# chaoyang223/UDA

Hardware: AMD Instinct MI355X
Metric: TeraSort shuffle+merge GB/s whole-node (higher is better)
Workload: dtype bytes

## Files before the change

### csrc/apps/colpack_bench_main.cc

```cpp
#include <chrono>
#include <cstdio>
#include <cstdlib>
#include <cstring>
#include <string>
#include <thread>
#include <vector>

#include "codec/colpack.h"

namespace {

double now_s() {
  return std::chrono::duration<double>(std::chrono::steady_clock::now().time_since_epoch()).count();
}

uint64_t splitmix(uint64_t& s) {
  uint64_t z = (s += 0x9e3779b97f4a7c15ull);
  z = (z ^ (z >> 30)) * 0xbf58476d1ce4e5b9ull;
  z = (z ^ (z >> 27)) * 0x94d049bb133111ebull;
  return z ^ (z >> 31);
}

void fill(std::vector<uint8_t>& v, int64_t n, uint64_t seed, uint64_t step_mask = 0xFFFFFF) {
  uint64_t key = seed << 40;
  for (int64_t r = 0; r < n; ++r) {
    uint8_t* p = v.data() + r * 104;
    p[0] = 0x0B, p[1] = 0x5B, p[2] = 0x0A, p[13] = 0x5A;
    key += splitmix(seed) & step_mask;
    for (int b = 0; b < 8; ++b) p[3 + b] = (uint8_t)(key >> (56 - 8 * b));
    const uint64_t t = splitmix(seed);
    p[11] = (uint8_t)t, p[12] = (uint8_t)(t >> 8);
    for (int c = 14; c < 104; ++c) p[c] = (uint8_t)('A' + splitmix(seed) % 26);
  }
}

struct Result {
  double unpack = 0, unpack_copy = 0, copy = 0;
  int64_t stride = 0;
};

}

int main(int argc, char** argv) {
  int threads = 1, reps = 3;
  int64_t mib = 128;
  bool scalar = false, v2 = false;
  for (int i = 1; i < argc; ++i) {
    const std::string a = argv[i];
    if (a == "--threads" && i + 1 < argc) threads = std::atoi(argv[++i]);
    else if (a == "--mib" && i + 1 < argc) mib = std::atoll(argv[++i]);
    else if (a == "--reps" && i + 1 < argc) reps = std::atoi(argv[++i]);
    else if (a == "--scalar") scalar = true;
    else if (a == "--v2") v2 = true;
    else {
      std::fprintf(stderr, "usage: uda_colpack_bench [--threads N] [--mib M] [--reps R] [--scalar] [--v2]\n");
      return 2;
    }
  }
  threads = threads < 1 ? 1 : threads;
  const int64_t buf_records = (1 << 20) / 104;
  const int64_t n = (mib << 20) / (buf_records * 104) * buf_records;
  if (n < buf_records || reps < 1) return 2;
  std::vector<Result> res((size_t)threads);
  std::vector<std::thread> thr;
  for (int t = 0; t < threads; ++t)
    thr.emplace_back([&, t] {
      std::vector<uint8_t> raw((size_t)(n * 104));
      fill(raw, n, 1234567 + (uint64_t)t, v2 ? (1ull << 38) - 1 : 0xFFFFFF);
      std::vector<uint8_t> piece((size_t)(v2 ? uda::colpack2_bound(104, n, buf_records) : uda::colpack_bound(104, n)));
      const int64_t len = v2 ? uda::colpack2_encode(raw.data(), n, 104, buf_records, 3, 10, piece.data())
                             : uda::colpack_encode(raw.data(), n, 104, buf_records, piece.data());
      uda::ColpackPiece p;
      if (!uda::colpack_open(piece.data(), len, 104, n, &p) || !p.packed || p.delta != v2) return;
      res[(size_t)t].stride = p.stride;
      std::vector<uint8_t> stg((size_t)(buf_records * 104) * 2), kv((size_t)(buf_records * 104));
      auto pass = [&](int mode) {
        double best = 0;
        for (int r = 0; r < reps; ++r) {
          const double t0 = now_s();
          int64_t turn = 0;
          for (int64_t row = 0; row < n; row += buf_records) {
            uint8_t* s = stg.data() + (size_t)(turn++ & 1) * (size_t)(buf_records * 104);
            if (mode != 2) {
              if (scalar) uda::colpack_unpack_scalar(p, row, buf_records, s);
              else uda::colpack_unpack(p, row, buf_records, s);
            }
            if (mode == 1) std::memcpy(kv.data(), s, kv.size());
            if (mode == 2) std::memcpy(kv.data(), raw.data() + row * 104, kv.size());
            asm volatile("" ::"r"(kv.data()), "r"(s) : "memory");
          }
          const double rate = (double)(n * 104) / (now_s() - t0);
          if (rate > best) best = rate;
        }
        return best;
      };
      res[(size_t)t].unpack = pass(0);
      res[(size_t)t].unpack_copy = pass(1);
      res[(size_t)t].copy = pass(2);
    });
  for (auto& t : thr) t.join();
  double u = 0, uc = 0, c = 0;
  for (const Result& r : res) {
    if (r.stride == 0) {
      std::fprintf(stderr, "a thread's piece did not pack\n");
      return 1;
    }
    u += r.unpack, uc += r.unpack_copy, c += r.copy;
  }
  std::printf("{\"threads\": %d, \"mib_per_thread\": %lld, \"version\": %d, \"stride\": %lld, \"bmi2\": %s, \"path\": \"%s\", "
              "\"unpack_GBps_per_thread\": %.2f, \"unpack_copy_GBps_per_thread\": %.2f, \"copy_GBps_per_thread\": %.2f}\n",
              threads, (long long)mib, v2 ? 2 : 1, (long long)res[0].stride, uda::colpack_have_bmi2() ? "true" : "false",
              scalar || !uda::colpack_have_bmi2() ? "scalar" : "bmi2", u / threads / 1e9, uc / threads / 1e9,
              c / threads / 1e9);
  return 0;
}
```

### csrc/codec/colpack.cc

```cpp
#include "codec/colpack.h"

#include <cstring>

#if defined(__x86_64__)
#include <immintrin.h>
#endif

namespace uda {

namespace {

typedef unsigned __int128 u128;

inline int bit_length(unsigned v) { return v ? 32 - __builtin_clz(v) : 0; }

inline u128 key_mask(int key_len) { return key_len >= 16 ? ~(u128)0 : (((u128)1 << (8 * key_len)) - 1); }

inline u128 load_be(const uint8_t* p, int n) {
  if (n >= 8) {
    uint64_t hi, lo;
    std::memcpy(&hi, p, 8);
    std::memcpy(&lo, p + n - 8, 8);
    return ((u128)__builtin_bswap64(hi) << (8 * (n - 8))) | __builtin_bswap64(lo);
  }
// ... 63 lines not shown

struct KeyWalk {
  const uint8_t* table = nullptr;
  int64_t buf_records = 1;
  int64_t next_restart = 0;
  int key_off = 0, key_len = 0;
  u128 mask = 0, sum = 0;

  void start(const ColpackPiece& p, const ColpackHeader& h, const Layout& lo, int64_t row0) {
    table = p.table;
    buf_records = p.buf_records;
    key_off = p.key_off;
    key_len = p.key_len;
    mask = key_mask(key_len);
    const int64_t rs = row0 - row0 % buf_records;
    next_restart = rs;
    if (rs == row0) return;
    sum = load_be(table + rs / buf_records * kColpackRestartBytes, key_len);
    for (int64_t r = rs + 1; r < row0; ++r)
      sum = (sum + key_delta_of_row(h, lo, p.rows + r * p.stride, key_off, key_len)) & mask;
    next_restart = rs + buf_records;
  }
  inline void fix(int64_t row, uint8_t* rec) {
    if (row == next_restart) {
      sum = load_be(table + row / buf_records * kColpackRestartBytes, key_len);
      next_restart += buf_records;
    } else {
      sum = (sum + load_be(rec + key_off, key_len)) & mask;
    }
    store_be(rec + key_off, key_len, sum);
  }
};

int64_t encode(const uint8_t* src, int64_t nrec, int L, int64_t buf_records, uint32_t version, int key_off,
               int key_len, uint8_t* dst) {
  if (L < 1 || L > kColpackMaxRecordBytes || nrec < 1) return 0;
  if (key_off < 0 || key_len < 0 || key_len > kColpackMaxKeyBytes || key_off + key_len > L) return 0;
  uint8_t mn[kColpackMaxRecordBytes], mx[kColpackMaxRecordBytes];
  uint8_t dmn[kColpackMaxKeyBytes], dmx[kColpackMaxKeyBytes];
  std::memset(mn, 0xFF, sizeof(mn));
  std::memset(mx, 0, sizeof(mx));
  std::memset(dmn, 0xFF, sizeof(dmn));
  std::memset(dmx, 0, sizeof(dmx));
  const bool keyed = key_len > 0 && buf_records >= 1;
  const u128 kmask = key_mask(key_len);
  u128 prev = 0;
  for (int64_t r = 0; r < nrec; ++r) {
    const uint8_t* rec = src + r * L;
    for (int c = 0; c < L; ++c) {
      if (rec[c] < mn[c]) mn[c] = rec[c];
      if (rec[c] > mx[c]) mx[c] = rec[c];
    }
    if (keyed) {
      const u128 k = load_be(rec + key_off, key_len);
      uint8_t t[kColpackMaxKeyBytes];
      store_be(t, key_len, r % buf_records == 0 ? (u128)0 : (k - prev) & kmask);
      prev = k;
      for (int c = 0; c < key_len; ++c) {
        if (t[c] < dmn[c]) dmn[c] = t[c];
        if (t[c] > dmx[c]) dmx[c] = t[c];
      }
    }
  }
  int64_t plain_bits = 0, delta_bits = 0;
  for (int c = 0; c < key_len; ++c) {
    plain_bits += bit_length((unsigned)(mx[key_off + c] - mn[key_off + c]));
    delta_bits += bit_length((unsigned)(dmx[c] - dmn[c]));
  }
  const bool delta = colpack2_choose_delta(plain_bits, delta_bits, nrec, buf_records, key_len);
  if (delta)
    for (int c = 0; c < key_len; ++c) {
      mn[key_off + c] = dmn[c];
      mx[key_off + c] = dmx[c];
    }
  ColpackHeader h;
  std::memset(&h, 0, sizeof(h));
  h.magic = kColpackMagic;
  h.version = version;
  h.record_bytes = (uint32_t)L;
  h.records = (uint64_t)nrec;
  h.buf_records = (uint32_t)buf_records;
  h.groups = (uint32_t)colpack_groups(L);
  h.key_off = (uint32_t)key_off;
  h.key_len = (uint32_t)key_len;
  uint8_t shift[kColpackMaxGroups][8];
  int bits[kColpackMaxGroups];
  uint16_t bo[kColpackMaxGroups];
  const int G = (int)h.groups;
  for (int g = 0; g < G; ++g) {
    int b = 0;
    for (int c = 0; c < 8 && 8 * g + c < L; ++c) {
      const int w = bit_length((unsigned)(mx[8 * g + c] - mn[8 * g + c]));
      shift[g][c] = (uint8_t)b;
      b += w;
      h.mask[g] |= (uint64_t)((1u << w) - 1) << (8 * c);
      h.base[g] |= (uint64_t)mn[8 * g + c] << (8 * c);
    }
    bits[g] = b;
  }
  const bool v1 = version == kColpackVersion;
  const int64_t S = colpack_layout(bits, G, v1, bo);
  for (int g = 0; g < G; ++g) {
    if (v1)
      h.gb[g] = (uint8_t)((bits[g] + 7) / 8);
    else
      h.bo[g] = bo[g];
  }
  h.stride = (uint32_t)S;
  const bool raw = colpack_is_raw(S, L);
  h.flags = (raw ? 0 : kColpackFlagPacked) | (delta ? kColpackFlagDelta : 0);
  std::memcpy(dst, &h, sizeof(h));
  if (raw) return (int64_t)kColpackHeaderBytes;
  const int64_t table_bytes = delta ? colpack2_table_bytes(nrec, buf_records) : 0;
  const int64_t total = v1 ? colpack_packed_bytes(S, nrec) : colpack2_packed_bytes(S, nrec, table_bytes);
  std::memset(dst + kColpackHeaderBytes, 0, (size_t)(total - (int64_t)kColpackHeaderBytes));
  if (delta)
    for (int64_t b = 0; b * buf_records < nrec; ++b)
      std::memcpy(dst + kColpackHeaderBytes + b * kColpackRestartBytes, src + b * buf_records * L + key_off,
                  (size_t)key_len);
  uint8_t* rows = dst + kColpackHeaderBytes + table_bytes;
  prev = 0;
  for (int64_t r = 0; r < nrec; ++r) {
    uint8_t rec[kColpackMaxRecordBytes];
    std::memcpy(rec, src + r * L, (size_t)L);
    if (delta) {
      const u128 k = load_be(rec + key_off, key_len);
      store_be(rec + key_off, key_len, r % buf_records == 0 ? (u128)0 : (k - prev) & kmask);
      prev = k;
    }
    uint8_t* row = rows + r * S;
    for (int g = 0; g < G; ++g) {
      uint64_t word = 0;
      for (int c = 0; c < 8 && 8 * g + c < L; ++c)
        word |= (uint64_t)(uint8_t)(rec[8 * g + c] - mn[8 * g + c]) << shift[g][c];
      const int sh = bo[g] & 7, nb = (sh + bits[g] + 7) / 8;
      word <<= sh;
      for (int k = 0; k < nb; ++k) row[(bo[g] >> 3) + k] |= (uint8_t)(word >> (8 * k));
    }
  }
  return total;
}

}

int64_t colpack_encode(const uint8_t* src, int64_t nrec, int L, int64_t buf_records, uint8_t* dst) {
  return encode(src, nrec, L, buf_records, kColpackVersion, 0, 0, dst);
}

int64_t colpack2_encode(const uint8_t* src, int64_t nrec, int L, int64_t buf_records, int key_off, int key_len,
                        uint8_t* dst) {
  if (key_off < 0 || key_len < 0 || key_len > kColpackMaxKeyBytes || key_off + key_len > L) return 0;
  if (buf_records < 1 || buf_records > 0xFFFFFFFFll) key_len = 0;
  return encode(src, nrec, L, buf_records, kColpackVersion2, key_len > 0 ? key_off : 0, key_len, dst);
}

bool colpack_open(const uint8_t* piece, int64_t len, int expect_L, int64_t expect_records, ColpackPiece* out,
                  const char** why) {
  auto fail = [&](const char* w) {
    if (why) *why = w;
    return false;
  };
  if (!piece || len < (int64_t)kColpackHeaderBytes) return fail("piece shorter than its header");
  const ColpackHeader* h = reinterpret_cast<const ColpackHeader*>(piece);
  ColpackHeader hc;
  std::memcpy(&hc, piece, sizeof(hc));
  if (hc.magic != kColpackMagic) return fail("bad magic");
  if (hc.version != kColpackVersion && hc.version != kColpackVersion2) return fail("unknown version");
  const bool v1 = hc.version == kColpackVersion;
  const int L = (int)hc.record_bytes;
  if (hc.record_bytes < 1 || hc.record_bytes > (uint32_t)kColpackMaxRecordBytes) return fail("record length out of range");
  if (expect_L > 0 && L != expect_L) return fail("record length differs from the stream's");
  if (hc.records < 1 || hc.records > (uint64_t)1 << 40) return fail("record count out of range");
  if (expect_records > 0 && (int64_t)hc.records != expect_records) return fail("record count differs from the item's");
  if ((int)hc.groups != colpack_groups(L)) return fail("group count does not match the record length");
  int bits[kColpackMaxGroups];
  uint16_t bo[kColpackMaxGroups];
  const int G = (int)hc.groups;
  for (int g = 0; g < G; ++g) {
    bits[g] = 0;
    for (int c = 0; c < 8; ++c) {
      const unsigned m = (unsigned)((hc.mask[g] >> (8 * c)) & 0xFF);
      if (m & (m + 1)) return fail("column mask is not a width mask");
      if (8 * g + c >= L && m) return fail("mask past the tail group's columns");
      bits[g] += __builtin_popcount(m);
    }
    if (v1 && hc.gb[g] != (bits[g] + 7) / 8) return fail("group size does not match its widths");
  }
  const int64_t S = colpack_layout(bits, G, v1, bo);
  if (!v1)
    for (int g = 0; g < kColpackMaxGroups; ++g)
      if (hc.bo[g] != (g < G ? bo[g] : 0)) return fail("group offsets do not match the masks");
  if ((int64_t)hc.stride != S) return fail(v1 ? "row stride does not match the group sizes" : "row stride does not match the masks");
  const bool packed = (hc.flags & kColpackFlagPacked) != 0;
  const bool delta = !v1 && (hc.flags & kColpackFlagDelta) != 0;
  int64_t table_bytes = 0;
  if (!v1) {
    if (hc.flags & ~(kColpackFlagPacked | kColpackFlagDelta)) return fail("unknown flags");
    if (hc.key_len > (uint32_t)kColpackMaxKeyBytes || hc.key_off > (uint32_t)L || hc.key_off + hc.key_len > (uint32_t)L)
      return fail("key field outside the record");
    if (delta && hc.key_len == 0) return fail("delta piece without a key");
    if (delta && hc.buf_records < 1) return fail("delta piece without buffer restarts");
    if (delta) table_bytes = colpack2_table_bytes((int64_t)hc.records, (int64_t)hc.buf_records);
  }
  if (packed) {
    if (colpack_is_raw(S, L)) return fail("packed piece with a raw stride");
    const int64_t need = v1 ? colpack_packed_bytes(S, (int64_t)hc.records)
                            : colpack2_packed_bytes(S, (int64_t)hc.records, table_bytes);
    if (need > len) return fail(v1 ? "rows exceed the piece's length" : "table and rows exceed the piece's length");
  }
  out->hdr = h;
  out->table = piece + kColpackHeaderBytes;
  out->rows = piece + kColpackHeaderBytes + table_bytes;
  out->L = L;
  out->version = (int)hc.version;
  out->records = (int64_t)hc.records;
  out->stride = S;
  out->buf_records = (int64_t)hc.buf_records;
  out->key_off = v1 ? 0 : (int)hc.key_off;
  out->key_len = v1 ? 0 : (int)hc.key_len;
  out->packed = packed;
  out->delta = delta;
  return true;
}

void colpack_unpack_scalar(const ColpackPiece& p, int64_t row0, int64_t rows, uint8_t* dst) {
  if (row0 < 0 || rows <= 0 || row0 + rows > p.records) return;
  ColpackHeader h;
  std::memcpy(&h, p.hdr, sizeof(h));
  const Layout lo = layout_of(h, p.L);
  KeyWalk kw;
  if (p.delta) kw.start(p, h, lo, row0);
  for (int64_t r = 0; r < rows; ++r) {
    const uint8_t* row = p.rows + (row0 + r) * p.stride;
    uint8_t* rec = dst + r * p.L;
    for (int g = 0; g < lo.groups; ++g) {
      const uint64_t word = load_le(row + lo.off[g], lo.nbytes[g]) >> lo.sh[g];
      for (int c = 0; c < lo.cols[g]; ++c) {
        const uint64_t m = (h.mask[g] >> (8 * c)) & 0xFF;
        rec[8 * g + c] = (uint8_t)(((word >> lo.shift[g][c]) & m) + ((h.base[g] >> (8 * c)) & 0xFF));
      }
    }
    if (p.delta) kw.fix(row0 + r, rec);
  }
}

bool colpack_have_bmi2() {
#if defined(__x86_64__)
  static const bool have = __builtin_cpu_supports("bmi2");
  return have;
#else
  return false;
#endif
}

#if defined(__x86_64__)
namespace {
template <int kFull, bool kDelta>
__attribute__((target("bmi2"))) void unpack_bmi2(const ColpackPiece& p, int64_t row0, int64_t rows, uint8_t* dst) {
  ColpackHeader h;
  std::memcpy(&h, p.hdr, sizeof(h));
  const Layout lo = layout_of(h, p.L);
  const int full = kFull ? kFull : p.L / 8;
  const int tail = kFull ? 0 : p.L % 8;
  const int64_t S = p.stride;
  const int L = p.L;
  KeyWalk kw;
  if (kDelta) kw.start(p, h, lo, row0);
  const uint8_t* row = p.rows + row0 * S;
  for (int64_t r = 0; r < rows; ++r, row += S, dst += L) {
#pragma GCC unroll 16
    for (int g = 0; g < full; ++g) {
      uint64_t x;
      std::memcpy(&x, row + lo.off[g], 8);
      x = _pdep_u64(x >> lo.sh[g], h.mask[g]) + h.base[g];
      std::memcpy(dst + 8 * g, &x, 8);
    }
    if (tail) {
      uint64_t x;
      std::memcpy(&x, row + lo.off[full], 8);
      x = _pdep_u64(x >> lo.sh[full], h.mask[full]) + h.base[full];
      std::memcpy(dst + 8 * full, &x, (size_t)tail);
    }
    if (kDelta) kw.fix(row0 + r, dst);
  }
}
}
#endif

bool colpack_unpack_bmi2(const ColpackPiece& p, int64_t row0, int64_t rows, uint8_t* dst) {
#if defined(__x86_64__)
  if (!colpack_have_bmi2()) return false;
  if (row0 < 0 || rows <= 0 || row0 + rows > p.records) return true;
  if (p.L == 104)
    p.delta ? unpack_bmi2<13, true>(p, row0, rows, dst) : unpack_bmi2<13, false>(p, row0, rows, dst);
  else
    p.delta ? unpack_bmi2<0, true>(p, row0, rows, dst) : unpack_bmi2<0, false>(p, row0, rows, dst);
  return true;
#else
  return false;
#endif
}

void colpack_unpack(const ColpackPiece& p, int64_t row0, int64_t rows, uint8_t* dst) {
  if (!colpack_unpack_bmi2(p, row0, rows, dst)) colpack_unpack_scalar(p, row0, rows, dst);
}

}
```

### csrc/codec/colpack.h

```cpp
#pragma once
#include <cstddef>
#include <cstdint>

#if defined(__HIP__)
#define UDA_COLPACK_HD __host__ __device__ inline
#else
#define UDA_COLPACK_HD inline
#endif

namespace uda {

constexpr uint32_t kColpackMagic = 0x4b504c43u;
constexpr uint32_t kColpackVersion = 1;
constexpr uint32_t kColpackVersion2 = 2;
constexpr int kColpackMaxRecordBytes = 256;
constexpr int kColpackMaxGroups = kColpackMaxRecordBytes / 8;
constexpr uint32_t kColpackFlagPacked = 1;
constexpr uint32_t kColpackFlagDelta = 2;
constexpr int kColpackMaxKeyBytes = 16;
constexpr int kColpackRestartBytes = 16;

struct ColpackHeader {
  uint32_t magic;
  uint32_t version;
  uint32_t record_bytes;
  uint32_t flags;
  uint64_t records;
  uint32_t buf_records;
  uint32_t stride;
  uint32_t groups;
  uint32_t key_off;
  uint32_t key_len;
  uint32_t reserved[5];
  uint64_t mask[kColpackMaxGroups];
  uint64_t base[kColpackMaxGroups];
  union {
    struct {
      uint8_t gb[kColpackMaxGroups];
      uint8_t pad[32];
    };
    uint16_t bo[kColpackMaxGroups];
  };
};
constexpr size_t kColpackHeaderBytes = sizeof(ColpackHeader);
static_assert(kColpackHeaderBytes == 640 && kColpackHeaderBytes % 64 == 0, "header is 64-byte aligned");

UDA_COLPACK_HD int colpack_groups(int L) { return (L + 7) / 8; }
UDA_COLPACK_HD bool colpack_is_raw(int64_t S, int64_t L) { return 10 * S > 9 * L; }
UDA_COLPACK_HD int64_t colpack_max_stride(int64_t L) { return 9 * L / 10; }
UDA_COLPACK_HD int64_t colpack_packed_bytes(int64_t S, int64_t nrec) {
  return ((int64_t)kColpackHeaderBytes + S * nrec + 8 + 63) / 64 * 64;
// ... 2 lines not shown


UDA_COLPACK_HD int colpack_layout(const int* bits, int groups, bool align_all, uint16_t* bo) {
  int cur = 0;
  for (int g = 0; g < groups; ++g) {
    if (bits[g] > 0 && (align_all || (cur & 7) + bits[g] > 64)) cur = (cur + 7) & ~7;
    bo[g] = (uint16_t)cur;
    cur += bits[g];
  }
  return (cur + 7) / 8;
}
UDA_COLPACK_HD int colpack_mask_bits(uint64_t m) {
  int n = 0;
  for (; m; m &= m - 1) ++n;
  return n;
}
UDA_COLPACK_HD int64_t colpack2_table_bytes(int64_t nrec, int64_t buf_records) {
  if (buf_records < 1) return 0;
  return ((nrec + buf_records - 1) / buf_records * kColpackRestartBytes + 63) / 64 * 64;
}
UDA_COLPACK_HD int64_t colpack2_packed_bytes(int64_t S, int64_t nrec, int64_t table_bytes) {
  return ((int64_t)kColpackHeaderBytes + table_bytes + S * nrec + 8 + 63) / 64 * 64;
}
UDA_COLPACK_HD int64_t colpack2_bound(int64_t L, int64_t nrec, int64_t buf_records) {
  return colpack2_packed_bytes(colpack_max_stride(L), nrec, colpack2_table_bytes(nrec, buf_records));
}
UDA_COLPACK_HD bool colpack2_choose_delta(int64_t plain_key_bits, int64_t delta_key_bits, int64_t nrec,
                                          int64_t buf_records, int key_len) {
  if (key_len <= 0 || buf_records < 1) return false;
  const int64_t entries = (nrec + buf_records - 1) / buf_records;
  return delta_key_bits * nrec + 128 * entries < plain_key_bits * nrec;
}

int64_t colpack_encode(const uint8_t* src, int64_t nrec, int L, int64_t buf_records, uint8_t* dst);
int64_t colpack2_encode(const uint8_t* src, int64_t nrec, int L, int64_t buf_records, int key_off, int key_len,
                        uint8_t* dst);

struct ColpackPiece {
  const ColpackHeader* hdr = nullptr;
  const uint8_t* table = nullptr;
  const uint8_t* rows = nullptr;
  int L = 0;
  int version = 0;
  int64_t records = 0;
  int64_t stride = 0;
  int64_t buf_records = 0;
  int key_off = 0, key_len = 0;
  bool packed = false;
  bool delta = false;
};
bool colpack_open(const uint8_t* piece, int64_t len, int expect_L, int64_t expect_records, ColpackPiece* out,
                  const char** why = nullptr);

void colpack_unpack(const ColpackPiece& p, int64_t row0, int64_t rows, uint8_t* dst);
void colpack_unpack_scalar(const ColpackPiece& p, int64_t row0, int64_t rows, uint8_t* dst);
bool colpack_unpack_bmi2(const ColpackPiece& p, int64_t row0, int64_t rows, uint8_t* dst);
bool colpack_have_bmi2();

}
```

### csrc/consumer/gpu_merge_device.cc

```cpp
#include <fcntl.h>
#include <sys/stat.h>
#include <hip/hip_runtime.h>
#include <unistd.h>

#include <algorithm>
#include <atomic>
#include <chrono>
#include <ctime>
#include <condition_variable>
#include <deque>
#include <map>
#include <memory>
#include <mutex>
#include <cstdio>
#include <cstdlib>
#include <cstring>
#include <fstream>
#include <future>
#include <random>
#include <set>
#include <thread>

#include "../gpu/block_decoder.h"
#include "../gpu/device_ptr.h"
// ... 479 lines not shown
    st_.hbm_wait_ms += hbm_res->wait_ms();
    st_.hbm_reserved = hbm_res->granted();
    st_.round_bytes = round_bytes;
  };
  if (codec_ != Codec::kNone) {
    const auto td = std::chrono::steady_clock::now();
    std::vector<const uint8_t*> cp;
    std::vector<int64_t> cl;
    for (const auto& p : parts) {
      cp.push_back(p->dptr);
      cl.push_back(p->part_len);
    }
    gpu::BlockPlan bp;
    std::vector<int64_t> roff;
    int64_t blocks = 0;
    std::vector<int> tails;
    const bool dev_frames = gpu::plan_block_streams_device(codec_, cp, cl, &bp, ws.frame_scratch, ws.frame_descs, s,
                                                           &tails, launch_checksums);
    if (dev_frames) {
      finish_checksums(!bp.descs.empty());
      for (size_t i = 0; i < parts.size(); ++i)
        if (tails[i] && parts[i]->raw_len > 0 && bp.raw_offset[i + 1] - bp.raw_offset[i] != parts[i]->raw_len)
          throw UdaError("compressed map output " + parts[i]->map_id + " decodes to " +
                         std::to_string(bp.raw_offset[i + 1] - bp.raw_offset[i]) + " bytes, its index says " +
                         std::to_string(parts[i]->raw_len));
    }
    if (dev_frames && kind_ == KeyKind::kText && combine_ == CombineOp::kNone &&
        host_->conf_i64("mapred.uda.gpu.decode.stream", 1) != 0) {
      gpu::DeviceReduceConfig cfg;
      cfg.device = device;
      cfg.kv_buf_bytes = kv_buf_size_;
      cfg.round_bytes = round_bytes;
      cfg.pack_version = delivery_pack_;
      cfg.piece_bytes = delivery_piece_bytes_;
      cfg.stop = [&] { return stop_.load(); };
      if (const int slots = (int)host_->conf_i64("mapred.uda.gpu.decode.stream.slots", 3); slots > 0) {
        cfg.decode_turn = [this, device, slots] {
          return DeviceGate::get(1).acquire(device, slots, [&] { return stop_.load(); });
        };
        cfg.decode_done = [device] { DeviceGate::get(1).release(device); };
      }
      bool streamed = false;
      const gpu::DeviceReduceStats ds = gpu::device_reduce_fixed_blocks(cfg, (int)codec_, bp, sink, &streamed);
      if (streamed) {
        std::lock_guard<std::mutex> g(st_mu_);
        st_.hbm_wait_ms += ds.hbm_wait_ms;
        st_.gpu_gate_wait_ms += ds.decode_wait_ms;
        st_.hbm_reserved = ds.hbm_reserved;
        st_.round_bytes = ds.round_bytes;
        st_.records = ds.records;
        st_.rpq_rounds = ds.rounds;
        st_.device_decoded_blocks += ds.decoded_blocks;
        st_.gpu_device_ms = ds.plan_ms + ds.merge_wait_ms;
        st_.gpu_d2h_wait_ms = ds.d2h_wait_ms;
        st_.gpu_sink_ms = ds.sink_ms;
        st_.gpu_d2h_bytes = ds.d2h_bytes;
        st_.gpu_packed_pieces = ds.packed_pieces;
        st_.gpu_raw_pieces = ds.raw_pieces;
        st_.gpu_unpack_ms = ds.unpack_ms;
        st_.fetch_ms = fetch_ms;
        st_.merge_ms = std::chrono::duration<double, std::milli>(std::chrono::steady_clock::now() - t0).count() - fetch_ms;
        st_.merge_path = "device-fixed10-stream";
        ws_lease.clean = true;
        return true;
      }
    }
    if (dev_frames) {
      const int64_t raw = bp.raw_total;
      gpu::DeviceReduceConfig pcfg;
      pcfg.kv_buf_bytes = kv_buf_size_;
      pcfg.pack_version = delivery_pack_;
      pcfg.piece_bytes = delivery_piece_bytes_;
      admit(std::max<int64_t>(0, raw + raw / 8 - (int64_t)ws.in.held()), [&](int64_t rb) {
        return gpu::fixed_round_ws_bytes(std::min(rb, raw), (int)parts.size(), &pcfg);
      });
    }
    GateLease dgate;
    dgate.which = 1;
    if (const int slots = (int)host_->conf_i64("mapred.uda.gpu.decode.slots", 1); slots > 0) {
      if (!DeviceGate::get(1).acquire(device, slots, [&] { return stop_.load(); }))
        throw UdaError("reduce task stopped while waiting for a device decode slot");
      dgate.device = device;
    }
    if (dev_frames) {
      DeviceWorkspace::ensure(ws.in, bp.raw_total);
      ws.decoder.decode(codec_, bp, nullptr, ws.in.as<uint8_t>(), s);
      roff = bp.raw_offset;
      blocks = (int64_t)bp.descs.size();
    } else {
      UDA_LOG(kInfo, "device decode: framing needs a host decode (%s)", codec_name(codec_));
      std::vector<std::vector<uint8_t>> raws;
      roff.assign(1, 0);
      for (size_t i = 0; i < cp.size(); ++i) {
        std::vector<uint8_t> c((size_t)cl[i]);
        if (cl[i] > 0) HIP_CHECK(hipMemcpy(c.data(), cp[i], (size_t)cl[i], hipMemcpyDefault));
        int tail = 0;
        std::vector<uint8_t> raw = host_decode_partition(codec_, c.data(), (int64_t)c.size(), &tail);
        if (tail) {
          ++trailers;
          const int64_t body = (int64_t)c.size() - tail;
          if (parts[i]->raw_len > 0 && (int64_t)raw.size() != parts[i]->raw_len)
            throw UdaError("compressed map output " + parts[i]->map_id + " decodes to " + std::to_string(raw.size()) +
                           " bytes, its index says " + std::to_string(parts[i]->raw_len));
          if (verify) {
// ... 9 lines not shown
      for (size_t i = 0; i < raws.size(); ++i)
        if (!raws[i].empty())
          HIP_CHECK(hipMemcpy(ws.in.as<uint8_t>() + roff[i], raws[i].data(), raws[i].size(), hipMemcpyHostToDevice));
    }
    for (size_t i = 0; i < parts.size(); ++i) {
      parts[i]->dptr = ws.in.as<uint8_t>() + roff[i];
      parts[i]->part_len = roff[i + 1] - roff[i];
    }
    HIP_CHECK(hipStreamSynchronize(s));
    std::lock_guard<std::mutex> g(st_mu_);
    st_.device_decoded_blocks += blocks;
    st_.gpu_decode_ms = std::chrono::duration<double, std::milli>(std::chrono::steady_clock::now() - td).count();
  }
  bool fixed = kind_ == KeyKind::kText && combine_ == CombineOp::kNone;
  std::vector<gpu::RunDesc> runs;
  for (const auto& p : parts) {
    const int64_t rec_bytes = p->part_len - kEofBytes;
    if (rec_bytes < 0 || rec_bytes % gpu::kTeraRecordBytes != 0) fixed = false;
    gpu::RunDesc d;
    d.base = p->dptr;
    d.nbytes = std::max<int64_t>(rec_bytes, 0);
    d.nrec = d.nbytes / gpu::kTeraRecordBytes;
    d.offsets = nullptr;
    runs.push_back(d);
  }
  const bool fixed10 = fixed && gpu::runs_are_fixed10(runs, s);
  finish_checksums(fixed && !runs.empty());
  if (fixed10) {
    gpu::DeviceReduceConfig cfg;
    cfg.device = device;
    cfg.kv_buf_bytes = kv_buf_size_;
    cfg.round_bytes = round_bytes;
    cfg.pack_version = delivery_pack_;
    cfg.piece_bytes = delivery_piece_bytes_;
    cfg.stop = [&] { return stop_.load(); };
    gpu::DeviceReduceStats ds = gpu::device_reduce_fixed(cfg, runs, sink);
    std::lock_guard<std::mutex> g(st_mu_);
    if (!hbm_res) {
      st_.hbm_wait_ms += ds.hbm_wait_ms;
      st_.hbm_reserved = ds.hbm_reserved;
    }
    st_.round_bytes = ds.round_bytes;
    st_.records = ds.records;
    st_.rpq_rounds = ds.rounds;
    st_.gpu_device_ms = ds.plan_ms + ds.merge_wait_ms;
    st_.gpu_d2h_wait_ms = ds.d2h_wait_ms;
    st_.gpu_sink_ms = ds.sink_ms;
    st_.gpu_d2h_bytes = ds.d2h_bytes;
    st_.gpu_packed_pieces = ds.packed_pieces;
    st_.gpu_raw_pieces = ds.raw_pieces;
    st_.gpu_unpack_ms = ds.unpack_ms;
    st_.fetch_ms = fetch_ms;
    st_.merge_ms = std::chrono::duration<double, std::milli>(std::chrono::steady_clock::now() - t0).count() - fetch_ms;
    st_.merge_path = "device-fixed10";
    ws_lease.clean = true;
    return true;
  }
  int64_t total = 0;
  std::vector<const uint8_t*> rptr;
  std::vector<int64_t> rlen;
  for (const auto& p : parts) {
    rptr.push_back(p->dptr);
    rlen.push_back(p->part_len);
    total += p->part_len;
  }
  if (!hbm_res) {
// ... 183 lines not shown
```

### csrc/consumer/gpu_prewarm.cc

```cpp
#include <hip/hip_runtime.h>

#include <algorithm>
#include <chrono>
#include <cstdio>
#include <memory>
#include <mutex>
#include <string>
#include <vector>

#include "../gpu/device_ptr.h"
#include "../gpu/device_reduce.h"
#include "../gpu/device_engine.h"
#include "../gpu/fixed_delivery.h"
#include "../gpu/sdma.h"
#include "gpu_workspace.h"
#include "reduce_task.h"
#include "uda/log.h"

namespace uda {

namespace {
void warm_code(int device) {
  static std::once_flag code_once;
  std::call_once(code_once, [device] {
// ... 5 lines not shown
    try {
      gpu::SdmaEngine::for_device(device).warm(tmp);
    } catch (const std::exception& e) {
      UDA_LOG(kWarn, "GPU prewarm: SDMA warm-up: %s", e.what());
    }
    HIP_CHECK(hipFree(tmp));
  });
}

void warm_workspaces(int device, int n) {
  std::vector<std::unique_ptr<PoolLease<DeviceWorkspace>>> held;
  for (int i = 0; i < std::max(1, n); ++i) {
    held.emplace_back(new PoolLease<DeviceWorkspace>{
        device, DevicePool<DeviceWorkspace>::get().acquire(device, [] { return std::make_unique<DeviceWorkspace>(); })});
    auto& wl = *held.back();
    if (wl.obj->ring.size() < (size_t)(2 * kPieceBytes))
      wl.obj->ring.alloc_on_node((size_t)(2 * kPieceBytes), gpu::device_numa_node(device));
    wl.clean = true;
  }
}
}

void prewarm_node_merges(int device, int tasks, int64_t round_bytes, int maps, int64_t kv_buf) {
  HIP_CHECK(hipSetDevice(device));
  (void)gpu::SdmaEngine::for_device(device);
  warm_code(device);
  warm_workspaces(device, tasks);
  gpu::prewarm_streams(device, tasks);
  gpu::DeviceReduceConfig cfg;
  cfg.device = device;
  cfg.kv_buf_bytes = kv_buf;
  cfg.round_bytes = round_bytes;
  cfg.pack_version = std::max(0, gpu::delivery_pack_version("auto"));
  gpu::prewarm_device_reduce(cfg, std::max(1, maps), tasks);
}

void ReduceTask::prewarm_gpu(PrewarmConf pc) {
  const auto t0 = std::chrono::steady_clock::now();
  auto tp = t0;
  std::string phases;
  auto lap = [&](const char* name) {
    const auto t = std::chrono::steady_clock::now();
    char b[48];
    std::snprintf(b, sizeof(b), "%s%s=%.1f", phases.empty() ? "" : " ", name,
                  std::chrono::duration<double, std::milli>(t - tp).count());
    phases += b;
    tp = t;
  };
  try {
    std::call_once(placed_, [this] { place_on_gpu(); });
    if (gpu::device_count() <= 0) return;
    const int device = device_;
    if (hipSetDevice(device) != hipSuccess) return;
    lap("hip");
    try {
      (void)gpu::SdmaEngine::for_device(device);
    } catch (const std::exception&) {
    }
    lap("sdma");
    warm_code(device);
    lap("code");
    warm_workspaces(device, 1);
    if (pc.early_h2d) {
      PoolLease<EarlyStager> sl{device, DevicePool<EarlyStager>::get().acquire(
                                            device, [device] { return std::make_unique<EarlyStager>(device); })};
      sl.clean = true;
    }
    lap("ws");
    {
      gpu::DeviceReduceConfig cfg;
      cfg.device = device;
      cfg.kv_buf_bytes = kv_buf_size_;
      cfg.round_bytes = pc.round_bytes;
      cfg.pack_version = pc.delivery_pack;
      cfg.piece_bytes = pc.delivery_piece_bytes;
      gpu::prewarm_device_reduce(cfg, std::max(1, pc.maps));
    }
    lap("fixed10");
    const int64_t pin = pc.pinned_bytes;
    std::vector<gpu::PinnedPool::Block> blocks;
    for (int64_t b = 0; b < pin && !stop_; b += (int64_t)gpu::PinnedArena::kBlock)
      blocks.push_back(gpu::PinnedPool::instance().acquire(gpu::PinnedArena::kBlock));
    for (auto& b : blocks) gpu::PinnedPool::instance().release(b);
    lap("pinned");
  } catch (const std::exception& e) {
    UDA_LOG(kWarn, "GPU prewarm: %s", e.what());
  }
  std::lock_guard<std::mutex> g(st_mu_);
  st_.gpu_prewarm_ms = std::chrono::duration<double, std::milli>(std::chrono::steady_clock::now() - t0).count();
  st_.gpu_prewarm_phases = phases;
}

void ReduceTask::join_prewarm() {
  if (!prewarm_thr_.joinable()) {
    std::call_once(placed_, [this] { place_on_gpu(); });
    return;
  }
  const auto t0 = std::chrono::steady_clock::now();
  prewarm_thr_.join();
  std::call_once(placed_, [this] { place_on_gpu(); });
  std::lock_guard<std::mutex> g(st_mu_);
  st_.gpu_prewarm_wait_ms = std::chrono::duration<double, std::milli>(std::chrono::steady_clock::now() - t0).count();
}

}
```

### csrc/consumer/reduce_task.cc

```cpp
#include "reduce_task.h"
#include "uda/fault.h"

#include <fcntl.h>
#include <climits>
#include <cstdlib>
#include <sys/stat.h>
#include <unistd.h>

#include <algorithm>
#include <chrono>
#include <cmath>
#include <cstdio>
#include <cstring>
#include <fstream>
#include <map>
#include <iomanip>
#include <random>
#include <sstream>

#include "../gpu/fixed_delivery.h"
#include "../gpu/hbm_ledger.h"
#include "uda/log.h"
#include "uda/node_registry.h"
#include "uda/queues.h"
// ... 472 lines not shown
    } else {
    const int64_t delta = pair - (hard_min + min_fetch);
    uncomp_buf = hard_min + (int64_t)((double)delta * std::min(1.0, std::max(0.0, ratio)));
    fetch_buf_ = pair - uncomp_buf;
    const int64_t spare = std::max<int64_t>(fetch_buf_ - max_fetch, 0);
    fetch_buf_ -= spare;
    uncomp_buf += spare;
    }
  }
  if (fault_hit("HOST_ALLOC")) throw UdaError("injected allocation failure for the fetch buffer pool");
  kv_buf_size_ = host_->conf_i64("mapred.uda.kv.buf.size", 1 << 20);
  fault_spec_ = host_->get_conf("mapred.uda.fault.inject", "");
  direct_chunk_ = std::max<int64_t>(buffer_size_, host_->conf_i64("mapred.uda.fetch.request.bytes", 4 << 20));
  backend_ = host_->get_conf("mapred.uda.merge.backend", "auto");
  if (backend_ == "auto") {
    backend_ = gpu::visible_device_keys().empty() ? "cpu" : "gpu";
    UDA_LOG(kInfo, "mapred.uda.merge.backend=auto: %s merge", backend_.c_str());
  }
  if (backend_ != "cpu" && backend_ != "gpu") throw ProtocolError("unknown mapred.uda.merge.backend " + backend_);
  const std::string comb = host_->get_conf("mapred.uda.merge.combine", "none");
  if (!combine_op_from_conf(comb, &combine_))
    throw ProtocolError("unknown mapred.uda.merge.combine \"" + comb + "\" (" + kCombineAllowed + ")");
  const std::string cob = host_->get_conf("mapred.uda.merge.combine.over.budget", "skip");
  if (cob != "skip" && cob != "combine")
    throw ProtocolError("unknown mapred.uda.merge.combine.over.budget \"" + cob + "\" (skip or combine)");
  combine_over_budget_ = cob == "combine";
  const std::string ck = host_->get_conf("mapred.uda.ifile.checksum", "auto");
  if (!checksum_mode_from_conf(ck, &checksum_))
    throw ProtocolError("unknown mapred.uda.ifile.checksum \"" + ck + "\" (auto or off)");
  merge_round_bytes_ = std::max<int64_t>(4 << 10, host_->conf_i64("mapred.uda.gpu.merge.round.bytes", 256ll << 20));
  if (backend_ == "gpu") {
    const std::string pack = host_->get_conf("mapred.uda.gpu.delivery.pack", "auto");
    delivery_pack_ = gpu::delivery_pack_version(pack);
    if (delivery_pack_ < 0) throw ProtocolError("unknown mapred.uda.gpu.delivery.pack \"" + pack + "\" (auto, v1 or off)");
    delivery_piece_bytes_ = host_->conf_i64("mapred.uda.gpu.delivery.piece.bytes", 64ll << 20);
    if (delivery_piece_bytes_ < 1)
      throw ProtocolError("mapred.uda.gpu.delivery.piece.bytes must be positive, got " + std::to_string(delivery_piece_bytes_));
  }
  const std::string tr = host_->get_conf("mapred.uda.transport", "tcp");
  transport_ = (tr == "loopback") ? make_loopback_client()
                                  : make_tcp_client(net_.data_port, net_.wqes_per_conn,
                                                    (int)host_->conf_i64("mapred.uda.tcp.connections", 4));
  {
    std::lock_guard<std::mutex> g(st_mu_);
    st_.backend = backend_;
    st_.combine = combine_op_name(combine_);
    st_.key_order = key_order_name(key_order_);
    st_.fetch_buf_bytes = fetch_buf_;
    st_.uncomp_buf_bytes = uncomp_buf;
  }
  inited_ = true;
  UDA_LOG(kInfo, "reduce task %s: maps=%d approach=%d lpqs=%d kv_bufs=%d buffer=%ld codec=%s key=%s backend=%s",
          p.reduce_task_id.c_str(), maps, net_.online, num_lpqs_, num_kv_bufs_, (long)buffer_size_,
          codec_name(codec_), key_kind_name(kind_), backend_.c_str());
  checkpoint_ = host_->conf_i64("mapred.uda.lpq.checkpoint", 0) != 0 && (backend_ == "gpu" || net_.online == 2);
  if (checkpoint_ && sandbox_.enabled && init_.local_dirs.empty()) checkpoint_ = false;
  if (checkpoint_) load_checkpoint();
  if (backend_ == "gpu") {
    device_conf_ = host_->get_conf("mapred.uda.gpu.device", "auto");
    hbm_budget_conf_ = std::atof(host_->get_conf("mapred.uda.gpu.hbm.budget", "0").c_str());
  }
  if (backend_ == "gpu" && host_->conf_i64("mapred.uda.gpu.prewarm", 1) != 0) {
    PrewarmConf pc;
    pc.early_h2d = host_->conf_i64("mapred.uda.gpu.early.h2d", 1) != 0;
    if (host_->get_conf("mapred.uda.gpu.fetch", "auto") != "device")
      pc.pinned_bytes = host_->conf_i64("mapred.uda.gpu.prewarm.pinned.mb", 1024) << 20;
    pc.round_bytes = host_->conf_i64("mapred.uda.gpu.round.bytes", 2ll << 30);
    pc.maps = p.num_maps;
    pc.delivery_pack = delivery_pack_;
    pc.delivery_piece_bytes = delivery_piece_bytes_;
    prewarm_thr_ = std::thread([this, pc] { name_thread("uda-task-warm"); prewarm_gpu(pc); });
  }
  merge_thr_ = std::thread([this] { name_thread("uda-task-merge"); merge_main(); });
}

void ReduceTask::place_on_gpu() {
  const std::string conf = forced_device_ >= 0 ? std::to_string(forced_device_) : device_conf_;
  const std::vector<std::string> keys = gpu::visible_device_keys();
  if (keys.empty()) {
    device_ = 0;
    return;
  }
  NodeRegistry* reg = NodeRegistry::instance();
  if (conf != "auto" && !conf.empty()) {
    device_ = std::atoi(conf.c_str());
    if (device_ < 0 || device_ >= (int)keys.size())
      throw UdaError("mapred.uda.gpu.device=" + conf + " but " + std::to_string(keys.size()) + " GPU(s) are visible");
    if (reg) registry_slot_ = reg->add_task(keys[(size_t)device_], init_.reduce_task_id);
  } else if (reg) {
    const NodeRegistry::Placement pl = reg->place_task(keys, init_.reduce_task_id);
    device_ = pl.index;
    registry_slot_ = pl.slot;
  } else {
    device_ = 0;
  }
  gpu::HbmLedger::get().configure(device_, hbm_budget_conf_);
  std::lock_guard<std::mutex> g(st_mu_);
  st_.gpu_device = device_;
}

std::string map_task_of(const std::string& attempt) {
  const size_t u = attempt.rfind('_');
// ... 451 lines not shown
```

### csrc/consumer/reduce_task.h

```cpp
#pragma once
#include <atomic>
#include <condition_variable>
#include <deque>
#include <functional>
#include <map>
#include <memory>
#include <mutex>
#include <set>
#include <string>
#include <thread>
#include <vector>

#include "uda/cmd.h"
#include "uda/codec.h"
#include "uda/combine.h"
#include "uda/compare.h"
#include "uda/host.h"
#include "uda/ifile.h"
#include "uda/transport.h"

namespace uda {

class MofFetcher;
class StagedMerge;
// ... 82 lines not shown
  bool finished() const { return finished_.load(); }
  std::string task_id() const { return inited_ ? init_.reduce_task_id : std::string(); }
  ReduceStats stats() const;
  std::string stats_json() const;

  ClientTransport* transport() { return transport_.get(); }
  int64_t fetch_direct(const FetchParams& f, uint8_t* dst, int64_t off, int64_t end, int depth,
                       const std::function<void(int64_t, int64_t)>& on_prefix = nullptr, int64_t prefix_step = 0);
  void fetch_begin();
  void fetch_end();

 private:
  void on_init(const InitParams& p);
  void merge_main();
  void merge_online();
  void merge_hybrid();
  void merge_gpu();
  bool merge_gpu_device(bool probe);
  struct DeclinedPart {
    FetchParams f;
    int64_t len = 0;
    std::string path;
    int64_t file_off = 0;
  };
  int64_t fetch_declined_bytes(int device, const std::vector<DeclinedPart>& parts, gpu::DeviceBuffer& dst,
                               std::vector<const uint8_t*>* at, int64_t* local);
  void release_descriptors(const std::set<std::string>& hosts, const std::string& holder);
  struct PrewarmConf {
    bool early_h2d = true;
    int64_t pinned_bytes = 0;
    int64_t round_bytes = 2ll << 30;
    int maps = 0;
    int delivery_pack = 2;
    int64_t delivery_piece_bytes = 64ll << 20;
  };
  void prewarm_gpu(PrewarmConf pc);
  void join_prewarm();
  void place_on_gpu();
  std::once_flag placed_;
  TaskSandbox sandbox_;
  int forced_device_ = -1;
  std::string device_conf_ = "auto";
  std::string fault_spec_;
  double hbm_budget_conf_ = 0;
  int delivery_pack_ = 2;
  CombineOp combine_ = CombineOp::kNone;
  ChecksumMode checksum_ = ChecksumMode::kAuto;
  void note_checksum(int64_t parts, int64_t bytes, double gpu_ms = 0);
  bool combine_over_budget_ = false;
  int64_t merge_round_bytes_ = 256ll << 20;
  int64_t delivery_piece_bytes_ = 64ll << 20;
  int device_ = 0;
  int registry_slot_ = -1;
  void note_map_fetched(int64_t bytes = 0);
  void fetch_phase(MergeQueue* q, int n, std::vector<std::string>* map_ids = nullptr);
  void load_checkpoint();
  std::string checkpoint_path() const;
  void merging_phase(MergeQueue* q);
  std::unique_ptr<Segment> segment_for(std::shared_ptr<MofFetcher> f, int index);

  NetlevOptions net_;
  Host* host_;
  InitParams init_;
  KeyKind kind_ = KeyKind::kText;
  KeyOrder key_order_ = KeyOrder::kReference;
  Codec codec_ = Codec::kNone;
  int64_t buffer_size_ = 0;
  int64_t direct_chunk_ = 0;
  int64_t fetch_buf_ = 0;
  int64_t kv_buf_size_ = 1 << 20;
  int num_kv_bufs_ = 0;
  int num_lpqs_ = 0;
  int num_parallel_lpqs_ = 3;
  bool checkpoint_ = false;
  std::vector<std::string> restored_files_;
  std::set<std::string> restored_maps_;
  std::map<std::string, std::string> restored_tasks_;
  void discard_checkpoint();
// ... 83 lines not shown
```

### csrc/gpu/colpack.hip

```cpp
#include "codec/colpack.h"
#include "kernels.h"

#include <algorithm>

namespace uda {
namespace gpu {

namespace {
constexpr int kCpThreads = 256;
constexpr int kCpTileRows = 128;
constexpr int kCpTileBytes = kCpTileRows * (9 * kColpackMaxRecordBytes / 10);
constexpr int kCpTableDelta = 2 * kColpackMaxRecordBytes;
constexpr int kCpTableStride = kCpTableDelta + 2 * kColpackMaxKeyBytes;

__device__ __forceinline__ uint64_t load_cols(const uint8_t* p, int n) {
  if (n == 8 && (reinterpret_cast<uintptr_t>(p) & 7) == 0) return *reinterpret_cast<const uint64_t*>(p);
  uint64_t x = 0;
  for (int k = 0; k < n; ++k) x |= (uint64_t)p[k] << (8 * k);
  return x;
}

struct Key128 {
  uint64_t hi, lo;
};
// ... 88 lines not shown
        }
      }
    }
#pragma unroll
    for (int c = 0; c < 8; ++c)
      if (c < ncol) {
        atomicMin(&s_mn[8 * g + c], mn[c]);
        atomicMax(&s_mx[8 * g + c], mx[c]);
        const int kc = 8 * g + c - ko;
        if (keyed && kc >= 0 && kc < kl) {
          atomicMin(&s_dmn[kc], dmn[c]);
          atomicMax(&s_dmx[kc], dmx[c]);
        }
      }
  }
  __syncthreads();
  uint32_t* tb = table + (size_t)blockIdx.y * kCpTableStride;
  if (t < L) {
    atomicMin(&tb[t], s_mn[t]);
    atomicMin(&tb[kColpackMaxRecordBytes + t], 255u - s_mx[t]);
  }
  if (t < kl) {
    atomicMin(&tb[kCpTableDelta + t], s_dmn[t]);
    atomicMin(&tb[kCpTableDelta + kColpackMaxKeyBytes + t], 255u - s_dmx[t]);
  }
}

__device__ __forceinline__ int width_of(uint32_t mn, uint32_t mx) {
  const uint32_t range = mx > mn ? mx - mn : 0;
  return range ? 32 - __clz((int)range) : 0;
}

__global__ void __launch_bounds__(64) colpack_plan_kernel(const ColpackPieceDesc* pieces, int L, uint32_t buf_records,
                                                          uint32_t version, int ko, int kl, const uint32_t* table,
                                                          ColpackResult* results) {
  const ColpackPieceDesc pc = pieces[blockIdx.x];
  const uint32_t* tb = table + (size_t)blockIdx.x * kCpTableStride;
  const int G = (L + 7) / 8;
  const int t = threadIdx.x;
  const bool v1 = version == kColpackVersion;
  ColpackHeader* h = reinterpret_cast<ColpackHeader*>(pc.dst);
  __shared__ int s_bits[kColpackMaxGroups];
  __shared__ uint16_t s_bo[kColpackMaxGroups];
  __shared__ int s_stride;
  int64_t plain_bits = 0, delta_bits = 0;
  for (int c = 0; c < kl; ++c) {
    plain_bits += width_of(tb[ko + c], 255u - tb[kColpackMaxRecordBytes + ko + c]);
    delta_bits += width_of(tb[kCpTableDelta + c], 255u - tb[kCpTableDelta + kColpackMaxKeyBytes + c]);
  }
  const bool delta = colpack2_choose_delta(plain_bits, delta_bits, pc.nrec, buf_records, kl);
  if (t < kColpackMaxGroups) {
    uint64_t mask = 0, base = 0;
    int bits = 0;
    if (t < G)
      for (int c = 0; c < 8 && 8 * t + c < L; ++c) {
        const int col = 8 * t + c, kc = col - ko;
        uint32_t mn = tb[col], mx = 255u - tb[kColpackMaxRecordBytes + col];
        if (delta && kc >= 0 && kc < kl) {
          mn = tb[kCpTableDelta + kc];
          mx = 255u - tb[kCpTableDelta + kColpackMaxKeyBytes + kc];
        }
        const int w = width_of(mn, mx);
        bits += w;
        mask |= (uint64_t)((1u << w) - 1) << (8 * c);
        base |= (uint64_t)(mn & 0xFF) << (8 * c);
      }
    h->mask[t] = mask;
    h->base[t] = base;
    s_bits[t] = bits;
  }
  __syncthreads();
  if (t == 0) s_stride = colpack_layout(s_bits, G, v1, s_bo);
  __syncthreads();
  if (t < kColpackMaxGroups) {
    if (v1) {
      h->gb[t] = (uint8_t)((s_bits[t] + 7) / 8);
      h->pad[t] = 0;
    } else {
      h->bo[t] = t < G ? s_bo[t] : (uint16_t)0;
    }
  }
  const int64_t S = s_stride;
  const bool raw = colpack_is_raw(S, L);
  const int64_t table_bytes = delta ? colpack2_table_bytes(pc.nrec, buf_records) : 0;
  const int64_t total = raw  ? (int64_t)kColpackHeaderBytes
                        : v1 ? colpack_packed_bytes(S, pc.nrec)
                             : colpack2_packed_bytes(S, pc.nrec, table_bytes);
  if (t == 0) {
    h->magic = kColpackMagic;
    h->version = version;
    h->record_bytes = (uint32_t)L;
    h->flags = (raw ? 0 : kColpackFlagPacked) | (delta ? kColpackFlagDelta : 0);
    h->records = (uint64_t)pc.nrec;
    h->buf_records = buf_records;
    h->stride = (uint32_t)S;
    h->groups = (uint32_t)G;
    h->key_off = (uint32_t)ko;
    h->key_len = (uint32_t)kl;
    for (int k = 0; k < 5; ++k) h->reserved[k] = 0;
    ColpackResult r;
    r.bytes = total;
    r.packed = raw ? 0 : 1;
    r.stride = (uint32_t)S;
    r.delta = delta ? 1 : 0;
    r.reserved = 0;
    results[blockIdx.x] = r;
  }
  if (raw) return;
  if (delta) {
    uint8_t* tab = pc.dst + kColpackHeaderBytes;
    const int64_t entries = (pc.nrec + buf_records - 1) / buf_records;
    for (int64_t b = t; b < entries; b += 64) {
      const uint8_t* key = pc.src + b * buf_records * L + ko;
      for (int k = 0; k < kColpackRestartBytes; ++k) tab[b * kColpackRestartBytes + k] = k < kl ? key[k] : (uint8_t)0;
    }
    for (int64_t i = entries * kColpackRestartBytes + t; i < table_bytes; i += 64) tab[i] = 0;
  }
  for (int64_t i = (int64_t)kColpackHeaderBytes + table_bytes + S * pc.nrec + t; i < total; i += 64) pc.dst[i] = 0;
}

template <int kG>
__global__ void __launch_bounds__(kCpThreads) colpack_pack_kernel(const ColpackPieceDesc* pieces, int L) {
  const ColpackPieceDesc pc = pieces[blockIdx.y];
  const ColpackHeader* h = reinterpret_cast<const ColpackHeader*>(pc.dst);
  const uint32_t flags = h->flags;
  if (!(flags & kColpackFlagPacked)) return;
  const int S = (int)h->stride;
  if (S == 0) return;
  const int64_t ntiles = (pc.nrec + kCpTileRows - 1) / kCpTileRows;
  if ((int64_t)blockIdx.x >= ntiles) return;
  const int G = kG ? kG : (L + 7) / 8;
  const int t = threadIdx.x;
  const bool delta = (flags & kColpackFlagDelta) != 0;
  const uint32_t buf_records = h->buf_records;
  const int ko = (int)h->key_off, kl = delta ? (int)h->key_len : 0;
  __shared__ uint64_t s_base[kColpackMaxGroups];
  __shared__ uint64_t s_shift[kColpackMaxGroups];
  __shared__ int s_bits[kColpackMaxGroups];
  __shared__ uint16_t s_bo[kColpackMaxGroups];
  __shared__ __attribute__((aligned(16))) uint32_t s_tile[kCpTileBytes / 4 + 4];
  if (t < G) {
    const uint64_t mask = h->mask[t];
    uint64_t sh = 0;
    int bits = 0;
    for (int c = 0; c < 8; ++c) {
      sh |= (uint64_t)bits << (8 * c);
      bits += __popc((uint32_t)(mask >> (8 * c)) & 0xFF);
    }
    s_shift[t] = sh;
    s_base[t] = h->base[t];
    s_bits[t] = bits;
  }
  __syncthreads();
  if (t == 0) colpack_layout(s_bits, G, h->version == kColpackVersion, s_bo);
  __syncthreads();
  uint8_t* rows = pc.dst + kColpackHeaderBytes + (delta ? colpack2_table_bytes(pc.nrec, buf_records) : 0);
  for (int64_t tile = blockIdx.x; tile < ntiles; tile += gridDim.x) {
    const int64_t r0 = tile * kCpTileRows;
    const int nrows = (int)min((int64_t)kCpTileRows, pc.nrec - r0);
    const int nbytes = nrows * S;
    for (int i = t; i < (nbytes + 15) >> 4; i += kCpThreads) reinterpret_cast<uint4*>(s_tile)[i] = make_uint4(0, 0, 0, 0);
    __syncthreads();
    const uint8_t* src = pc.src + r0 * L;
    for (int i = t; i < nrows * G; i += kCpThreads) {
      const int r = i / G, g = i - r * G;
      if (s_bits[g] == 0) continue;
      const int ncol = min(8, L - 8 * g);
      const uint8_t* rec = src + (int64_t)r * L;
      uint64_t x = load_cols(rec + 8 * g, ncol);
      if (group_has_key(g, ko, kl)) x = with_key_delta(x, g, key_delta(rec, r0 + r, L, buf_records, ko, kl), ko, kl);
      x -= s_base[g];
      const uint64_t sh = s_shift[g];
      uint64_t word = 0;
#pragma unroll
      for (int c = 0; c < 8; ++c) word |= ((x >> (8 * c)) & 0xFF) << ((uint32_t)(sh >> (8 * c)) & 0xFF);
      const int bit = r * S * 8 + s_bo[g];
      const int wi = bit >> 5, ws = bit & 31;
      const uint64_t lo = word << ws;
      const uint32_t w0 = (uint32_t)lo, w1 = (uint32_t)(lo >> 32), w2 = ws ? (uint32_t)(word >> (64 - ws)) : 0u;
      if (w0) atomicOr(&s_tile[wi], w0);
      if (w1) atomicOr(&s_tile[wi + 1], w1);
      if (w2) atomicOr(&s_tile[wi + 2], w2);
    }
    __syncthreads();
    uint8_t* out = rows + r0 * S;
    const int n16 = nbytes >> 4;
    for (int i = t; i < n16; i += kCpThreads)
      reinterpret_cast<uint4*>(out)[i] = reinterpret_cast<const uint4*>(s_tile)[i];
    for (int i = (n16 << 4) + t; i < nbytes; i += kCpThreads) out[i] = reinterpret_cast<const uint8_t*>(s_tile)[i];
    __syncthreads();
  }
}
}

size_t colpack_table_bytes(int npieces) { return (size_t)npieces * kCpTableStride * sizeof(uint32_t); }

void launch_colpack(const ColpackPieceDesc* pieces, int npieces, int64_t max_nrec, int L, int64_t buf_records,
                    uint32_t* table, ColpackResult* results, hipStream_t s, int version, int key_off, int key_len) {
  if (npieces <= 0) return;
  if (version != (int)kColpackVersion2) version = (int)kColpackVersion, key_len = 0;
  if (key_len <= 0 || key_len > kColpackMaxKeyBytes || key_off < 0 || key_off + key_len > L || buf_records < 1 ||
      buf_records > 0xFFFFFFFFll)
    key_len = 0;
  if (key_len == 0) key_off = 0;
  (void)hipMemsetAsync(table, 0xFF, colpack_table_bytes(npieces), s);
  const int G = (L + 7) / 8;
  const int rows_per_iter = kCpThreads / G;
  int64_t sb = (max_nrec + (int64_t)rows_per_iter * 32 - 1) / ((int64_t)rows_per_iter * 32);
  sb = std::max<int64_t>(1, std::min<int64_t>(sb, 256));
  hipLaunchKernelGGL(colpack_stats_kernel, dim3((unsigned)sb, (unsigned)npieces), dim3(kCpThreads), 0, s, pieces, L,
                     (uint32_t)buf_records, key_off, key_len, table);
  hipLaunchKernelGGL(colpack_plan_kernel, dim3((unsigned)npieces), dim3(64), 0, s, pieces, L, (uint32_t)buf_records,
                     (uint32_t)version, key_off, key_len, table, results);
  int64_t pb = (max_nrec + kCpTileRows - 1) / kCpTileRows;
  pb = std::max<int64_t>(1, std::min<int64_t>(pb, 1024));
  if (G == 13)
    hipLaunchKernelGGL(colpack_pack_kernel<13>, dim3((unsigned)pb, (unsigned)npieces), dim3(kCpThreads), 0, s, pieces, L);
  else
    hipLaunchKernelGGL(colpack_pack_kernel<0>, dim3((unsigned)pb, (unsigned)npieces), dim3(kCpThreads), 0, s, pieces, L);
}

}
}
```

### csrc/gpu/device_engine.cc

```cpp
#include "device_engine.h"
#include "device_ptr.h"
#include "hbm_ledger.h"
#include "merge_plan.h"
#include "sdma.h"
#include "uda/fault.h"
#include "uda/topology.h"
#include "uda/trace.h"

#include <rccl/rccl.h>
#include <unistd.h>

#include <algorithm>
#include <atomic>
#include <chrono>
#include <cstring>
#include <map>
#include <mutex>
#include <numeric>
#include <stdexcept>

#include "uda/log.h"
#include "uda/vint.h"
#include "uda/thread_name.h"

// ... 673 lines not shown
  PlanBufs& pb = pbufs_[kp.pslot];
  HIP_CHECK(hipStreamWaitEvent(s, pb.planned, 0));
  KwayDesc kd = kp.kd;
  static const bool prof = std::getenv("UDA_KWAY_PROF") != nullptr;
  if (prof) {
    auto ensure = [](DeviceBuffer& b, size_t bytes) {
      if (b.size() < bytes) b.alloc_local(bytes + bytes / 8);
    };
    ensure(kw_prof_, (size_t)kp.ncells * 5 * 8);
    HIP_CHECK(hipMemsetAsync(kw_prof_.as(), 0, (size_t)kp.ncells * 5 * 8, s));
    kd.prof = kw_prof_.as<unsigned long long>();
  }
  HIP_CHECK(hipGetLastError());
  launch_kway_tiles(kd, kp.ncells, out, s);
  HIP_CHECK(hipGetLastError());
  HIP_CHECK(hipEventRecord(pb.used, s));
  pb.used_valid = true;
  if (prof) report_kway_phases(kd.prof, kp.ncells, s);
  last_passes_ = 1;
  return kp.total;
}

ShuffleJob::ShuffleJob(const ShuffleConfig& cfg) : cfg_(cfg) {
  if (cfg_.world < 1 || cfg_.rank < 0 || cfg_.rank >= cfg_.world)
    throw std::runtime_error("ShuffleJob: bad rank/world");
  if (cfg_.maps_per_rank < 1) throw std::runtime_error("ShuffleJob: maps_per_rank < 1");
  if (cfg_.rounds < 1) cfg_.rounds = 1;
  if (cfg_.reducers < 1) cfg_.reducers = 1;
  if (cfg_.pinned_slots < 2) cfg_.pinned_slots = 2;
  if (cfg_.d2h != "sdma" && cfg_.d2h != "hip") throw std::runtime_error("ShuffleJob: d2h must be sdma or hip");
  if (cfg_.store != "hbm" && cfg_.store != "host" && cfg_.store != "disk")
    throw std::runtime_error("unknown store tier " + cfg_.store);
  const int version = delivery_pack_version(cfg_.delivery_pack);
  if (version < 0) throw std::runtime_error("ShuffleJob: delivery_pack must be auto, v1 or off");
  check_delivery_order(cfg_.delivery_order);
  pack_ = cfg_.deliver_host && version != 0;
  lay_ = fixed_layout(cfg_.kv_buf_bytes, cfg_.d2h_piece_bytes, cfg_.pinned_slots, pack_ ? version : 0);
  R_ = cfg_.reducers;
  Q_ = cfg_.rounds;
  C_ = R_ * Q_;
  if ((int64_t)R_ * cfg_.world * cfg_.maps_per_rank > 65536)
    throw std::runtime_error("ShuffleJob: reducers * world * maps_per_rank must be <= 65536 (merge run index)");
  HIP_CHECK(hipSetDevice(cfg_.device));
  int lo_prio = 0, hi_prio = 0;
  HIP_CHECK(hipDeviceGetStreamPriorityRange(&lo_prio, &hi_prio));
  const bool spill = cfg_.store != "hbm";
  HIP_CHECK(hipStreamCreateWithPriority(&s_comm_, hipStreamNonBlocking, spill ? lo_prio : hi_prio));
  HIP_CHECK(hipStreamCreateWithPriority(&s_compute_, hipStreamNonBlocking, spill ? hi_prio : lo_prio));
  HIP_CHECK(hipStreamCreateWithFlags(&s_copy_, hipStreamNonBlocking));
  HIP_CHECK(hipStreamCreateWithFlags(&s_plan_, hipStreamNonBlocking));
  merged_ev_.resize(kSlots);
  comm_ev_.resize(kSlots);
  sent_ev_.resize(2);
  early_ev_.resize(kSlots);
  for (auto& e : early_ev_) HIP_CHECK(hipEventCreateWithFlags(&e, hipEventDisableTiming));
  for (auto& e : merged_ev_) HIP_CHECK(hipEventCreateWithFlags(&e, hipEventDisableTiming));
  for (auto& e : comm_ev_) HIP_CHECK(hipEventCreateWithFlags(&e, hipEventDisableTiming));
  for (auto& e : sent_ev_) HIP_CHECK(hipEventCreateWithFlags(&e, hipEventDisableTiming));
}

ShuffleJob::~ShuffleJob() {
  {
    std::lock_guard<std::mutex> g(mu_);
    stop_ = true;
  }
  cv_.notify_all();
  if (copy_thr_.joinable()) copy_thr_.join();
  for (auto& t : consumers_)
    if (t.joinable()) t.join();
  (void)hipDeviceSynchronize();
// ... 13 lines not shown
  exchange_.reset();
  if (s_copy_) (void)hipStreamDestroy(s_copy_);
  if (s_plan_) (void)hipStreamDestroy(s_plan_);
  if (s_comm_) (void)hipStreamDestroy(s_comm_);
  if (s_compute_) (void)hipStreamDestroy(s_compute_);
}

void ShuffleJob::init_comm(const std::string& uid) {
  if (cfg_.world == 1) return;
  HIP_CHECK(hipSetDevice(cfg_.device));
  exchange_ = make_rccl_exchange(cfg_.rank, cfg_.world, uid);
}

void ShuffleJob::init_local() {
  if (cfg_.world == 1) return;
  if (cfg_.local_group.empty()) throw std::runtime_error("init_local: config.local_group is empty");
  HIP_CHECK(hipSetDevice(cfg_.device));
  exchange_ = make_local_exchange(cfg_.local_group, cfg_.rank, cfg_.world);
}

void ShuffleJob::init_ipc(const std::string& name) {
  if (cfg_.world == 1) return;
  HIP_CHECK(hipSetDevice(cfg_.device));
  exchange_ = make_ipc_exchange(name, cfg_.rank, cfg_.world, cfg_.device);
}

std::string ShuffleJob::delivery_name() const {
  if (!cfg_.deliver_host) return "none";
  std::string name = sdma_ ? sdma_->describe() : "hip[numa=" + std::to_string(device_numa_node(cfg_.device)) + "]";
  name += " ring=" + ring_numa_ + " order=" + cfg_.delivery_order;
  if (!pack_) return name + " pack=off";
  name += " pack=colbits v" + std::to_string(lay_.pack_version);
  if (last_delta_ >= 0) name += last_delta_ ? " delta" : " plain";
  if (last_d2h_ratio_ >= 0) {
    char b[32];
    std::snprintf(b, sizeof(b), " d2h/in=%.3f", last_d2h_ratio_);
    name += b;
  }
  return name;
}

std::vector<ShuffleJob::PackPiece> ShuffleJob::round_pieces(const std::vector<int64_t>& group_recs) const {
  std::vector<PackPiece> v;
  int64_t doff = 0;
  for (const DeliveryPiece& dp : delivery_schedule(group_recs, lay_.piece, "reducer", kTeraRecordBytes)) {
    const int64_t nrec = dp.len / kTeraRecordBytes;
    v.push_back(PackPiece{dp.src_off, doff, nrec});
    doff += lay_.piece_bound(nrec);
  }
  return v;
}

void ShuffleJob::note_issue(int k, double now) {
  if (first_issue_ms_ < 0) first_issue_ms_ = now;
  if (flying_ == 0 && idle_since_ms_ >= 0) step_link_idle_ms_ += now - idle_since_ms_;
  slot_flying_[k] = true;
  ++flying_;
}

void ShuffleJob::note_landing(int k, double now) {
  if (!slot_flying_[k]) return;
  slot_flying_[k] = false;
  last_landing_ms_ = now;
  if (--flying_ == 0) idle_since_ms_ = now;
}

// ... 723 lines not shown
        if (pack_) {
          const size_t pi = (size_t)dp.pack_index;
          if (pi >= ppieces.size() || (size_t)issued >= ppieces.size() || ppieces[pi].src_off != dp.src_off ||
              ppieces[pi].nrec * kTeraRecordBytes != dp.len)
            throw std::runtime_error("delivery_pack: piece list out of step with the copy loop");
          const ColpackResult pr = pres[issued];
          if (pr.packed) {
            packed = true;
            copy_len = lay_.packed_copy_len(pr.bytes, ppieces[pi].nrec);
            from = packed_slots_[r.slot].as<uint8_t>() + ppieces[pi].dst_off;
          }
        }
        if (sdma_) {
          SdmaEngine::arm(piece_sig_[k], sdma_->parts((size_t)copy_len, cfg_.d2h_engines));
          sdma_->copy_d2h(dst, from, (size_t)copy_len, piece_sig_[k], cfg_.d2h_engines);
        } else {
          HIP_CHECK(hipMemcpyAsync(dst, from, (size_t)copy_len, hipMemcpyDeviceToHost, s_copy_));
          HIP_CHECK(hipEventRecord(piece_ev_[k], s_copy_));
        }
        used.push_back(k);
        ++issued;
        {
          std::lock_guard<std::mutex> g(mu_);
          const double now = now_ms();
          note_issue(k, now);
          items_[dp.reducer].push_back(Item{k, dp.len, last_round && dp.last_of_reducer, now, r.q, packed, copy_len});
          step_d2h_bytes_ += copy_len;
          ++(packed ? step_packed_ : step_raw_);
          if (packed) {
            const ColpackResult pr = pres[issued - 1];
            step_delta_ += pr.delta ? 1 : 0;
            step_stride_min_ = step_stride_min_ < 0 ? (int64_t)pr.stride : std::min<int64_t>(step_stride_min_, pr.stride);
            step_stride_max_ = std::max<int64_t>(step_stride_max_, pr.stride);
          }
        }
        cv_.notify_all();
      }
      for (int k : used) {
        if (sdma_)
          SdmaEngine::wait(piece_sig_[k]);
        else
          HIP_CHECK(hipEventSynchronize(piece_ev_[k]));
        std::lock_guard<std::mutex> g(mu_);
        note_landing(k, now_ms());
      }
      {
        std::lock_guard<std::mutex> g(mu_);
        out_free_[r.q] = 1;
      }
      cv_.notify_all();
    }
  } catch (const std::exception& e) {
    std::lock_guard<std::mutex> g(mu_);
    if (step_error_msg_.empty()) step_error_msg_ = std::string("delivery copy thread: ") + e.what();
    stop_ = true;
    cv_.notify_all();
  }
}

void ShuffleJob::consume_loop(int i) {
  try {
    bind_thread_to_cpus(device_consumer_cpus(cfg_.device));
    HIP_CHECK(hipSetDevice(cfg_.device));
    FixedBuffers bufs;
    bufs.tail = eof_bufs_[i].get();
    if (pack_) {
// ... 135 lines not shown
        note(first[3], "output slot changed between the merge and its D2H", q, i, pre_d2h[(size_t)q * R_ + i], merged);
      }
      if (deliv[(size_t)q * R_ + i] != merged) {
        ++st.delivery_errors;
        note(first[4], "consumer received other bytes than the merge wrote", q, i, deliv[(size_t)q * R_ + i], merged);
      }
    }
  }
  st.diag.clear();
  for (const auto& f : first)
    if (!f.empty()) st.diag += (st.diag.empty() ? "" : "; ") + f;
}

StepStats ShuffleJob::run_step(bool validate) {
  trace::Range tr_step("uda.step");
  HIP_CHECK(hipSetDevice(cfg_.device));
  if (!merger_) throw std::runtime_error("run_step before plan()");
  StepStats st;
  st.validated = validate;
  const double t0 = now_ms();
  const int M = cfg_.maps_per_rank, W = cfg_.world, me = cfg_.rank;
  const bool deliver = cfg_.deliver_host;
  {
    std::lock_guard<std::mutex> g(mu_);
    if (stop_) throw std::runtime_error("delivery pipeline stopped: " + step_error_msg_);
    out_free_.assign(Q_, 0);
    eof_count_ = 0;
    step_buffers_ = 0;
    step_error_ = 0;
    step_d2h_ms_ = 0;
    step_d2h_bytes_ = step_packed_ = step_raw_ = step_delta_ = 0;
    step_stride_min_ = -1;
    step_stride_max_ = 0;
    step_unpack_ms_ = 0;
    step_t0_ms_ = t0;
    first_issue_ms_ = last_landing_ms_ = idle_since_ms_ = eof_done_ms_ = -1;
    step_link_idle_ms_ = step_slot_wait_ms_ = 0;
    step_check_delivery_ = validate && cfg_.check_delivery && deliver;
    pre_d2h_ck_.assign((size_t)Q_ * R_, 0);
    delivered_ck_.assign((size_t)Q_ * R_, 0);
  }
  std::vector<hipEvent_t> ev(4 * (size_t)Q_);
  for (auto& e : ev) HIP_CHECK(hipEventCreate(&e));
  unsigned long long* vstats = d_validate_.as<unsigned long long>();
  Elem* vprev = reinterpret_cast<Elem*>(d_validate_.as<uint8_t>() + 64);
  Elem* vlast = vprev + R_;
  std::vector<bool> has_prev(R_, false);
  if (validate) {
    HIP_CHECK(hipMemsetAsync(d_validate_.as(), 0, 64, s_compute_));
    HIP_CHECK(hipMemsetAsync(d_diag_.as(), 0, (size_t)Q_ * diag_stride() * 8, s_compute_));
  }
  if (cfg_.replan) {
    const double tp = now_ms();
    refresh_plan();
    st.plan_ms = now_ms() - tp;
  }

  auto wait_until = [&](const std::function<bool()>& ready) {
    std::unique_lock<std::mutex> lk(mu_);
    while (!cv_.wait_for(lk, std::chrono::milliseconds(100), [&] { return ready() || stop_; })) {
      if (exchange_) {
        lk.unlock();
        wait_exchange_ok();
        lk.lock();
      }
    }
// ... 216 lines not shown
    HIP_CHECK(hipEventRecord(ev[4 * q + 2], s_compute_));
    uint8_t* out = out_slots_[slot].as<uint8_t>();
    int64_t n = 0;
    if (lookahead) {
      n = merger_->run_kway(next_plan, out, s_compute_);
      if (q + 1 < Q_) {
        build_runs(q + 1, runs, group_first);
        next_plan = merger_->plan_kway(runs, group_first, s_plan_);
      }
    } else {
      n = merger_->merge_fixed(runs, group_first, out, s_compute_);
    }
    HIP_CHECK(hipGetLastError());
    st.merge_passes = std::max(st.merge_passes, merger_->last_passes());
    if (validate) {
      int64_t goff = 0;
      for (int i = 0; i < R_; ++i) {
        const int64_t g = rp.group_recs[i];
        if (g > 0) {
          launch_validate_fixed(out + goff * kTeraRecordBytes, g, vprev + i, has_prev[i] ? 1 : 0, vlast + i, vstats,
                                s_compute_, dg + 4 + i);
          HIP_CHECK(hipMemcpyAsync(vprev + i, vlast + i, sizeof(Elem), hipMemcpyDeviceToDevice, s_compute_));
          has_prev[i] = true;
        }
        goff += g;
      }
      check_inputs(1);
    }
    HIP_CHECK(hipEventRecord(ev[4 * q + 3], s_compute_));
    if (pack_ && deliver && pack_n_[q] > 0) {
      auto pack_range = [&](int a, int b) {
        launch_colpack(d_pack_pieces_[q].as<ColpackPieceDesc>() + a, b - a, pack_max_nrec_[q], kTeraRecordBytes,
                       lay_.buf_records, d_pack_table_.as<uint32_t>(), d_pack_results_[slot].as<ColpackResult>() + a,
                       s_compute_, lay_.pack_version, kTeraKeyOffset, kTeraKeyBytes);
        HIP_CHECK(hipGetLastError());
        HIP_CHECK(hipMemcpyAsync(h_pack_results_[slot].as<ColpackResult>() + a,
                                 d_pack_results_[slot].as<ColpackResult>() + a, (size_t)(b - a) * sizeof(ColpackResult),
                                 hipMemcpyDeviceToHost, s_compute_));
      };
      if (pack_early_[q] > 0) {
        pack_range(0, pack_early_[q]);
        HIP_CHECK(hipEventRecord(early_ev_[slot], s_compute_));
      }
      pack_range(pack_early_[q], pack_n_[q]);
    }
    HIP_CHECK(hipEventRecord(merged_ev_[slot], s_compute_));
    if (sdma_stage) {
      std::lock_guard<std::mutex> g(mu_);
      merge_recorded[q] = 1;
      cv_.notify_all();
    }
    st.records += n;
    if (deliver) {
      {
        std::lock_guard<std::mutex> g(mu_);
        round_q_.push_back(RoundOut{q, slot, rp.group_recs, pack_early_[q]});
      }
      cv_.notify_all();
    }
  }
  if (deliver) wait_until([&] { return eof_count_ == R_; });
  if (exchange_) exchange_->wait(s_comm_);
  HIP_CHECK(hipStreamSynchronize(s_compute_));
  HIP_CHECK(hipStreamSynchronize(s_comm_));
  HIP_CHECK(hipStreamSynchronize(s_copy_));
  if (stage_thr.joinable()) stage_thr.join();
  if (exchange_) exchange_->quiesce();
  st.wall_ms = now_ms() - t0;
  st.stage_ms = stage_ms;
  for (int q = 0; q < Q_; ++q) {
    float a = 0, b = 0;
    if (staged() && hipEventElapsedTime(&a, ev[4 * q + 0], ev[4 * q + 1]) == hipSuccess) st.comm_ms += a;
    if (hipEventElapsedTime(&b, ev[4 * q + 2], ev[4 * q + 3]) == hipSuccess) st.merge_ms += b;
    st.round_comm_ms.push_back(a);
    st.round_merge_ms.push_back(b);
  }
  static const bool round_trace = std::getenv("UDA_ROUND_TRACE") != nullptr;
  if (round_trace && staged()) {
    std::string line = "[round trace ms: comm start-end | merge start-end]";
    for (int q = 0; q < Q_; ++q) {
      float t[4] = {0, 0, 0, 0};
      for (int k = 0; k < 4; ++k) (void)hipEventElapsedTime(&t[k], ev[0], ev[4 * q + k]);
      char b[96];
      snprintf(b, sizeof(b), " q%d %.0f-%.0f|%.0f-%.0f", q, t[0], t[1], t[2], t[3]);
      line += b;
    }
    fprintf(stderr, "%s\n", line.c_str());
  }
  for (auto e : ev) (void)hipEventDestroy(e);
  st.d2h_ms = step_d2h_ms_;
  st.bytes_in = st.records * kTeraRecordBytes;
  st.buffers = step_buffers_;
  {
    std::lock_guard<std::mutex> g(mu_);
    st.d2h_bytes = step_d2h_bytes_;
    st.packed_pieces = step_packed_;
    st.raw_pieces = step_raw_;
    st.pack_delta_pieces = step_delta_;
    st.pack_stride_min = std::max<int64_t>(step_stride_min_, 0);
    st.pack_stride_max = step_stride_max_;
    if (deliver && pack_) last_delta_ = step_packed_ > 0 && step_delta_ == step_packed_ ? 1 : 0;
    st.unpack_ms = step_unpack_ms_;
    st.slot_wait_ms = step_slot_wait_ms_;
    if (first_issue_ms_ >= 0) {
      st.lead_in_ms = first_issue_ms_ - step_t0_ms_;
      st.link_idle_ms = step_link_idle_ms_;
      if (eof_done_ms_ >= last_landing_ms_) st.tail_ms = eof_done_ms_ - last_landing_ms_;
    }
  }
  if (deliver && st.bytes_in > 0) last_d2h_ratio_ = (double)st.d2h_bytes / (double)st.bytes_in;
  if (validate) {
    unsigned long long v[3];
    HIP_CHECK(hipMemcpy(v, vstats, sizeof(v), hipMemcpyDeviceToHost));
    st.order_errors = (int64_t)v[0];
    st.checksum = v[1];
    st.exchange_errors = W > 1 ? (int64_t)v[2] : 0;
    localize_mismatch(st);
  }
  st.bad_layout = merger_->bad_layout();
  if (step_error_) throw std::runtime_error("delivery sink reported error " + std::to_string(step_error_));
  return st;
}

}
}
```

### csrc/gpu/device_engine.h

```cpp
#pragma once
#include <hip/hip_runtime.h>

#include <atomic>
#include <condition_variable>
#include <cstdint>
#include <deque>
#include <functional>
#include <map>
#include <memory>
#include <mutex>
#include <string>
#include <thread>
#include <vector>

#include "delivery_schedule.h"
#include "exchange.h"
#include "fixed_delivery.h"
#include "kernels.h"
#include "disk_store.h"
#include "sdma.h"

namespace uda {
namespace gpu {

// ... 185 lines not shown
  int d2h_engines = 1;
  std::string d2h = "sdma";
  bool deliver_host = true;
  bool validate = false;
  std::string local_group;
  std::string store = "hbm";
  std::string local_dirs;
  bool replan = false;
  bool map_sort = false;
  bool check_delivery = false;
  std::string delivery_pack = "auto";
  std::string delivery_order = "wave";
};

struct StepStats {
  double wall_ms = 0;
  double comm_ms = 0;
  double merge_ms = 0;
  double d2h_ms = 0;
  double wait_out_ms = 0;
  double plan_ms = 0;
  double stage_ms = 0;
  int64_t bytes_in = 0;
  int64_t records = 0;
  int64_t bytes_sent = 0;
  int64_t bytes_h2d = 0;
  int64_t buffers = 0;
  int64_t d2h_bytes = 0;
  int64_t packed_pieces = 0;
  int64_t raw_pieces = 0;
  int64_t pack_delta_pieces = 0;
  int64_t pack_stride_min = 0;
  int64_t pack_stride_max = 0;
  double unpack_ms = 0;
  double lead_in_ms = 0;
  double link_idle_ms = 0;
  double tail_ms = 0;
  double slot_wait_ms = 0;
  int merge_passes = 0;
  bool validated = false;
  int64_t order_errors = -1;
  uint64_t checksum = 0;
  int64_t exchange_errors = -1;
  bool bad_layout = false;
  int64_t pre_merge_errors = -1;
  int64_t own_errors = -1;
  int64_t merge_errors = -1;
  int64_t pre_d2h_errors = -1;
  int64_t delivery_errors = -1;
  std::string diag;
  std::vector<double> round_comm_ms, round_merge_ms;
};

class ShuffleJob {
 public:
  explicit ShuffleJob(const ShuffleConfig& cfg);
  ~ShuffleJob();

  const ShuffleConfig& config() const { return cfg_; }
  void init_comm(const std::string& uid);
  void init_local();
  void init_ipc(const std::string& name);
  void generate();
  std::vector<std::vector<uint64_t>> sample_keys(int64_t every);
  void set_bounds(const std::vector<uint64_t>& bounds);
  void plan();
// ... 85 lines not shown
  std::vector<DeviceBuffer> d_own_runs_, d_own_expect_;
  std::vector<int> own_n_;
  std::vector<int64_t> own_max_nrec_;
  std::vector<uint64_t> expect_group_ck_;
  DeviceBuffer d_diag_;
  int diag_stride() const { return 4 + R_; }
  std::vector<uint64_t> pre_d2h_ck_, delivered_ck_;
  bool step_check_delivery_ = false;
  DeviceBuffer d_d2h_runs_, d_d2h_ck_;
  std::vector<DeviceBuffer> h2d_descs_;
  std::vector<int> h2d_n_;
  std::vector<int64_t> h2d_max_;
  int h2d_blocks_ = 2048;
  bool sdma_h2d_ = true;
  hipStream_t s_stage_ = nullptr;
  FixedLayout lay_;
  struct PackPiece {
    int64_t src_off;
    int64_t dst_off;
    int64_t nrec;
  };
  std::vector<PackPiece> round_pieces(const std::vector<int64_t>& group_recs) const;
  bool pack_ = false;
  std::vector<DeviceBuffer> packed_slots_;
  std::vector<DeviceBuffer> d_pack_pieces_;
  std::vector<int> pack_n_;
  std::vector<int> pack_early_;
  std::vector<hipEvent_t> early_ev_;
  std::vector<int64_t> pack_max_nrec_;
  DeviceBuffer d_pack_table_;
  std::vector<DeviceBuffer> d_pack_results_;
  std::vector<PinnedBuffer> h_pack_results_;
  double last_d2h_ratio_ = -1;
  int last_delta_ = -1;

  std::unique_ptr<SdmaEngine> sdma_;
  uint8_t* ring_ = nullptr;
  std::string ring_numa_;
  std::vector<hsa_signal_t> piece_sig_;
  std::vector<hipEvent_t> piece_ev_;
  struct RoundOut {
    int q;
    int slot;
    std::vector<int64_t> group_recs;
    int early = 0;
  };
  struct Item {
    int pslot;
    int64_t bytes;
    bool last;
    double issued_ms;
    int q;
    bool packed = false;
    int64_t copied = 0;
  };
  std::mutex mu_;
  std::condition_variable cv_;
  std::deque<RoundOut> round_q_;
  std::vector<std::deque<Item>> items_;
  std::vector<bool> pinned_free_;
  std::vector<int> out_free_;
  std::thread copy_thr_;
  std::vector<std::thread> consumers_;
  bool stop_ = false;
  int eof_count_ = 0;
  int64_t step_buffers_ = 0;
  int step_error_ = 0;
  std::string step_error_msg_;
  double step_d2h_ms_ = 0;
  int64_t step_d2h_bytes_ = 0, step_packed_ = 0, step_raw_ = 0, step_delta_ = 0;
  int64_t step_stride_min_ = -1, step_stride_max_ = 0;
  double step_unpack_ms_ = 0;
  std::vector<bool> slot_flying_;
  int flying_ = 0;
  double step_t0_ms_ = 0, first_issue_ms_ = -1, last_landing_ms_ = -1, idle_since_ms_ = -1, eof_done_ms_ = -1;
  double step_link_idle_ms_ = 0, step_slot_wait_ms_ = 0;
  void note_issue(int k, double now);
  void note_landing(int k, double now);
  void poll_landings();
  SinkFn sink_;
  std::vector<std::unique_ptr<uint8_t[]>> eof_bufs_;
  std::vector<std::unique_ptr<uint8_t[]>> unpack_bufs_;
};

std::string nccl_unique_id();
int device_count();

hipStream_t pooled_stream(int priority = 0);
int64_t device_guard_violations();
void return_stream(hipStream_t s);
void prewarm_streams(int device, int n);

}
}
```

### csrc/gpu/device_reduce.cc

```cpp
#include "device_reduce.h"

#include <unistd.h>

#include <cstdio>
#include <cstdlib>

#include <algorithm>
#include <chrono>
#include <condition_variable>
#include <cstring>
#include <exception>
#include <map>
#include <memory>
#include <mutex>
#include <stdexcept>
#include <thread>

#include "block_decoder.h"
#include "codec/colpack.h"
#include "device_engine.h"
#include "fixed_delivery.h"
#include "hbm_ledger.h"
#include "sdma.h"
#include "uda/error.h"
// ... 224 lines not shown
 public:
  FixedDelivery(const DeviceReduceConfig& cfg, const FixedLayout& lay, FixedWs& ws, DeviceReduceStats& st,
                const FixedSink& sink)
      : lay_(lay), ws_(ws), st_(st), sink_(sink), ring_(SdmaEngine::for_device(cfg.device), lay.ring_bytes, lay.slots),
        tail_((size_t)std::max(lay.kv_buf_bytes, lay.buf_bytes) + 16), held_((size_t)lay.slots) {
    bufs_.tail = tail_.data();
    if (lay_.pack_version != 0)
      for (int i = 0; i < 2; ++i) bufs_.staging[i] = lay_.staging(ring_.p, i);
  }

  void deliver_round(int q, int64_t recs, bool last_round) {
    const int par = q & 1;
    const int S = lay_.slots;
    const int64_t bytes = recs * kTeraRecordBytes, piece = lay_.piece;
    const int64_t np = (bytes + piece - 1) / piece;
    const uint8_t* src = ws_.out[par].as<uint8_t>();
    const bool pack = lay_.pack_version != 0 && np > 0;
    const int64_t groups = (np + S - 1) / S;
    auto pack_group = [&](int64_t j) {
      const int half = (int)(j & 1);
      const int n = (int)std::min<int64_t>(S, np - j * S);
      if ((int64_t)(half * S + n) * lay_.region_bytes > (int64_t)ws_.pring.size())
        throw std::runtime_error("device reduce: a round with more pieces than its packed ring holds");
      ColpackPieceDesc* hd = ws_.h_pk->as<ColpackPieceDesc>() + half * S;
      for (int i = 0; i < n; ++i) {
        const int64_t k = j * S + i;
        hd[i] = ColpackPieceDesc{src + k * piece, ws_.pring.as<uint8_t>() + (int64_t)(half * S + i) * lay_.region_bytes,
                                 std::min(lay_.piece_recs, recs - k * lay_.piece_recs)};
      }
      ColpackPieceDesc* dd = ws_.d_pk_desc.as<ColpackPieceDesc>() + half * S;
      ColpackResult* dr = ws_.d_pk_res.as<ColpackResult>() + half * S;
      HIP_CHECK(hipMemcpyAsync(dd, hd, (size_t)n * sizeof(ColpackPieceDesc), hipMemcpyHostToDevice, ws_.ps));
      launch_colpack(dd, n, hd[0].nrec, (int)kTeraRecordBytes, lay_.buf_records, ws_.d_pk_table.as<uint32_t>(), dr, ws_.ps,
                     lay_.pack_version, kTeraKeyOffset, kTeraKeyBytes);
      HIP_CHECK(hipGetLastError());
      HIP_CHECK(hipMemcpyAsync(host_results() + half * S, dr, (size_t)n * sizeof(ColpackResult), hipMemcpyDeviceToHost, ws_.ps));
      HIP_CHECK(hipEventRecord(ws_.packed_ev[half], ws_.ps));
    };
    int64_t ready = -1;
    SdmaEngine& eng = ring_.eng;
    auto issue = [&](int64_t k) {
      const int64_t off = k * piece, len = std::min(piece, bytes - off);
      Held& h = held_[(size_t)(k % S)];
      h = Held{len, false};
      const uint8_t* from = src + off;
      if (pack) {
        const int64_t j = k / S;
        const int at = (int)(j & 1) * S + (int)(k % S);
        if (j > ready) {
          const double a = now_ms();
          HIP_CHECK(hipEventSynchronize(ws_.packed_ev[j & 1]));
          st_.pack_wait_ms += now_ms() - a;
          ready = j;
        }
        const ColpackResult pr = host_results()[at];
        if (pr.packed) {
          h = Held{lay_.packed_copy_len(pr.bytes, len / kTeraRecordBytes), true};
          from = ws_.pring.as<uint8_t>() + (int64_t)at * lay_.region_bytes;
          st_.delta_pieces += pr.delta ? 1 : 0;
        }
      }
      hsa_signal_t sg = ring_.sig[(size_t)(k % S)];
      SdmaEngine::arm(sg, eng.parts((size_t)h.copied, 1));
      eng.copy_d2h(lay_.slot(ring_.p, k), from, (size_t)h.copied, sg, 1);
      st_.d2h_bytes += h.copied;
      st_.pieces++;
      ++(h.packed ? st_.packed_pieces : st_.raw_pieces);
    };
    if (pack)
      for (int64_t j = 0; j < std::min<int64_t>(groups, 2); ++j) pack_group(j);
    for (int64_t k = 0; k < std::min<int64_t>(np, S); ++k) issue(k);
    for (int64_t k = 0; k < np; ++k) {
      const double a = now_ms();
      SdmaEngine::wait(ring_.sig[(size_t)(k % S)]);
      st_.d2h_wait_ms += now_ms() - a;
      if (pack && k % S == S - 1 && k / S + 2 < groups) pack_group(k / S + 2);
      const Held& h = held_[(size_t)(k % S)];
      FixedPiece p;
      p.base = lay_.slot(ring_.p, k);
      p.copied = h.copied;
      p.record_bytes = std::min(piece, bytes - k * piece);
      p.packed = h.packed;
      p.last = last_round && k == np - 1;
      deliver(p);
      if (k + S < np) issue(k + S);
    }
    st_.bytes += bytes;
    if (last_round && !eof_sent_) eof_only();
  }

  void eof_only() {
    FixedPiece p;
// ... 4 lines not shown
 private:
  struct Held {
    int64_t copied = 0;
    bool packed = false;
  };
  ColpackResult* host_results() const {
    return reinterpret_cast<ColpackResult*>(ws_.h_pk->as<ColpackPieceDesc>() + 2 * lay_.slots);
  }
  void deliver(const FixedPiece& p) {
    FixedDeliveryCounters c;
    c.eof_sent = eof_sent_;
    deliver_fixed_piece(p, lay_.buf_bytes, lay_.kv_buf_bytes, bufs_, sink_, &c);
    eof_sent_ = c.eof_sent;
    st_.buffers += c.buffers;
    st_.sink_ms += c.sink_ms;
    st_.unpack_ms += c.unpack_ms;
  }
  const FixedLayout lay_;
  FixedWs& ws_;
  DeviceReduceStats& st_;
  const FixedSink& sink_;
  Ring ring_;
  std::vector<uint8_t> tail_;
  std::vector<Held> held_;
  FixedBuffers bufs_;
  bool eof_sent_ = false;
};
}

int64_t fixed_round_ws_bytes(int64_t round_bytes, int runs, const DeviceReduceConfig* cfg) {
  const double slot = (double)round_bytes * 1.1 * 1.125;
  int64_t packed = 0;
  if (cfg && cfg->pack_version != 0) {
    const FixedLayout lay = fixed_layout(cfg->kv_buf_bytes, cfg->piece_bytes, cfg->pinned_slots, cfg->pack_version);
    const PackNeed n = pack_need(lay, (int64_t)((double)round_bytes * 1.1) / kTeraRecordBytes + 1);
    packed = n.ring + n.desc + n.res + n.table;
    packed += packed / 8;
  }
  return (int64_t)(2 * slot + 0.02 * (double)round_bytes) + packed + (int64_t)runs * 4096 + (16ll << 20);
}

void prewarm_device_reduce(const DeviceReduceConfig& cfg, int runs, int count) {
  HIP_CHECK(hipSetDevice(cfg.device));
  const int64_t rec = std::max<int64_t>(1, cfg.round_bytes / kTeraRecordBytes);
  const int64_t mr = rec + rec / 8;
  const FixedLayout lay = fixed_layout(cfg.kv_buf_bytes, cfg.piece_bytes, cfg.pinned_slots, cfg.pack_version);
  std::vector<std::unique_ptr<WsLease>> leases;
  std::vector<std::unique_ptr<Ring>> rings;
  for (int i = 0; i < std::max(1, count); ++i) {
    leases.push_back(std::make_unique<WsLease>(cfg.device));
    FixedWs& ws = *leases.back()->w;
    if (!ws.merger || ws.merger->max_records() < mr || ws.merger->max_runs() < runs) ws.merger.reset(new DeviceMerger(mr, runs));
    rings.push_back(std::make_unique<Ring>(SdmaEngine::for_device(cfg.device), lay.ring_bytes, lay.slots));
  }
  rings.clear();
  for (auto& l : leases) l->clean = true;
}

bool runs_are_fixed10(const std::vector<RunDesc>& runs, hipStream_t s) {
  if (runs.empty()) return true;
  int64_t max_n = 0;
  for (const auto& r : runs) {
    if (r.nbytes != r.nrec * kTeraRecordBytes) return false;
    max_n = std::max(max_n, r.nrec);
  }
  int device = 0;
  HIP_CHECK(hipGetDevice(&device));
  WsLease lease(device);
  DeviceBuffer& d_runs = lease.w->d_runs;
  DeviceBuffer& flag = lease.w->flag;
  FixedWs::ensure(d_runs, runs.size() * sizeof(RunDesc));
  FixedWs::ensure(flag, sizeof(int));
  HIP_CHECK(hipMemcpyAsync(d_runs.as(), runs.data(), runs.size() * sizeof(RunDesc), hipMemcpyHostToDevice, s));
  HIP_CHECK(hipMemsetAsync(flag.as(), 0, sizeof(int), s));
  for (size_t b = 0; b < runs.size(); b += 65535)
    launch_check_fixed(d_runs.as<RunDesc>() + b, (int)std::min<size_t>(65535, runs.size() - b), max_n, flag.as<int>(), s);
  HIP_CHECK(hipGetLastError());
  int bad = 0;
  HIP_CHECK(hipMemcpyAsync(&bad, flag.as(), sizeof(int), hipMemcpyDeviceToHost, s));
  HIP_CHECK(hipStreamSynchronize(s));
  lease.clean = true;
  return bad == 0;
}

DeviceReduceStats device_reduce_fixed(const DeviceReduceConfig& cfg, const std::vector<RunDesc>& runs,
                                      const std::function<int(const uint8_t*, int64_t)>& sink) {
  trace::Range tr("uda.device_reduce");
  HIP_CHECK(hipSetDevice(cfg.device));
  if (const hipError_t pending = hipGetLastError(); pending != hipSuccess)
    throw std::runtime_error(std::string("device reduce: HIP error pending on entry: ") + hipGetErrorString(pending));
  DeviceReduceStats st;
  const double t0 = now_ms();
  const int K = (int)runs.size();
  if (K > 65536) throw std::runtime_error("device reduce: more than 65536 runs");
  int64_t N = 0;
  for (const auto& r : runs) N += r.nrec;
  WsLease lease(cfg.device, N * kTeraRecordBytes);
  FixedWs& ws = *lease.w;
  hipStream_t s = ws.s;
  const FixedLayout lay = fixed_layout(cfg.kv_buf_bytes, cfg.piece_bytes, cfg.pinned_slots, cfg.pack_version);
  if (N == 0) {
    const uint8_t eof[2] = {0xFF, 0xFF};
    const double a = now_ms();
    if (sink(eof, kEofBytes) != 0) throw std::runtime_error("dataFromUda callback failed");
    st.sink_ms += now_ms() - a;
    st.buffers++;
    lease.clean = true;
    return st;
  }

  HbmLedger& led = HbmLedger::get();
  int64_t round_bytes = std::max<int64_t>(cfg.round_bytes, kTeraRecordBytes);
  const bool caller_reserved = led.bound() != nullptr && led.bound()->device() == cfg.device;
  std::unique_ptr<HbmLedger::Reservation> res;
  if (!caller_reserved) {
    auto need = [&](int64_t rb) {
      const int64_t r = std::min(rb, N * kTeraRecordBytes), slot = (int64_t)((double)r * 1.1);
      return FixedWs::grow(ws.out[0], slot) + FixedWs::grow(ws.out[1], slot) +
             pack_grow(ws, lay, slot / kTeraRecordBytes + 1) + (int64_t)(0.02 * (double)r) + (int64_t)K * 4096 + (16ll << 20);
    };
    const int64_t hr = led.headroom(cfg.device);
    while (round_bytes > (64ll << 20) && need(round_bytes) > hr) round_bytes /= 2;
    res = led.reserve(cfg.device, need(round_bytes), cfg.stop);
    st.hbm_wait_ms = res->wait_ms();
    st.hbm_reserved = res->granted();
  }
  st.round_bytes = round_bytes;
  const int Q = (int)std::max<int64_t>(1, (N * kTeraRecordBytes + round_bytes - 1) / round_bytes);
  std::vector<int64_t> pos((size_t)K * (Q + 1), 0);
  {
    std::vector<uint8_t*> bases(K);
    std::vector<int64_t> nrec(K);
    for (int k = 0; k < K; ++k) {
// ... 177 lines not shown
    HIP_CHECK(hipMemcpyAsync(keys.data(), ws.d_keys.as(), (size_t)NB * sizeof(Elem), hipMemcpyDeviceToHost, s));
    HIP_CHECK(hipMemcpyAsync(flags, ws.flag.as(), sizeof(flags), hipMemcpyDeviceToHost, s));
  }
  HIP_CHECK(hipStreamSynchronize(s));
  if (flags[0]) throw UdaError("corrupt compressed block in a map output partition");
  if (flags[1]) {
    lease.clean = true;
    return st;
  }
  std::vector<std::vector<std::pair<int64_t, Elem>>> idx(K);
  std::vector<Elem> samp;
  for (int k = 0; k < K; ++k)
    for (int64_t b = blk0[k]; b < blk0[k + 1]; ++b)
      if (first[(size_t)b] >= 0) {
        if (!idx[k].empty() && key_less(keys[(size_t)b], idx[k].back().second)) {
          lease.clean = true;
          return st;
        }
        idx[k].emplace_back(b, keys[(size_t)b]);
        samp.push_back(keys[(size_t)b]);
      }
  std::sort(samp.begin(), samp.end(), key_less);
  *streamed = true;
  auto emit_eof_only = [&] {
    uint8_t eof[2] = {0xFF, 0xFF};
    if (sink(eof, kEofBytes) != 0) throw std::runtime_error("dataFromUda callback failed");
    st.buffers++;
  };
  if (N == 0) {
    emit_eof_only();
    lease.clean = true;
    return st;
  }
  const FixedLayout lay = fixed_layout(cfg.kv_buf_bytes, cfg.piece_bytes, cfg.pinned_slots, cfg.pack_version);
  HbmLedger& led = HbmLedger::get();
  int64_t round_bytes = std::max<int64_t>(cfg.round_bytes, kTeraRecordBytes);
  struct Span {
    int64_t b0 = 0, b1 = -1;
    int64_t rec0 = 0, rec1 = 0;
    int64_t in_off = 0;
  };
  int Q = 1;
  std::vector<Elem> bounds;
  std::vector<std::vector<Span>> spans;
  std::vector<int64_t> in_bytes, in_recs;
  auto plan_rounds = [&](int64_t rb) {
    Q = (int)std::max<int64_t>(1, (N * kTeraRecordBytes + rb - 1) / rb);
    bounds.assign((size_t)std::max(0, Q - 1), Elem{0, 0});
    for (int q = 1; q < Q; ++q) bounds[(size_t)q - 1] = samp.empty() ? Elem{~0ull, ~0ull} : samp[samp.size() * (size_t)q / (size_t)Q];
    spans.assign((size_t)Q, std::vector<Span>((size_t)K));
    in_bytes.assign((size_t)Q, 0);
    in_recs.assign((size_t)Q, 0);
    for (int q = 0; q < Q; ++q) {
      int64_t cur = 0;
      for (int k = 0; k < K; ++k) {
        Span& sp = spans[(size_t)q][(size_t)k];
        if (nrec[k] == 0 || blk0[k] == blk0[k + 1]) continue;
        const auto& ix = idx[k];
        sp.b0 = blk0[k];
        if (q > 0) {
          const Elem lo = bounds[(size_t)q - 1];
          auto it = std::lower_bound(ix.begin(), ix.end(), lo, [](const std::pair<int64_t, Elem>& a, const Elem& v) {
            return key_less(a.second, v);
          });
          if (it != ix.begin()) sp.b0 = std::prev(it)->first;
        }
        sp.b1 = blk0[k + 1] - 1;
// ... 216 lines not shown
```

### csrc/gpu/device_reduce.h

```cpp
#pragma once
#include <hip/hip_runtime.h>

#include <cstdint>
#include <functional>
#include <string>
#include <vector>

#include "kernels.h"

namespace uda {
namespace gpu {

struct DeviceReduceConfig {
  int device = 0;
  int64_t kv_buf_bytes = 1 << 20;
  int64_t round_bytes = 2ll << 30;
  int64_t piece_bytes = 64ll << 20;
  int pinned_slots = 4;
  int pack_version = 0;
  int64_t sample_every = 4096;
  std::function<bool()> stop;
  std::function<bool()> decode_turn;
  std::function<void()> decode_done;
};

struct DeviceReduceStats {
  int64_t records = 0;
  int64_t bytes = 0;
  int64_t buffers = 0;
  int rounds = 0;
  int merge_passes = 0;
  double plan_ms = 0, merge_wait_ms = 0, d2h_wait_ms = 0, sink_ms = 0;
  double hbm_wait_ms = 0;
  double decode_wait_ms = 0;
  int64_t hbm_reserved = 0;
  int64_t round_bytes = 0;
  int64_t decoded_blocks = 0;
  int64_t d2h_bytes = 0;
  int64_t pieces = 0;
  int64_t packed_pieces = 0;
  int64_t raw_pieces = 0;
  int64_t delta_pieces = 0;
  double unpack_ms = 0;
  double pack_wait_ms = 0;
};

void prewarm_device_reduce(const DeviceReduceConfig& cfg, int runs, int count = 1);

int64_t fixed_round_ws_bytes(int64_t round_bytes, int runs, const DeviceReduceConfig* cfg = nullptr);

bool runs_are_fixed10(const std::vector<RunDesc>& runs, hipStream_t s);

DeviceReduceStats device_reduce_fixed(const DeviceReduceConfig& cfg, const std::vector<RunDesc>& runs,
                                      const std::function<int(const uint8_t*, int64_t)>& sink);

struct BlockPlan;
DeviceReduceStats device_reduce_fixed_blocks(const DeviceReduceConfig& cfg, int codec, const BlockPlan& plan,
                                             const std::function<int(const uint8_t*, int64_t)>& sink,
                                             bool* streamed);

}
}
```

### csrc/gpu/fixed_delivery.cc

```cpp
#include "fixed_delivery.h"

#include <algorithm>
#include <chrono>
#include <cstdlib>
#include <cstring>
#include <stdexcept>

#include "codec/colpack.h"

namespace uda {
namespace gpu {

namespace {
double now_ms() {
  return std::chrono::duration<double, std::milli>(std::chrono::steady_clock::now().time_since_epoch()).count();
}
int64_t align64(int64_t v) { return (v + 63) / 64 * 64; }
}

int delivery_pack_version(const std::string& value) {
  int v;
  if (value == "auto")
    v = (int)kColpackVersion2;
  else if (value == "v1")
    v = (int)kColpackVersion;
  else if (value == "off")
    v = 0;
  else
    return -1;
  if (const char* e = std::getenv("UDA_DELIVERY_PACK"))
    if (std::atoi(e) == 0) v = 0;
  return v;
}

int64_t FixedLayout::piece_bound(int64_t nrec) const {
  return pack_version == (int)kColpackVersion ? colpack_bound(kFixedRecordBytes, nrec)
                                              : colpack2_bound(kFixedRecordBytes, nrec, buf_records);
}

int64_t FixedLayout::packed_copy_len(int64_t packed_bytes, int64_t nrec) const {
  if (packed_bytes < (int64_t)kColpackHeaderBytes || packed_bytes > piece_bound(nrec) || packed_bytes > slot_bytes)
    throw std::runtime_error("fixed delivery: packed length outside the piece's region");
  return packed_bytes;
}

FixedLayout fixed_layout(int64_t kv_buf_bytes, int64_t piece_bytes, int pinned_slots, int pack_version) {
  FixedLayout l;
  l.pack_version = pack_version;
  l.slots = std::max(2, pinned_slots);
  l.kv_buf_bytes = kv_buf_bytes;
  l.buf_records = std::max<int64_t>(1, kv_buf_bytes / kFixedRecordBytes);
  l.buf_bytes = l.buf_records * kFixedRecordBytes;
  l.piece = std::max<int64_t>(1, piece_bytes / l.buf_bytes) * l.buf_bytes;
  l.piece_recs = l.piece / kFixedRecordBytes;
  l.slot_bytes = l.piece;
  if (pack_version != 0) {
    l.region_bytes = align64(l.piece_bound(l.piece_recs));
    l.slot_bytes = std::max(align64(l.piece), l.region_bytes);
    l.staging_bytes = align64(std::max(kv_buf_bytes, l.buf_bytes) + 16);
  }
  l.ring_bytes = (size_t)(l.slots * l.slot_bytes + 2 * l.staging_bytes);
  return l;
}

void deliver_fixed_piece(const FixedPiece& p, int64_t buf_bytes, int64_t kv_buf_bytes, FixedBuffers& bufs,
                         const FixedSink& sink, FixedDeliveryCounters* c) {
  if (buf_bytes < kFixedRecordBytes || buf_bytes % kFixedRecordBytes || p.record_bytes < 0 ||
      p.record_bytes % kFixedRecordBytes)
    throw std::runtime_error("fixed delivery: a piece or buffer that does not hold whole records");
  ColpackPiece pp;
  if (p.packed) {
    const char* why = "";
    if (!colpack_open(p.base, p.copied, (int)kFixedRecordBytes, p.record_bytes / kFixedRecordBytes, &pp, &why))
      throw std::runtime_error(std::string("packed piece rejected: ") + why);
    if (!pp.packed) throw std::runtime_error("packed piece rejected: not marked packed");
  } else if (p.copied != p.record_bytes) {
    throw std::runtime_error("fixed delivery: an unpacked piece of another length than its records");
  }
  const bool drop = !sink;
  auto emit = [&](const uint8_t* b, int64_t len) {
    if (!drop) {
// ... 36 lines not shown
```

### csrc/gpu/fixed_delivery.h

```cpp
#pragma once
#include <cstddef>
#include <cstdint>
#include <functional>
#include <string>

namespace uda {
namespace gpu {

constexpr int64_t kFixedRecordBytes = 104;
constexpr int64_t kFixedEofBytes = 2;

int delivery_pack_version(const std::string& value);

struct FixedLayout {
  int pack_version = 0;
  int slots = 2;
  int64_t kv_buf_bytes = 0;
  int64_t buf_records = 1, buf_bytes = kFixedRecordBytes;
  int64_t piece = 0, piece_recs = 0;
  int64_t slot_bytes = 0;
  int64_t region_bytes = 0;
  int64_t staging_bytes = 0;
  size_t ring_bytes = 0;
  int64_t piece_bound(int64_t nrec) const;
  int64_t packed_copy_len(int64_t packed_bytes, int64_t nrec) const;
  uint8_t* slot(uint8_t* ring, int64_t k) const { return ring + (k % slots) * slot_bytes; }
  uint8_t* staging(uint8_t* ring, int i) const { return ring + (int64_t)slots * slot_bytes + (i & 1) * staging_bytes; }
};
FixedLayout fixed_layout(int64_t kv_buf_bytes, int64_t piece_bytes, int pinned_slots, int pack_version);

struct FixedPiece {
  const uint8_t* base = nullptr;
  int64_t copied = 0;
  int64_t record_bytes = 0;
  bool packed = false;
  bool last = false;
};
struct FixedBuffers {
  uint8_t* staging[2] = {nullptr, nullptr};
  uint8_t* tail = nullptr;
  int64_t turn = 0;
};
struct FixedDeliveryCounters {
  int64_t buffers = 0;
  double unpack_ms = 0, sink_ms = 0;
  bool eof_sent = false;
};
using FixedSink = std::function<int(const uint8_t*, int64_t)>;

void deliver_fixed_piece(const FixedPiece& p, int64_t buf_bytes, int64_t kv_buf_bytes, FixedBuffers& bufs,
                         const FixedSink& sink, FixedDeliveryCounters* c);

}
}
```

### csrc/gpu/kernels.h

```cpp
#pragma once
#include "uda/hash.h"
#include <hip/hip_runtime.h>

#include <cstdint>

namespace uda {
enum class CombineOp : int;
namespace gpu {

struct alignas(16) Elem {
  uint64_t hi;
  uint64_t lo;
};

constexpr int kTeraKeyBytes = 10;
constexpr int kTeraValBytes = 90;
constexpr int kTeraRecordBytes = 104;
constexpr int kTeraKeyOffset = 3;

struct RunDesc {
  const uint8_t* base;
  int64_t nrec;
  int64_t nbytes;
  const int64_t* offsets;
// ... 117 lines not shown

constexpr int kCombineTile = 256;
void launch_combine_heads(GenericKeyCtx ctx, const Elem* order, int64_t n, CombineOp op, int64_t* heads,
                          unsigned long long* bad, hipStream_t s);
void launch_combine_check_values(GenericKeyCtx ctx, int64_t n, CombineOp op, int* any_bad, hipStream_t s);
void launch_combine_round_heads(GenericKeyCtx ctx, const Elem* order, int64_t i0, int64_t i1, int64_t* heads,
                                unsigned long long* last_head, hipStream_t s);
void launch_combine_sums(GenericKeyCtx ctx, const Elem* order, const int64_t* gidx, int64_t n, CombineOp op,
                         unsigned long long* sums, int64_t* sizes, hipStream_t s);
void launch_gather_combine(GenericKeyCtx ctx, const Elem* elems, int64_t n, const int64_t* gidx,
                           const int64_t* out_off, const unsigned long long* sums, CombineOp op, uint8_t* out,
                           hipStream_t s);

void launch_gather_fixed(const Elem* elems, int64_t n, uint8_t* const* run_bases, uint8_t* out,
                         hipStream_t s);

struct CopyDesc {
  const uint8_t* src;
  uint8_t* dst;
  int64_t bytes;
};
void launch_batched_copy(const CopyDesc* descs, int n, int64_t max_bytes, hipStream_t s, int max_blocks = 2048);

struct ColpackPieceDesc {
  const uint8_t* src;
  uint8_t* dst;
  int64_t nrec;
};
struct ColpackResult {
  int64_t bytes;
  uint32_t packed;
  uint32_t stride;
  uint32_t delta;
  uint32_t reserved;
};
size_t colpack_table_bytes(int npieces);
void launch_colpack(const ColpackPieceDesc* pieces, int npieces, int64_t max_nrec, int L, int64_t buf_records,
                    uint32_t* table, ColpackResult* results, hipStream_t s, int version = 1, int key_off = 0,
                    int key_len = 0);

struct DecodeDesc {
  int64_t src;
  int64_t src_end;
  int64_t dst;
  int64_t raw;
};
void launch_block_decode(int codec, const uint8_t* in, uint8_t* out, const DecodeDesc* descs, int n, int* status,
                         hipStream_t s, int64_t clip = 0);
constexpr int64_t kDecodePrefixSlot = 128;
struct DecodeGeometry {
  int reg_window, reg_align, lds_window, lds_align, short_copy, vec_bytes, wave_step, lane_word, waves_per_block,
      prefix_slot;
};
DecodeGeometry decode_geometry();
bool lzo_lane_decode_host(const uint8_t* in, int64_t n, uint8_t* out, int64_t out_cap, int64_t* out_len);
void launch_frame_streams(const uint8_t* const* ptrs, const int64_t* lens, int nstreams, int codec,
                          const int64_t* desc_first, const int64_t* raw_first, int64_t* nblocks, int64_t* raw,
                          DecodeDesc* out, int* status, hipStream_t s, int* tails = nullptr);

struct CrcDesc {
  const uint8_t* p;
  int64_t len;
};
int64_t crc32_chunk_bytes();
size_t crc32_ws_bytes(int64_t total_chunks);
int64_t crc32_chunk_plan(const CrcDesc* descs, int n, int64_t* chunk_first);
void launch_crc32(const CrcDesc* descs, int n, const int64_t* chunk_first, int64_t total_chunks, void* ws,
                  uint32_t* out, hipStream_t s);
void launch_crc32_trailers(const CrcDesc* descs, int n, uint32_t* stored, hipStream_t s);

void launch_validate_fixed(const uint8_t* recs, int64_t n, const Elem* prev_key, int has_prev,
                           Elem* last_key, unsigned long long* stats, hipStream_t s,
// ... 13 lines not shown
```

### csrc/python/bindings.cc

```cpp
#include <map>
#include <memory>
#include <condition_variable>
#include <mutex>
#include <pybind11/functional.h>
#include <pybind11/numpy.h>
#include <pybind11/pybind11.h>
#include <pybind11/stl.h>

#include <fcntl.h>
#include <unistd.h>

#include <atomic>
#include <chrono>
#include <cstring>
#include <random>

#include "block_decoder.h"
#include "device_engine.h"
#include "device_ptr.h"
#include "device_reduce.h"
#include "fixed_delivery.h"
#include "mof_cache.h"
#include "consumer/reduce_task.h"
#include "service/merge_service.h"
// ... 24 lines not shown
#include <thread>

namespace py = pybind11;
using namespace uda;

namespace {

struct GpuNoise {
  std::atomic<bool> stop{false};
  std::thread thr;
  std::atomic<int64_t> ops{0};
};
GpuNoise* g_noise = nullptr;

py::dict stats_to_dict(const gpu::StepStats& s) {
  py::dict d;
  d["wall_ms"] = s.wall_ms;
  d["comm_ms"] = s.comm_ms;
  d["plan_ms"] = s.plan_ms;
  d["merge_ms"] = s.merge_ms;
  d["d2h_ms"] = s.d2h_ms;
  d["wait_out_ms"] = s.wait_out_ms;
  d["stage_ms"] = s.stage_ms;
  d["bytes_in"] = s.bytes_in;
  d["records"] = s.records;
  d["bytes_sent"] = s.bytes_sent;
  d["bytes_h2d"] = s.bytes_h2d;
  d["buffers"] = s.buffers;
  d["d2h_bytes"] = s.d2h_bytes;
  d["packed_pieces"] = s.packed_pieces;
  d["pack_delta_pieces"] = s.pack_delta_pieces;
  d["pack_stride_min"] = s.pack_stride_min;
  d["pack_stride_max"] = s.pack_stride_max;
  d["raw_pieces"] = s.raw_pieces;
  d["unpack_ms"] = s.unpack_ms;
  d["lead_in_ms"] = s.lead_in_ms;
  d["link_idle_ms"] = s.link_idle_ms;
  d["tail_ms"] = s.tail_ms;
  d["slot_wait_ms"] = s.slot_wait_ms;
  d["merge_passes"] = s.merge_passes;
  d["order_errors"] = s.order_errors;
  d["checksum"] = s.checksum;
  d["exchange_errors"] = s.exchange_errors;
  d["validated"] = s.validated;
  d["bad_layout"] = s.bad_layout;
  d["pre_merge_errors"] = s.pre_merge_errors;
  d["own_errors"] = s.own_errors;
  d["merge_errors"] = s.merge_errors;
  d["pre_d2h_errors"] = s.pre_d2h_errors;
  d["delivery_errors"] = s.delivery_errors;
  d["diag"] = s.diag;
  d["round_comm_ms"] = s.round_comm_ms;
  d["round_merge_ms"] = s.round_merge_ms;
  return d;
}

gpu::ShuffleConfig config_from_dict(const py::dict& d) {
  gpu::ShuffleConfig c;
  auto get = [&](const char* k, auto& field) {
    if (d.contains(k)) field = d[k].cast<std::decay_t<decltype(field)>>();
  };
  get("device", c.device);
  get("rank", c.rank);
  get("world", c.world);
  get("maps_per_rank", c.maps_per_rank);
  get("records_per_map", c.records_per_map);
// ... 264 lines not shown
      d["reducer"] = p.reducer;
      d["src_off"] = p.src_off;
      d["len"] = p.len;
      d["pack_index"] = p.pack_index;
      d["last_of_reducer"] = p.last_of_reducer;
      out.append(d);
    }
    return out;
  }, py::arg("group_recs"), py::arg("piece_bytes"), py::arg("order") = "wave", py::arg("record_bytes") = 104);
  m.def("colpack_header_bytes", [] { return (int64_t)kColpackHeaderBytes; });
  m.def("colpack_have_bmi2", &colpack_have_bmi2);
  m.def("colpack_encode", [](py::bytes b, int L, int64_t buf_records) {
    std::string s = b;
    if (L < 1 || L > kColpackMaxRecordBytes || s.empty() || s.size() % (size_t)L)
      throw py::value_error("colpack_encode: need whole records of 1..256 bytes");
    const int64_t nrec = (int64_t)s.size() / L;
    std::string out((size_t)colpack_bound(L, nrec), '\0');
    const int64_t n = colpack_encode((const uint8_t*)s.data(), nrec, L, buf_records, (uint8_t*)&out[0]);
    out.resize((size_t)n);
    return py::bytes(out);
  }, py::arg("records"), py::arg("record_bytes"), py::arg("buf_records") = 1);
  m.def("colpack2_encode", [](py::bytes b, int L, int64_t buf_records, int key_off, int key_len) {
    std::string s = b;
    if (L < 1 || L > kColpackMaxRecordBytes || s.empty() || s.size() % (size_t)L)
      throw py::value_error("colpack2_encode: need whole records of 1..256 bytes");
    if (key_off < 0 || key_len < 0 || key_len > kColpackMaxKeyBytes || key_off + key_len > L)
      throw py::value_error("colpack2_encode: key field outside the record or longer than 16 bytes");
    const int64_t nrec = (int64_t)s.size() / L;
    std::string out((size_t)colpack2_bound(L, nrec, buf_records), '\0');
    const int64_t n = colpack2_encode((const uint8_t*)s.data(), nrec, L, buf_records, key_off, key_len, (uint8_t*)&out[0]);
    out.resize((size_t)n);
    return py::bytes(out);
  }, py::arg("records"), py::arg("record_bytes"), py::arg("buf_records"), py::arg("key_off"), py::arg("key_len"));
  m.def("colpack_decode", [](py::bytes b, int expect_L, int64_t expect_records, const std::string& path, int64_t row0,
                             int64_t rows) {
    std::string s = b;
    ColpackPiece p;
    const char* why = "";
    if (!colpack_open((const uint8_t*)s.data(), (int64_t)s.size(), expect_L, expect_records, &p, &why))
      throw py::value_error(std::string("colpack: ") + why);
    if (!p.packed) throw py::value_error("colpack: raw piece");
    if (rows < 0) rows = p.records - row0;
    if (row0 < 0 || rows < 0 || row0 + rows > p.records) throw py::value_error("colpack: rows out of range");
    std::string out((size_t)(rows * p.L), '\0');
    if (path == "bmi2") {
      if (!colpack_unpack_bmi2(p, row0, rows, (uint8_t*)&out[0])) throw std::runtime_error("no BMI2 on this CPU");
    } else if (path == "scalar") {
      colpack_unpack_scalar(p, row0, rows, (uint8_t*)&out[0]);
    } else {
      colpack_unpack(p, row0, rows, (uint8_t*)&out[0]);
    }
    return py::bytes(out);
  }, py::arg("piece"), py::arg("expect_record_bytes") = 0, py::arg("expect_records") = 0, py::arg("path") = "auto",
     py::arg("row0") = 0, py::arg("rows") = -1);
  auto gpu_encode = [](const std::vector<std::string>& pieces, int L, int64_t buf_records, int device, int version,
                       int key_off, int key_len) {
    if (L < 1 || L > kColpackMaxRecordBytes || pieces.empty()) throw py::value_error("gpu_colpack_encode: bad arguments");
    if (key_off < 0 || key_len < 0 || key_len > kColpackMaxKeyBytes || key_off + key_len > L)
      throw py::value_error("gpu_colpack_encode: key field outside the record or longer than 16 bytes");
    auto bound = [&](int64_t n) { return version == 2 ? colpack2_bound(L, n, buf_records) : colpack_bound(L, n); };
    std::vector<int64_t> src_off, dst_off, nrec;
    int64_t src_bytes = 0, dst_bytes = 0, max_nrec = 0;
    for (const auto& s : pieces) {
      if (s.empty() || s.size() % (size_t)L) throw py::value_error("gpu_colpack_encode: need whole records");
      src_off.push_back(src_bytes);
      dst_off.push_back(dst_bytes);
      nrec.push_back((int64_t)s.size() / L);
      max_nrec = std::max(max_nrec, nrec.back());
      src_bytes += ((int64_t)s.size() + 7) / 8 * 8;
      dst_bytes += bound(nrec.back());
    }
    const int n = (int)pieces.size();
    std::vector<gpu::ColpackResult> res((size_t)n);
    std::vector<std::string> out((size_t)n);
    {
      py::gil_scoped_release rel;
      HIP_CHECK(hipSetDevice(device));
      gpu::DeviceBuffer dsrc, ddst, ddesc, dtab, dres;
      dsrc.alloc((size_t)src_bytes);
      ddst.alloc((size_t)dst_bytes);
      ddesc.alloc((size_t)n * sizeof(gpu::ColpackPieceDesc));
      dtab.alloc(gpu::colpack_table_bytes(n));
      dres.alloc((size_t)n * sizeof(gpu::ColpackResult));
      std::vector<gpu::ColpackPieceDesc> descs;
      for (int i = 0; i < n; ++i) {
        HIP_CHECK(hipMemcpy(dsrc.as<uint8_t>() + src_off[i], pieces[i].data(), pieces[i].size(), hipMemcpyHostToDevice));
        descs.push_back(gpu::ColpackPieceDesc{dsrc.as<uint8_t>() + src_off[i], ddst.as<uint8_t>() + dst_off[i], nrec[i]});
      }
      HIP_CHECK(hipMemset(ddst.as(), 0xEE, (size_t)dst_bytes));
      HIP_CHECK(hipMemcpy(ddesc.as(), descs.data(), descs.size() * sizeof(descs[0]), hipMemcpyHostToDevice));
      hipStream_t s = nullptr;
      HIP_CHECK(hipStreamCreateWithFlags(&s, hipStreamNonBlocking));
      gpu::launch_colpack(ddesc.as<gpu::ColpackPieceDesc>(), n, max_nrec, L, buf_records, dtab.as<uint32_t>(),
                          dres.as<gpu::ColpackResult>(), s, version, key_off, key_len);
      HIP_CHECK(hipGetLastError());
      HIP_CHECK(hipStreamSynchronize(s));
      HIP_CHECK(hipStreamDestroy(s));
      HIP_CHECK(hipMemcpy(res.data(), dres.as(), res.size() * sizeof(res[0]), hipMemcpyDeviceToHost));
      for (int i = 0; i < n; ++i) {
        if (res[(size_t)i].bytes < 0 || res[(size_t)i].bytes > bound(nrec[i]))
          throw std::runtime_error("gpu_colpack_encode: a piece's length is outside its region");
        out[(size_t)i].resize((size_t)res[(size_t)i].bytes);
        HIP_CHECK(hipMemcpy(&out[(size_t)i][0], ddst.as<uint8_t>() + dst_off[i], out[(size_t)i].size(), hipMemcpyDeviceToHost));
      }
    }
    py::list ret;
    for (int i = 0; i < n; ++i)
      ret.append(py::make_tuple(py::bytes(out[(size_t)i]), res[(size_t)i].packed != 0, (int64_t)res[(size_t)i].stride));
    return ret;
  };
  m.def("gpu_colpack_encode", [gpu_encode](const std::vector<std::string>& pieces, int L, int64_t buf_records, int device) {
    return gpu_encode(pieces, L, buf_records, device, 1, 0, 0);
  }, py::arg("pieces"), py::arg("record_bytes"), py::arg("buf_records") = 1, py::arg("device") = 0);
  m.def("gpu_colpack2_encode", [gpu_encode](const std::vector<std::string>& pieces, int L, int64_t buf_records,
                                            int key_off, int key_len, int device) {
    return gpu_encode(pieces, L, buf_records, device, 2, key_off, key_len);
  }, py::arg("pieces"), py::arg("record_bytes"), py::arg("buf_records"), py::arg("key_off"), py::arg("key_len"),
     py::arg("device") = 0);
  m.def("fixed_delivery_piece", [](py::bytes piece, int64_t record_bytes, int64_t buf_bytes, int64_t kv_buf, bool packed,
                                   bool last, bool deliver) -> py::object {
    std::string s = piece;
    if (kv_buf < 1 || buf_bytes < 1) throw py::value_error("fixed_delivery_piece: bad buffer sizes");
    const size_t one = (size_t)std::max(kv_buf, buf_bytes) + 16;
    std::vector<uint8_t> stg(2 * one), tail(one);
    gpu::FixedBuffers bufs;
    bufs.staging[0] = stg.data();
    bufs.staging[1] = stg.data() + one;
    bufs.tail = tail.data();
    gpu::FixedPiece p;
    p.base = (const uint8_t*)s.data();
    p.copied = (int64_t)s.size();
    p.record_bytes = record_bytes;
    p.packed = packed;
    p.last = last;
    std::vector<std::string> out;
    gpu::FixedDeliveryCounters c;
    gpu::FixedSink sink;
    if (deliver)
      sink = [&](const uint8_t* b, int64_t len) {
        out.emplace_back((const char*)b, (size_t)len);
        return 0;
      };
    gpu::deliver_fixed_piece(p, buf_bytes, kv_buf, bufs, sink, &c);
    if (!deliver) {
      py::dict d;
      d["buffers"] = c.buffers;
      d["eof_sent"] = c.eof_sent;
      d["unpack_ms"] = c.unpack_ms;
      return d;
    }
    py::list ret;
    for (const auto& b : out) ret.append(py::bytes(b));
    return ret;
  }, py::arg("piece"), py::arg("record_bytes"), py::arg("buf_bytes"), py::arg("kv_buf"), py::arg("packed"), py::arg("last"),
     py::arg("deliver") = true);
  m.def("delivery_pack_version", &gpu::delivery_pack_version);
  m.def("fixed_delivery_packed_copy_len", [](int64_t kv_buf, int64_t piece_bytes, int pinned_slots, int pack_version,
                                             int64_t packed_bytes, int64_t nrec) {
    return gpu::fixed_layout(kv_buf, piece_bytes, pinned_slots, pack_version).packed_copy_len(packed_bytes, nrec);
  });
  m.def("fixed_delivery_layout", [](int64_t kv_buf, int64_t piece_bytes, int pinned_slots, int pack_version) {
    const gpu::FixedLayout l = gpu::fixed_layout(kv_buf, piece_bytes, pinned_slots, pack_version);
    py::dict d;
    d["buf_records"] = l.buf_records;
    d["piece"] = l.piece;
    d["slots"] = l.slots;
    d["slot_bytes"] = l.slot_bytes;
    d["region_bytes"] = l.region_bytes;
    d["staging_bytes"] = l.staging_bytes;
    d["ring_bytes"] = (int64_t)l.ring_bytes;
    d["bound_full"] = pack_version ? l.piece_bound(l.piece_recs) : 0;
    return d;
  });
  m.def("gpu_device_reduce_fixed", [](const std::vector<std::string>& runs, int64_t kv_buf, int64_t round_bytes,
                                      int64_t piece_bytes, const std::string& pack, int device) {
    gpu::DeviceReduceConfig cfg;
    cfg.device = device;
    cfg.kv_buf_bytes = kv_buf;
    cfg.round_bytes = round_bytes;
    cfg.piece_bytes = piece_bytes;
    cfg.sample_every = 16;
    cfg.pack_version = gpu::delivery_pack_version(pack);
    if (cfg.pack_version < 0) throw py::value_error("gpu_device_reduce_fixed: pack is auto, v1 or off");
    if (kv_buf < 1 || round_bytes < 1 || piece_bytes < 1) throw py::value_error("gpu_device_reduce_fixed: bad sizes");
    for (const auto& r : runs)
      if (r.size() % (size_t)gpu::kTeraRecordBytes) throw py::value_error("gpu_device_reduce_fixed: need whole records");
    std::vector<std::string> out;
    gpu::DeviceReduceStats st;
    {
      py::gil_scoped_release rel;
      HIP_CHECK(hipSetDevice(device));
      std::vector<gpu::DeviceBuffer> dev(runs.size());
      std::vector<gpu::RunDesc> rd(runs.size());
      for (size_t i = 0; i < runs.size(); ++i) {
        dev[i].alloc(std::max<size_t>(runs[i].size(), 16));
        if (!runs[i].empty()) HIP_CHECK(hipMemcpy(dev[i].as(), runs[i].data(), runs[i].size(), hipMemcpyHostToDevice));
        rd[i].base = dev[i].as<uint8_t>();
        rd[i].nbytes = (int64_t)runs[i].size();
        rd[i].nrec = rd[i].nbytes / gpu::kTeraRecordBytes;
        rd[i].offsets = nullptr;
      }
      st = gpu::device_reduce_fixed(cfg, rd, [&](const uint8_t* b, int64_t len) {
        out.emplace_back((const char*)b, (size_t)len);
        return 0;
      });
    }
    py::list bufs;
    for (const auto& b : out) bufs.append(py::bytes(b));
    py::dict d;
    d["records"] = st.records;
    d["bytes"] = st.bytes;
    d["buffers"] = st.buffers;
    d["rounds"] = st.rounds;
    d["round_bytes"] = st.round_bytes;
    d["hbm_reserved"] = st.hbm_reserved;
    d["d2h_bytes"] = st.d2h_bytes;
    d["pieces"] = st.pieces;
    d["packed_pieces"] = st.packed_pieces;
    d["raw_pieces"] = st.raw_pieces;
    d["delta_pieces"] = st.delta_pieces;
    d["unpack_ms"] = st.unpack_ms;
    d["pack_wait_ms"] = st.pack_wait_ms;
    d["d2h_wait_ms"] = st.d2h_wait_ms;
    d["sink_ms"] = st.sink_ms;
    return py::make_tuple(bufs, d);
  }, py::arg("runs"), py::arg("kv_buf"), py::arg("round_bytes"), py::arg("piece_bytes") = 64ll << 20,
     py::arg("pack") = "auto", py::arg("device") = 0);
  m.def("gpu_merge_fixed", [](const py::list& runs, const py::object& group_first, int device, int pad) {
    if (pad != 0 && pad != 8 && pad != 2) throw py::value_error("gpu_merge_fixed: pad is 0, 8 or 2");
    const int K = (int)runs.size();
    std::vector<std::string> host((size_t)K);
    std::vector<size_t> at((size_t)K);
    size_t in_bytes = 0;
    int64_t total = 0;
    for (int i = 0; i < K; ++i) {
      py::buffer_info v = py::cast<py::buffer>(runs[i]).request();
      host[i].assign((const char*)v.ptr, (size_t)(v.size * v.itemsize));
      if (host[i].size() % (size_t)gpu::kTeraRecordBytes) throw py::value_error("gpu_merge_fixed: need whole records");
      at[i] = ((in_bytes + 15) & ~(size_t)15) + (size_t)pad;
      in_bytes = at[i] + host[i].size();
      total += (int64_t)(host[i].size() / (size_t)gpu::kTeraRecordBytes);
    }
    std::vector<int> gf = group_first.is_none() ? std::vector<int>{0, K} : group_first.cast<std::vector<int>>();
    for (size_t g = 0; g + 1 < gf.size(); ++g)
      if (gf[g] > gf[g + 1]) throw py::value_error("gpu_merge_fixed: group_first must not decrease");
    const int64_t out_bytes = total * gpu::kTeraRecordBytes;
    PyObject* o = PyBytes_FromStringAndSize(nullptr, (Py_ssize_t)out_bytes);
    if (!o) throw py::error_already_set();
    py::bytes out = py::reinterpret_steal<py::bytes>(o);
    int passes = 0, overflow = 0;
    bool bad = false, kway = false;
    {
      py::gil_scoped_release rel;
// ... 1495 lines not shown
```

Measured before the change: 91.87.

## Add mixed-radix column packing for colpack v2 pieces with AVX2 decoder

Adds a radix variant of colpack v2 that packs groups of four byte columns as mixed-radix numbers, using each column's exact value range instead of rounding it to a power-of-two width. Rows become fewer bits, which shrinks the device-to-host bytes moved during the shuffle. It adds a GPU encode path, a scalar decoder and an AVX2 decoder, plus header validation. In exchange, decode needs divisions by multiply-shift, which costs more CPU than plain bit extraction. Whether it runs by default depends on how the pack setting resolves.

```diff
diff --git a/csrc/apps/colpack_bench_main.cc b/csrc/apps/colpack_bench_main.cc
--- a/csrc/apps/colpack_bench_main.cc
+++ b/csrc/apps/colpack_bench_main.cc
@@ -36,7 +36,7 @@
 
 struct Result {
   double unpack = 0, unpack_copy = 0, copy = 0;
-  int64_t stride = 0;
+  int64_t stride = 0, row_bits = 0;
 };
 
 }
@@ -44,7 +44,7 @@
 int main(int argc, char** argv) {
   int threads = 1, reps = 3;
   int64_t mib = 128;
-  bool scalar = false, v2 = false;
+  bool scalar = false, v2 = false, radix = false;
   for (int i = 1; i < argc; ++i) {
     const std::string a = argv[i];
     if (a == "--threads" && i + 1 < argc) threads = std::atoi(argv[++i]);
@@ -52,8 +52,9 @@
     else if (a == "--reps" && i + 1 < argc) reps = std::atoi(argv[++i]);
     else if (a == "--scalar") scalar = true;
     else if (a == "--v2") v2 = true;
+    else if (a == "--radix") v2 = radix = true;
     else {
-      std::fprintf(stderr, "usage: uda_colpack_bench [--threads N] [--mib M] [--reps R] [--scalar] [--v2]\n");
+      std::fprintf(stderr, "usage: uda_colpack_bench [--threads N] [--mib M] [--reps R] [--scalar] [--v2] [--radix]\n");
       return 2;
     }
   }
@@ -68,11 +69,13 @@
       std::vector<uint8_t> raw((size_t)(n * 104));
       fill(raw, n, 1234567 + (uint64_t)t, v2 ? (1ull << 38) - 1 : 0xFFFFFF);
       std::vector<uint8_t> piece((size_t)(v2 ? uda::colpack2_bound(104, n, buf_records) : uda::colpack_bound(104, n)));
-      const int64_t len = v2 ? uda::colpack2_encode(raw.data(), n, 104, buf_records, 3, 10, piece.data())
-                             : uda::colpack_encode(raw.data(), n, 104, buf_records, piece.data());
+      const int64_t len = radix ? uda::colpack2r_encode(raw.data(), n, 104, buf_records, 3, 10, piece.data())
+                          : v2  ? uda::colpack2_encode(raw.data(), n, 104, buf_records, 3, 10, piece.data())
+                                : uda::colpack_encode(raw.data(), n, 104, buf_records, piece.data());
       uda::ColpackPiece p;
-      if (!uda::colpack_open(piece.data(), len, 104, n, &p) || !p.packed || p.delta != v2) return;
+      if (!uda::colpack_open(piece.data(), len, 104, n, &p) || !p.packed || p.delta != v2 || p.radix != radix) return;
       res[(size_t)t].stride = p.stride;
+      res[(size_t)t].row_bits = p.row_bits;
       std::vector<uint8_t> stg((size_t)(buf_records * 104) * 2), kv((size_t)(buf_records * 104));
       auto pass = [&](int mode) {
         double best = 0;
@@ -107,9 +110,9 @@
     }
     u += r.unpack, uc += r.unpack_copy, c += r.copy;
   }
-  std::printf("{\"threads\": %d, \"mib_per_thread\": %lld, \"version\": %d, \"stride\": %lld, \"bmi2\": %s, \"path\": \"%s\", "
+  std::printf("{\"threads\": %d, \"mib_per_thread\": %lld, \"version\": %d, \"radix\": %s, \"stride\": %lld, \"row_bits\": %lld, \"bmi2\": %s, \"path\": \"%s\", "
               "\"unpack_GBps_per_thread\": %.2f, \"unpack_copy_GBps_per_thread\": %.2f, \"copy_GBps_per_thread\": %.2f}\n",
-              threads, (long long)mib, v2 ? 2 : 1, (long long)res[0].stride, uda::colpack_have_bmi2() ? "true" : "false",
+              threads, (long long)mib, v2 ? 2 : 1, radix ? "true" : "false", (long long)res[0].stride, (long long)res[0].row_bits, uda::colpack_have_bmi2() ? "true" : "false",
               scalar || !uda::colpack_have_bmi2() ? "scalar" : "bmi2", u / threads / 1e9, uc / threads / 1e9,
               c / threads / 1e9);
   return 0;
diff --git a/csrc/codec/colpack.cc b/csrc/codec/colpack.cc
--- a/csrc/codec/colpack.cc
+++ b/csrc/codec/colpack.cc
@@ -119,8 +119,121 @@
   }
 };
 
+struct Half {
+  int cols = 0, bits = 0;
+  bool radix = false;
+  uint32_t n[4] = {1, 1, 1, 1};
+  uint8_t mn[4] = {0, 0, 0, 0};
+};
+struct RadixLayout {
+  int L = 0, groups = 0;
+  int64_t row_bits = 0;
+  int bo[kColpackMaxGroups], bits[kColpackMaxGroups], cols[kColpackMaxGroups];
+  Half half[kColpackMaxGroups][2];
+};
+
+RadixLayout radix_layout_of(const ColpackHeader& h, const uint8_t* ranges, int L) {
+  RadixLayout rl;
+  rl.L = L;
+  rl.groups = colpack_groups(L);
+  int cur = 0;
+  for (int g = 0; g < rl.groups; ++g) {
+    rl.cols[g] = L - 8 * g < 8 ? L - 8 * g : 8;
+    for (int k = 0; k < 2; ++k) {
+      Half& hf = rl.half[g][k];
+      const int c0 = 8 * g + 4 * k;
+      hf.cols = L - c0 < 0 ? 0 : (L - c0 < 4 ? L - c0 : 4);
+      if (hf.cols == 4) (void)colpack2r_quad(ranges + c0, &hf.radix);
+      uint64_t prod = 1;
+      int w = 0;
+      for (int c = 0; c < hf.cols; ++c) {
+        const int wc = bit_length(ranges[c0 + c]);
+        hf.n[c] = hf.radix ? (uint32_t)ranges[c0 + c] + 1 : 1u << wc;
+        hf.mn[c] = (uint8_t)(h.base[g] >> (8 * (4 * k + c)));
+        prod *= hf.n[c];
+        w += wc;
+      }
+      hf.bits = hf.radix ? 64 - __builtin_clzll(prod - 1) : w;
+    }
+    rl.bits[g] = rl.half[g][0].bits + rl.half[g][1].bits;
+    rl.bo[g] = cur;
+    cur += rl.bits[g];
+  }
+  rl.row_bits = cur;
+  return rl;
+}
+
+inline uint64_t low_bits(int n) { return n >= 64 ? ~0ull : ((1ull << n) - 1); }
+
+inline uint64_t get_bits(const uint8_t* base, int64_t pos, int n) {
+  if (n == 0) return 0;
+  const uint8_t* p = base + (pos >> 3);
+  const int sh = (int)(pos & 7), nb = (sh + n + 7) / 8;
+  u128 x = 0;
+  for (int k = 0; k < nb; ++k) x |= (u128)p[k] << (8 * k);
+  return (uint64_t)(x >> sh) & low_bits(n);
+}
+
+inline void put_bits(uint8_t* base, int64_t pos, int n, uint64_t word) {
+  if (n == 0) return;
+  uint8_t* p = base + (pos >> 3);
+  const int sh = (int)(pos & 7), nb = (sh + n + 7) / 8;
+  const u128 x = (u128)word << sh;
+  for (int k = 0; k < nb; ++k) p[k] |= (uint8_t)(x >> (8 * k));
+}
+
+void radix_decode_row(const RadixLayout& rl, const uint8_t* rows, int64_t r, uint8_t* rec) {
+  const int64_t rowbit = r * rl.row_bits;
+  for (int g = 0; g < rl.groups; ++g) {
+    const uint64_t word = get_bits(rows, rowbit + rl.bo[g], rl.bits[g]);
+    for (int k = 0; k < 2; ++k) {
+      const Half& hf = rl.half[g][k];
+      uint64_t f = k == 0 ? word & low_bits(hf.bits) : (rl.half[g][0].bits >= 64 ? 0 : word >> rl.half[g][0].bits);
+      for (int c = 0; c < hf.cols; ++c) {
+        rec[8 * g + 4 * k + c] = (uint8_t)(f % hf.n[c] + hf.mn[c]);
+        f /= hf.n[c];
+      }
+    }
+  }
+}
+
+void radix_encode_row(const RadixLayout& rl, uint8_t* rows, int64_t r, const uint8_t* rec) {
+  const int64_t rowbit = r * rl.row_bits;
+  for (int g = 0; g < rl.groups; ++g) {
+    uint64_t word = 0;
+    for (int k = 1; k >= 0; --k) {
+      const Half& hf = rl.half[g][k];
+      uint64_t f = 0, mult = 1;
+      for (int c = 0; c < hf.cols; ++c) {
+        f += (uint64_t)(uint8_t)(rec[8 * g + 4 * k + c] - hf.mn[c]) * mult;
+        mult *= hf.n[c];
+      }
+      word = k == 1 ? f : ((rl.half[g][0].bits >= 64 ? 0 : word << rl.half[g][0].bits) | f);
+    }
+    put_bits(rows, rowbit + rl.bo[g], rl.bits[g], word);
+  }
+}
+
+void radix_key_start(KeyWalk& kw, const ColpackPiece& p, const RadixLayout& rl, int64_t row0) {
+  kw.table = p.table;
+  kw.buf_records = p.buf_records;
+  kw.key_off = p.key_off;
+  kw.key_len = p.key_len;
+  kw.mask = key_mask(p.key_len);
+  const int64_t rs = row0 - row0 % p.buf_records;
+  kw.next_restart = rs;
+  if (rs == row0) return;
+  kw.sum = load_be(p.table + rs / p.buf_records * kColpackRestartBytes, p.key_len);
+  uint8_t rec[kColpackMaxRecordBytes];
+  for (int64_t r = rs + 1; r < row0; ++r) {
+    radix_decode_row(rl, p.rows, r, rec);
+    kw.sum = (kw.sum + load_be(rec + p.key_off, p.key_len)) & kw.mask;
+  }
+  kw.next_restart = rs + p.buf_records;
+}
+
 int64_t encode(const uint8_t* src, int64_t nrec, int L, int64_t buf_records, uint32_t version, int key_off,
-               int key_len, uint8_t* dst) {
+               int key_len, uint8_t* dst, bool allow_radix = false) {
   if (L < 1 || L > kColpackMaxRecordBytes || nrec < 1) return 0;
   if (key_off < 0 || key_len < 0 || key_len > kColpackMaxKeyBytes || key_off + key_len > L) return 0;
   uint8_t mn[kColpackMaxRecordBytes], mx[kColpackMaxRecordBytes];
@@ -186,6 +299,44 @@
     bits[g] = b;
   }
   const bool v1 = version == kColpackVersion;
+  if (allow_radix && !v1) {
+    uint8_t ranges[kColpackMaxRecordBytes];
+    for (int c = 0; c < L; ++c) ranges[c] = (uint8_t)(mx[c] - mn[c]);
+    int rbits[kColpackMaxGroups];
+    uint64_t bitmap = 0;
+    const int row_bits = colpack2r_layout(ranges, L, rbits, bo, &bitmap);
+    const int64_t table_bytes = delta ? colpack2_table_bytes(nrec, buf_records) : 0;
+    if (colpack2r_choose(bitmap, row_bits, nrec, L, buf_records, table_bytes)) {
+      for (int g = 0; g < G; ++g) h.bo[g] = bo[g];
+      h.stride = (uint32_t)((row_bits + 7) / 8);
+      h.flags = kColpackFlagPacked | (delta ? kColpackFlagDelta : 0) | kColpackFlagRadix;
+      h.reserved[0] = (uint32_t)bitmap;
+      h.reserved[1] = (uint32_t)(bitmap >> 32);
+      h.reserved[2] = (uint32_t)row_bits;
+      const int64_t total = colpack2r_packed_bytes(row_bits, nrec, L, table_bytes);
+      std::memcpy(dst, &h, sizeof(h));
+      std::memset(dst + kColpackHeaderBytes, 0, (size_t)(total - (int64_t)kColpackHeaderBytes));
+      std::memcpy(dst + kColpackHeaderBytes, ranges, (size_t)L);
+      uint8_t* tab = dst + kColpackHeaderBytes + colpack2r_range_bytes(L);
+      if (delta)
+        for (int64_t b = 0; b * buf_records < nrec; ++b)
+          std::memcpy(tab + b * kColpackRestartBytes, src + b * buf_records * L + key_off, (size_t)key_len);
+      const RadixLayout rl = radix_layout_of(h, ranges, L);
+      uint8_t* rows = tab + table_bytes;
+      prev = 0;
+      for (int64_t r = 0; r < nrec; ++r) {
+        uint8_t rec[kColpackMaxRecordBytes];
+        std::memcpy(rec, src + r * L, (size_t)L);
+        if (delta) {
+          const u128 k = load_be(rec + key_off, key_len);
+          store_be(rec + key_off, key_len, r % buf_records == 0 ? (u128)0 : (k - prev) & kmask);
+          prev = k;
+        }
+        radix_encode_row(rl, rows, r, rec);
+      }
+      return total;
+    }
+  }
   const int64_t S = colpack_layout(bits, G, v1, bo);
   for (int g = 0; g < G; ++g) {
     if (v1)
@@ -239,6 +390,13 @@
   if (key_off < 0 || key_len < 0 || key_len > kColpackMaxKeyBytes || key_off + key_len > L) return 0;
   if (buf_records < 1 || buf_records > 0xFFFFFFFFll) key_len = 0;
   return encode(src, nrec, L, buf_records, kColpackVersion2, key_len > 0 ? key_off : 0, key_len, dst);
+}
+
+int64_t colpack2r_encode(const uint8_t* src, int64_t nrec, int L, int64_t buf_records, int key_off, int key_len,
+                         uint8_t* dst) {
+  if (key_off < 0 || key_len < 0 || key_len > kColpackMaxKeyBytes || key_off + key_len > L) return 0;
+  if (buf_records < 1 || buf_records > 0xFFFFFFFFll) key_len = 0;
+  return encode(src, nrec, L, buf_records, kColpackVersion2, key_len > 0 ? key_off : 0, key_len, dst, true);
 }
 
 bool colpack_open(const uint8_t* piece, int64_t len, int expect_L, int64_t expect_records, ColpackPiece* out,
@@ -273,7 +431,27 @@
     }
     if (v1 && hc.gb[g] != (bits[g] + 7) / 8) return fail("group size does not match its widths");
   }
-  const int64_t S = colpack_layout(bits, G, v1, bo);
+  const bool radix = !v1 && (hc.flags & kColpackFlagRadix) != 0;
+  int64_t row_bits = 0;
+  if (radix) {
+    const uint64_t bitmap = (uint64_t)hc.reserved[0] | ((uint64_t)hc.reserved[1] << 32);
+    if (bitmap == 0) return fail("radix piece without a radix quad");
+    for (int q = 0; q < 64; ++q)
+      if (((bitmap >> q) & 1) && 4 * q + 4 > L) return fail("radix bit on a partial quad");
+    if (len < (int64_t)kColpackHeaderBytes + colpack2r_range_bytes(L)) return fail("piece shorter than its range table");
+    const uint8_t* ranges = piece + kColpackHeaderBytes;
+    for (int c = 0; c < (int)colpack2r_range_bytes(L); ++c) {
+      const unsigned m = c < L ? (unsigned)((hc.mask[c / 8] >> (8 * (c % 8))) & 0xFF) : 0u;
+      if (c >= L ? ranges[c] != 0 : m != (1u << bit_length(ranges[c])) - 1)
+        return fail("range table does not match the masks");
+    }
+    uint64_t bm = 0;
+    row_bits = colpack2r_layout(ranges, L, bits, bo, &bm);
+    if (bm != bitmap) return fail("radix bitmap does not match the ranges");
+    if ((int64_t)hc.reserved[2] != row_bits || hc.reserved[3] || hc.reserved[4]) return fail("row bits do not match the ranges");
+    if (!(hc.flags & kColpackFlagPacked)) return fail("radix piece that is not packed");
+  }
+  const int64_t S = radix ? (row_bits + 7) / 8 : colpack_layout(bits, G, v1, bo);
   if (!v1)
     for (int g = 0; g < kColpackMaxGroups; ++g)
       if (hc.bo[g] != (g < G ? bo[g] : 0)) return fail("group offsets do not match the masks");
@@ -282,7 +460,7 @@
   const bool delta = !v1 && (hc.flags & kColpackFlagDelta) != 0;
   int64_t table_bytes = 0;
   if (!v1) {
-    if (hc.flags & ~(kColpackFlagPacked | kColpackFlagDelta)) return fail("unknown flags");
+    if (hc.flags & ~(kColpackFlagPacked | kColpackFlagDelta | kColpackFlagRadix)) return fail("unknown flags");
     if (hc.key_len > (uint32_t)kColpackMaxKeyBytes || hc.key_off > (uint32_t)L || hc.key_off + hc.key_len > (uint32_t)L)
       return fail("key field outside the record");
     if (delta && hc.key_len == 0) return fail("delta piece without a key");
@@ -291,13 +469,21 @@
   }
   if (packed) {
     if (colpack_is_raw(S, L)) return fail("packed piece with a raw stride");
-    const int64_t need = v1 ? colpack_packed_bytes(S, (int64_t)hc.records)
-                            : colpack2_packed_bytes(S, (int64_t)hc.records, table_bytes);
+    const int64_t need = v1      ? colpack_packed_bytes(S, (int64_t)hc.records)
+                         : radix ? colpack2r_packed_bytes(row_bits, (int64_t)hc.records, L, table_bytes)
+                                 : colpack2_packed_bytes(S, (int64_t)hc.records, table_bytes);
     if (need > len) return fail(v1 ? "rows exceed the piece's length" : "table and rows exceed the piece's length");
   }
+  if (!radix)
+    for (int k = 0; k < 5; ++k)
+      if (hc.reserved[k]) return fail("reserved header words are not zero");
+  const int64_t range_bytes = radix ? colpack2r_range_bytes(L) : 0;
   out->hdr = h;
-  out->table = piece + kColpackHeaderBytes;
-  out->rows = piece + kColpackHeaderBytes + table_bytes;
+  out->ranges = radix ? piece + kColpackHeaderBytes : nullptr;
+  out->table = piece + kColpackHeaderBytes + range_bytes;
+  out->rows = piece + kColpackHeaderBytes + range_bytes + table_bytes;
+  out->radix = radix;
+  out->row_bits = radix ? row_bits : 8 * S;
   out->L = L;
   out->version = (int)hc.version;
   out->records = (int64_t)hc.records;
@@ -314,6 +500,16 @@
   if (row0 < 0 || rows <= 0 || row0 + rows > p.records) return;
   ColpackHeader h;
   std::memcpy(&h, p.hdr, sizeof(h));
+  if (p.radix) {
+    const RadixLayout rl = radix_layout_of(h, p.ranges, p.L);
+    KeyWalk kw;
+    if (p.delta) radix_key_start(kw, p, rl, row0);
+    for (int64_t r = 0; r < rows; ++r) {
+      radix_decode_row(rl, p.rows, row0 + r, dst + r * p.L);
+      if (p.delta) kw.fix(row0 + r, dst + r * p.L);
+    }
+    return;
+  }
   const Layout lo = layout_of(h, p.L);
   KeyWalk kw;
   if (p.delta) kw.start(p, h, lo, row0);
@@ -374,9 +570,152 @@
 }
 #endif
 
+#if defined(__x86_64__)
+namespace {
+constexpr int kRadixBlocks = kColpackMaxGroups / 4;
+struct RadixSimdPlan {
+  int npdep = 0, nblocks = 0, tail_group = -1;
+  int pg[kColpackMaxGroups];
+  bool wide[kColpackMaxGroups];
+  int vg[kRadixBlocks][4], cnt[kRadixBlocks];
+  int off[8][kRadixBlocks][4];
+  alignas(32) uint64_t sh[8][kRadixBlocks][2][4];
+  alignas(32) uint64_t fm[kRadixBlocks][2][4];
+  alignas(32) uint64_t m1[kRadixBlocks][2][4], k1[kRadixBlocks][2][4], d1[kRadixBlocks][2][4];
+  alignas(32) uint16_t p2[kRadixBlocks][16], m2[kRadixBlocks][16], c2[kRadixBlocks][16];
+  alignas(32) uint8_t base[kRadixBlocks][32];
+};
+
+bool radix_simd_plan(const RadixLayout& rl, RadixSimdPlan* sp) {
+  int vg[kColpackMaxGroups], nv = 0;
+  for (int g = 0; g < rl.groups; ++g) {
+    sp->wide[g] = rl.bits[g] > 57;
+    if (rl.cols[g] < 8) sp->tail_group = g;
+    if (!rl.half[g][0].radix && !rl.half[g][1].radix) {
+      sp->pg[sp->npdep++] = g;
+      continue;
+    }
+    if (rl.bits[g] > 57) return false;
+    vg[nv++] = g;
+  }
+  sp->nblocks = (nv + 3) / 4;
+  for (int j = 0; j < sp->nblocks; ++j) {
+    sp->cnt[j] = nv - 4 * j < 4 ? nv - 4 * j : 4;
+    for (int s = 0; s < 4; ++s) {
+      const int g = vg[4 * j + (s < sp->cnt[j] ? s : sp->cnt[j] - 1)];
+      sp->vg[j][s] = g;
+      const int word0 = s == 0 ? 0 : s == 1 ? 8 : s == 2 ? 4 : 12;
+      for (int k = 0; k < 2; ++k) {
+        const Half& hf = rl.half[g][k];
+        const int v = s >> 1, lane = 2 * (s & 1) + k;
+        const uint64_t d1 = (uint64_t)hf.n[0] * hf.n[1];
+        const bool pow2 = (d1 & (d1 - 1)) == 0;
+        const int k1 = pow2 ? __builtin_ctzll(d1) : hf.bits + bit_length((unsigned)d1);
+        if (!pow2 && hf.bits > 30) return false;
+        sp->fm[j][v][lane] = low_bits(hf.bits);
+        sp->d1[j][v][lane] = d1;
+        sp->k1[j][v][lane] = (uint64_t)k1;
+        sp->m1[j][v][lane] = pow2 ? 1 : (1ull << k1) / d1 + 1;
+        for (int ph = 0; ph < 8; ++ph) {
+          sp->off[ph][j][s] = (ph + rl.bo[g]) >> 3;
+          sp->sh[ph][j][v][lane] = (uint64_t)(((ph + rl.bo[g]) & 7) + (k ? rl.half[g][0].bits : 0));
+        }
+        for (int t = 0; t < 2; ++t) {
+          const uint64_t n = hf.n[2 * t], xmax = n * hf.n[2 * t + 1] - 1;
+          const uint64_t m2 = n == 1 ? 32768 : (65536 + n - 1) / n;
+          if (n > 1 && xmax * (m2 * n - 65536) >= 65536) return false;
+          const int w = word0 + 2 * k + t;
+          sp->p2[j][w] = n == 1 ? 2 : 1;
+          sp->m2[j][w] = (uint16_t)m2;
+          sp->c2[j][w] = (uint16_t)(256 - n);
+          sp->base[j][2 * w] = hf.mn[2 * t];
+          sp->base[j][2 * w + 1] = hf.mn[2 * t + 1];
+        }
+      }
+    }
+  }
+  return true;
+}
+
+__attribute__((target("avx2"))) inline __m256i radix_level1(const RadixSimdPlan& sp, const uint8_t* row, int ph, int j, int v) {
+  const __m128i wa = _mm_broadcastq_epi64(_mm_loadl_epi64((const __m128i_u*)(row + sp.off[ph][j][2 * v])));
+  const __m128i wb = _mm_broadcastq_epi64(_mm_loadl_epi64((const __m128i_u*)(row + sp.off[ph][j][2 * v + 1])));
+  __m256i f = _mm256_inserti128_si256(_mm256_castsi128_si256(wa), wb, 1);
+  f = _mm256_and_si256(_mm256_srlv_epi64(f, *(const __m256i*)sp.sh[ph][j][v]), *(const __m256i*)sp.fm[j][v]);
+  const __m256i hi = _mm256_srlv_epi64(_mm256_mul_epu32(f, *(const __m256i*)sp.m1[j][v]), *(const __m256i*)sp.k1[j][v]);
+  const __m256i lo = _mm256_sub_epi64(f, _mm256_mul_epu32(hi, *(const __m256i*)sp.d1[j][v]));
+  return _mm256_or_si256(lo, _mm256_slli_epi64(hi, 32));
+}
+
+template <bool kDelta>
+__attribute__((target("avx2,bmi2"))) void unpack_radix_avx2(const ColpackPiece& p, const ColpackHeader& h,
+                                                            const RadixLayout& rl, const RadixSimdPlan& sp, int64_t row0,
+                                                            int64_t rows, uint8_t* dst) {
+  const int L = p.L;
+  KeyWalk kw;
+  if (kDelta) radix_key_start(kw, p, rl, row0);
+  auto store = [&](uint8_t* rec, int g, uint64_t x) {
+    if (g == sp.tail_group)
+      std::memcpy(rec + 8 * g, &x, (size_t)rl.cols[g]);
+    else
+      std::memcpy(rec + 8 * g, &x, 8);
+  };
+  int64_t rowbit = row0 * rl.row_bits;
+  for (int64_t r = 0; r < rows; ++r, rowbit += rl.row_bits, dst += L) {
+    const uint8_t* row = p.rows + (rowbit >> 3);
+    const int ph = (int)(rowbit & 7);
+    for (int i = 0; i < sp.npdep; ++i) {
+      const int g = sp.pg[i];
+      const int pos = ph + rl.bo[g];
+      uint64_t x;
+      std::memcpy(&x, row + (pos >> 3), 8);
+      x >>= pos & 7;
+      if (sp.wide[g] && (pos & 7)) {
+        uint64_t y;
+        std::memcpy(&y, row + (pos >> 3) + 8, 8);
+        x |= y << (64 - (pos & 7));
+      }
+      store(dst, g, _pdep_u64(x, h.mask[g]) + h.base[g]);
+    }
+    for (int j = 0; j < sp.nblocks; ++j) {
+      const __m256i x = _mm256_packus_epi32(radix_level1(sp, row, ph, j, 0), radix_level1(sp, row, ph, j, 1));
+      const __m256i q = _mm256_mulhi_epu16(_mm256_mullo_epi16(x, *(const __m256i*)sp.p2[j]), *(const __m256i*)sp.m2[j]);
+      const __m256i digits = _mm256_add_epi16(x, _mm256_mullo_epi16(q, *(const __m256i*)sp.c2[j]));
+      const __m256i out = _mm256_add_epi8(digits, *(const __m256i*)sp.base[j]);
+      const __m128i ac = _mm256_castsi256_si128(out), bd = _mm256_extracti128_si256(out, 1);
+      const int n = sp.cnt[j];
+      store(dst, sp.vg[j][0], (uint64_t)_mm_cvtsi128_si64(ac));
+      if (n > 1) store(dst, sp.vg[j][1], (uint64_t)_mm_cvtsi128_si64(bd));
+      if (n > 2) store(dst, sp.vg[j][2], (uint64_t)_mm_extract_epi64(ac, 1));
+      if (n > 3) store(dst, sp.vg[j][3], (uint64_t)_mm_extract_epi64(bd, 1));
+    }
+    if (kDelta) kw.fix(row0 + r, dst);
+  }
+}
+}
+#endif
+
+bool colpack_unpack_radix_simd(const ColpackPiece& p, int64_t row0, int64_t rows, uint8_t* dst) {
+#if defined(__x86_64__)
+  static const bool have = __builtin_cpu_supports("avx2") && __builtin_cpu_supports("bmi2");
+  if (!have || !p.radix) return false;
+  ColpackHeader h;
+  std::memcpy(&h, p.hdr, sizeof(h));
+  const RadixLayout rl = radix_layout_of(h, p.ranges, p.L);
+  RadixSimdPlan sp;
+  if (!radix_simd_plan(rl, &sp)) return false;
+  if (row0 < 0 || rows <= 0 || row0 + rows > p.records) return true;
+  p.delta ? unpack_radix_avx2<true>(p, h, rl, sp, row0, rows, dst) : unpack_radix_avx2<false>(p, h, rl, sp, row0, rows, dst);
+  return true;
+#else
+  return false;
+#endif
+}
+
 bool colpack_unpack_bmi2(const ColpackPiece& p, int64_t row0, int64_t rows, uint8_t* dst) {
 #if defined(__x86_64__)
   if (!colpack_have_bmi2()) return false;
+  if (p.radix) return colpack_unpack_radix_simd(p, row0, rows, dst);
   if (row0 < 0 || rows <= 0 || row0 + rows > p.records) return true;
   if (p.L == 104)
     p.delta ? unpack_bmi2<13, true>(p, row0, rows, dst) : unpack_bmi2<13, false>(p, row0, rows, dst);
diff --git a/csrc/codec/colpack.h b/csrc/codec/colpack.h
--- a/csrc/codec/colpack.h
+++ b/csrc/codec/colpack.h
@@ -17,6 +17,7 @@
 constexpr int kColpackMaxGroups = kColpackMaxRecordBytes / 8;
 constexpr uint32_t kColpackFlagPacked = 1;
 constexpr uint32_t kColpackFlagDelta = 2;
+constexpr uint32_t kColpackFlagRadix = 4;
 constexpr int kColpackMaxKeyBytes = 16;
 constexpr int kColpackRestartBytes = 16;
 
@@ -85,9 +86,58 @@
   return delta_key_bits * nrec + 128 * entries < plain_key_bits * nrec;
 }
 
+UDA_COLPACK_HD int64_t colpack2r_range_bytes(int64_t L) { return (L + 63) / 64 * 64; }
+UDA_COLPACK_HD int64_t colpack2r_packed_bytes(int64_t row_bits, int64_t nrec, int64_t L, int64_t table_bytes) {
+  return ((int64_t)kColpackHeaderBytes + colpack2r_range_bytes(L) + table_bytes + (row_bits * nrec + 7) / 8 + 16 + 63) /
+         64 * 64;
+}
+UDA_COLPACK_HD int colpack2r_quad(const uint8_t* range, bool* radix) {
+  uint64_t prod = 1;
+  int w = 0;
+  for (int c = 0; c < 4; ++c) {
+    prod *= (uint64_t)range[c] + 1;
+    for (unsigned v = range[c]; v; v >>= 1) ++w;
+  }
+  int rb = 0;
+  for (uint64_t v = prod - 1; v; v >>= 1) ++rb;
+  *radix = rb < w;
+  return rb < w ? rb : w;
+}
+UDA_COLPACK_HD int colpack2r_layout(const uint8_t* range, int L, int* bits, uint16_t* bo, uint64_t* bitmap) {
+  const int G = colpack_groups(L);
+  int cur = 0;
+  uint64_t bm = 0;
+  for (int g = 0; g < G; ++g) {
+    int b = 0;
+    for (int h = 0; h < 2; ++h) {
+      const int c0 = 8 * g + 4 * h;
+      if (c0 + 4 <= L) {
+        bool rx;
+        b += colpack2r_quad(range + c0, &rx);
+        if (rx) bm |= (uint64_t)1 << (2 * g + h);
+      } else {
+        for (int c = c0; c < L; ++c)
+          for (unsigned v = range[c]; v; v >>= 1) ++b;
+      }
+    }
+    bits[g] = b;
+    bo[g] = (uint16_t)cur;
+    cur += b;
+  }
+  *bitmap = bm;
+  return cur;
+}
+UDA_COLPACK_HD bool colpack2r_choose(uint64_t bitmap, int row_bits, int64_t nrec, int64_t L, int64_t buf_records,
+                                     int64_t table_bytes) {
+  return bitmap != 0 && !colpack_is_raw((row_bits + 7) / 8, L) &&
+         colpack2r_packed_bytes(row_bits, nrec, L, table_bytes) <= colpack2_bound(L, nrec, buf_records);
+}
+
 int64_t colpack_encode(const uint8_t* src, int64_t nrec, int L, int64_t buf_records, uint8_t* dst);
 int64_t colpack2_encode(const uint8_t* src, int64_t nrec, int L, int64_t buf_records, int key_off, int key_len,
                         uint8_t* dst);
+int64_t colpack2r_encode(const uint8_t* src, int64_t nrec, int L, int64_t buf_records, int key_off, int key_len,
+                         uint8_t* dst);
 
 struct ColpackPiece {
   const ColpackHeader* hdr = nullptr;
@@ -101,6 +151,9 @@
   int key_off = 0, key_len = 0;
   bool packed = false;
   bool delta = false;
+  bool radix = false;
+  int64_t row_bits = 0;
+  const uint8_t* ranges = nullptr;
 };
 bool colpack_open(const uint8_t* piece, int64_t len, int expect_L, int64_t expect_records, ColpackPiece* out,
                   const char** why = nullptr);
@@ -109,5 +162,6 @@
 void colpack_unpack_scalar(const ColpackPiece& p, int64_t row0, int64_t rows, uint8_t* dst);
 bool colpack_unpack_bmi2(const ColpackPiece& p, int64_t row0, int64_t rows, uint8_t* dst);
 bool colpack_have_bmi2();
+bool colpack_unpack_radix_simd(const ColpackPiece& p, int64_t row0, int64_t rows, uint8_t* dst);
 
 }
diff --git a/csrc/consumer/gpu_merge_device.cc b/csrc/consumer/gpu_merge_device.cc
--- a/csrc/consumer/gpu_merge_device.cc
+++ b/csrc/consumer/gpu_merge_device.cc
@@ -535,6 +535,7 @@
       cfg.kv_buf_bytes = kv_buf_size_;
       cfg.round_bytes = round_bytes;
       cfg.pack_version = delivery_pack_;
+      cfg.pack_radix = delivery_pack_radix_;
       cfg.piece_bytes = delivery_piece_bytes_;
       cfg.stop = [&] { return stop_.load(); };
       if (const int slots = (int)host_->conf_i64("mapred.uda.gpu.decode.stream.slots", 3); slots > 0) {
@@ -573,6 +574,7 @@
       gpu::DeviceReduceConfig pcfg;
       pcfg.kv_buf_bytes = kv_buf_size_;
       pcfg.pack_version = delivery_pack_;
+      pcfg.pack_radix = delivery_pack_radix_;
       pcfg.piece_bytes = delivery_piece_bytes_;
       admit(std::max<int64_t>(0, raw + raw / 8 - (int64_t)ws.in.held()), [&](int64_t rb) {
         return gpu::fixed_round_ws_bytes(std::min(rb, raw), (int)parts.size(), &pcfg);
@@ -648,6 +650,7 @@
     cfg.kv_buf_bytes = kv_buf_size_;
     cfg.round_bytes = round_bytes;
     cfg.pack_version = delivery_pack_;
+    cfg.pack_radix = delivery_pack_radix_;
     cfg.piece_bytes = delivery_piece_bytes_;
     cfg.stop = [&] { return stop_.load(); };
     gpu::DeviceReduceStats ds = gpu::device_reduce_fixed(cfg, runs, sink);
diff --git a/csrc/consumer/gpu_prewarm.cc b/csrc/consumer/gpu_prewarm.cc
--- a/csrc/consumer/gpu_prewarm.cc
+++ b/csrc/consumer/gpu_prewarm.cc
@@ -61,6 +61,7 @@
   cfg.kv_buf_bytes = kv_buf;
   cfg.round_bytes = round_bytes;
   cfg.pack_version = std::max(0, gpu::delivery_pack_version("auto"));
+  cfg.pack_radix = gpu::delivery_pack_radix("auto");
   gpu::prewarm_device_reduce(cfg, std::max(1, maps), tasks);
 }
 
@@ -102,6 +103,7 @@
       cfg.kv_buf_bytes = kv_buf_size_;
       cfg.round_bytes = pc.round_bytes;
       cfg.pack_version = pc.delivery_pack;
+      cfg.pack_radix = pc.delivery_pack_radix;
       cfg.piece_bytes = pc.delivery_piece_bytes;
       gpu::prewarm_device_reduce(cfg, std::max(1, pc.maps));
     }
diff --git a/csrc/consumer/reduce_task.cc b/csrc/consumer/reduce_task.cc
--- a/csrc/consumer/reduce_task.cc
+++ b/csrc/consumer/reduce_task.cc
@@ -528,7 +528,8 @@
   if (backend_ == "gpu") {
     const std::string pack = host_->get_conf("mapred.uda.gpu.delivery.pack", "auto");
     delivery_pack_ = gpu::delivery_pack_version(pack);
-    if (delivery_pack_ < 0) throw ProtocolError("unknown mapred.uda.gpu.delivery.pack \"" + pack + "\" (auto, v1 or off)");
+    if (delivery_pack_ < 0) throw ProtocolError("unknown mapred.uda.gpu.delivery.pack \"" + pack + "\" (auto, v2, v1 or off)");
+    delivery_pack_radix_ = gpu::delivery_pack_radix(pack);
     delivery_piece_bytes_ = host_->conf_i64("mapred.uda.gpu.delivery.piece.bytes", 64ll << 20);
     if (delivery_piece_bytes_ < 1)
       throw ProtocolError("mapred.uda.gpu.delivery.piece.bytes must be positive, got " + std::to_string(delivery_piece_bytes_));
@@ -564,6 +565,7 @@
     pc.round_bytes = host_->conf_i64("mapred.uda.gpu.round.bytes", 2ll << 30);
     pc.maps = p.num_maps;
     pc.delivery_pack = delivery_pack_;
+    pc.delivery_pack_radix = delivery_pack_radix_;
     pc.delivery_piece_bytes = delivery_piece_bytes_;
     prewarm_thr_ = std::thread([this, pc] { name_thread("uda-task-warm"); prewarm_gpu(pc); });
   }
diff --git a/csrc/consumer/reduce_task.h b/csrc/consumer/reduce_task.h
--- a/csrc/consumer/reduce_task.h
+++ b/csrc/consumer/reduce_task.h
@@ -138,6 +138,7 @@
     int64_t round_bytes = 2ll << 30;
     int maps = 0;
     int delivery_pack = 2;
+    bool delivery_pack_radix = true;
     int64_t delivery_piece_bytes = 64ll << 20;
   };
   void prewarm_gpu(PrewarmConf pc);
@@ -150,6 +151,7 @@
   std::string fault_spec_;
   double hbm_budget_conf_ = 0;
   int delivery_pack_ = 2;
+  bool delivery_pack_radix_ = true;
   CombineOp combine_ = CombineOp::kNone;
   ChecksumMode checksum_ = ChecksumMode::kAuto;
   void note_checksum(int64_t parts, int64_t bytes, double gpu_ms = 0);
diff --git a/csrc/gpu/colpack.hip b/csrc/gpu/colpack.hip
--- a/csrc/gpu/colpack.hip
+++ b/csrc/gpu/colpack.hip
@@ -144,8 +144,8 @@
 }
 
 __global__ void __launch_bounds__(64) colpack_plan_kernel(const ColpackPieceDesc* pieces, int L, uint32_t buf_records,
-                                                          uint32_t version, int ko, int kl, const uint32_t* table,
-                                                          ColpackResult* results) {
+                                                          uint32_t version, int ko, int kl, int allow_radix,
+                                                          const uint32_t* table, ColpackResult* results) {
   const ColpackPieceDesc pc = pieces[blockIdx.x];
   const uint32_t* tb = table + (size_t)blockIdx.x * kCpTableStride;
   const int G = (L + 7) / 8;
@@ -155,6 +155,11 @@
   __shared__ int s_bits[kColpackMaxGroups];
   __shared__ uint16_t s_bo[kColpackMaxGroups];
   __shared__ int s_stride;
+  __shared__ uint8_t s_range[kColpackMaxRecordBytes];
+  __shared__ int s_rbits[kColpackMaxGroups];
+  __shared__ uint16_t s_rbo[kColpackMaxGroups];
+  __shared__ int s_row_bits;
+  __shared__ uint64_t s_bitmap;
   int64_t plain_bits = 0, delta_bits = 0;
   for (int c = 0; c < kl; ++c) {
     plain_bits += width_of(tb[ko + c], 255u - tb[kColpackMaxRecordBytes + ko + c]);
@@ -173,6 +178,7 @@
           mx = 255u - tb[kCpTableDelta + kColpackMaxKeyBytes + kc];
         }
         const int w = width_of(mn, mx);
+        s_range[col] = (uint8_t)(mx > mn ? mx - mn : 0);
         bits += w;
         mask |= (uint64_t)((1u << w) - 1) << (8 * c);
         base |= (uint64_t)(mn & 0xFF) << (8 * c);
@@ -182,7 +188,21 @@
     s_bits[t] = bits;
   }
   __syncthreads();
-  if (t == 0) s_stride = colpack_layout(s_bits, G, v1, s_bo);
+  const int64_t table_bytes = delta ? colpack2_table_bytes(pc.nrec, buf_records) : 0;
+  if (t == 0) {
+    s_row_bits = 0;
+    if (allow_radix && !v1) {
+      uint64_t bitmap = 0;
+      const int row_bits = colpack2r_layout(s_range, L, s_rbits, s_rbo, &bitmap);
+      if (colpack2r_choose(bitmap, row_bits, pc.nrec, L, buf_records, table_bytes)) {
+        s_row_bits = row_bits;
+        s_bitmap = bitmap;
+        s_stride = (row_bits + 7) / 8;
+        for (int g = 0; g < G; ++g) s_bo[g] = s_rbo[g];
+      }
+    }
+    if (s_row_bits == 0) s_stride = colpack_layout(s_bits, G, v1, s_bo);
+  }
   __syncthreads();
   if (t < kColpackMaxGroups) {
     if (v1) {
@@ -193,16 +213,19 @@
     }
   }
   const int64_t S = s_stride;
+  const int row_bits = s_row_bits;
+  const bool radix = row_bits > 0;
   const bool raw = colpack_is_raw(S, L);
-  const int64_t table_bytes = delta ? colpack2_table_bytes(pc.nrec, buf_records) : 0;
-  const int64_t total = raw  ? (int64_t)kColpackHeaderBytes
-                        : v1 ? colpack_packed_bytes(S, pc.nrec)
-                             : colpack2_packed_bytes(S, pc.nrec, table_bytes);
+  const int64_t range_bytes = radix ? colpack2r_range_bytes(L) : 0;
+  const int64_t total = raw     ? (int64_t)kColpackHeaderBytes
+                        : v1    ? colpack_packed_bytes(S, pc.nrec)
+                        : radix ? colpack2r_packed_bytes(row_bits, pc.nrec, L, table_bytes)
+                                : colpack2_packed_bytes(S, pc.nrec, table_bytes);
   if (t == 0) {
     h->magic = kColpackMagic;
     h->version = version;
     h->record_bytes = (uint32_t)L;
-    h->flags = (raw ? 0 : kColpackFlagPacked) | (delta ? kColpackFlagDelta : 0);
+    h->flags = (raw ? 0 : kColpackFlagPacked) | (delta ? kColpackFlagDelta : 0) | (radix ? kColpackFlagRadix : 0);
     h->records = (uint64_t)pc.nrec;
     h->buf_records = buf_records;
     h->stride = (uint32_t)S;
@@ -210,17 +233,24 @@
     h->key_off = (uint32_t)ko;
     h->key_len = (uint32_t)kl;
     for (int k = 0; k < 5; ++k) h->reserved[k] = 0;
+    if (radix) {
+      h->reserved[0] = (uint32_t)s_bitmap;
+      h->reserved[1] = (uint32_t)(s_bitmap >> 32);
+      h->reserved[2] = (uint32_t)row_bits;
+    }
     ColpackResult r;
     r.bytes = total;
     r.packed = raw ? 0 : 1;
     r.stride = (uint32_t)S;
     r.delta = delta ? 1 : 0;
-    r.reserved = 0;
+    r.row_bits = radix ? (uint32_t)row_bits : 0u;
     results[blockIdx.x] = r;
   }
   if (raw) return;
+  if (radix)
+    for (int64_t i = t; i < range_bytes; i += 64) pc.dst[kColpackHeaderBytes + i] = i < L ? s_range[i] : (uint8_t)0;
   if (delta) {
-    uint8_t* tab = pc.dst + kColpackHeaderBytes;
+    uint8_t* tab = pc.dst + kColpackHeaderBytes + range_bytes;
     const int64_t entries = (pc.nrec + buf_records - 1) / buf_records;
     for (int64_t b = t; b < entries; b += 64) {
       const uint8_t* key = pc.src + b * buf_records * L + ko;
@@ -228,7 +258,8 @@
     }
     for (int64_t i = entries * kColpackRestartBytes + t; i < table_bytes; i += 64) tab[i] = 0;
   }
-  for (int64_t i = (int64_t)kColpackHeaderBytes + table_bytes + S * pc.nrec + t; i < total; i += 64) pc.dst[i] = 0;
+  const int64_t row_bytes = radix ? ((int64_t)row_bits * pc.nrec + 7) / 8 : S * pc.nrec;
+  for (int64_t i = (int64_t)kColpackHeaderBytes + range_bytes + table_bytes + row_bytes + t; i < total; i += 64) pc.dst[i] = 0;
 }
 
 template <int kG>
@@ -239,6 +270,8 @@
   if (!(flags & kColpackFlagPacked)) return;
   const int S = (int)h->stride;
   if (S == 0) return;
+  const bool radix = (flags & kColpackFlagRadix) != 0;
+  const int row_bits = radix ? (int)h->reserved[2] : 8 * S;
   const int64_t ntiles = (pc.nrec + kCpTileRows - 1) / kCpTileRows;
   if ((int64_t)blockIdx.x >= ntiles) return;
   const int G = kG ? kG : (L + 7) / 8;
@@ -250,8 +283,32 @@
   __shared__ uint64_t s_shift[kColpackMaxGroups];
   __shared__ int s_bits[kColpackMaxGroups];
   __shared__ uint16_t s_bo[kColpackMaxGroups];
+  __shared__ uint32_t s_mult[kColpackMaxGroups][8];
+  __shared__ uint8_t s_h0[kColpackMaxGroups];
   __shared__ __attribute__((aligned(16))) uint32_t s_tile[kCpTileBytes / 4 + 4];
-  if (t < G) {
+  if (radix && t < G) {
+    const uint64_t mask = h->mask[t];
+    const uint8_t* range = pc.dst + kColpackHeaderBytes + 8 * t;
+    const uint64_t bitmap = (uint64_t)h->reserved[0] | ((uint64_t)h->reserved[1] << 32);
+    int bits = 0;
+    for (int k = 0; k < 2; ++k) {
+      const bool rx = (bitmap >> (2 * t + k)) & 1;
+      uint64_t prod = 1;
+      int w = 0;
+      for (int c = 4 * k; c < 4 * k + 4; ++c) {
+        const int wc = __popc((uint32_t)(mask >> (8 * c)) & 0xFF);
+        s_mult[t][c] = (uint32_t)prod;
+        prod *= rx ? (uint64_t)range[c] + 1 : (uint64_t)1 << wc;
+        w += wc;
+      }
+      const int hb = rx ? 64 - __clzll((long long)(prod - 1)) : w;
+      if (k == 0) s_h0[t] = (uint8_t)hb;
+      bits += hb;
+    }
+    s_base[t] = h->base[t];
+    s_bits[t] = bits;
+    s_bo[t] = h->bo[t];
+  } else if (t < G) {
     const uint64_t mask = h->mask[t];
     uint64_t sh = 0;
     int bits = 0;
@@ -264,13 +321,14 @@
     s_bits[t] = bits;
   }
   __syncthreads();
-  if (t == 0) colpack_layout(s_bits, G, h->version == kColpackVersion, s_bo);
-  __syncthreads();
-  uint8_t* rows = pc.dst + kColpackHeaderBytes + (delta ? colpack2_table_bytes(pc.nrec, buf_records) : 0);
+  if (t == 0 && !radix) colpack_layout(s_bits, G, h->version == kColpackVersion, s_bo);
+  __syncthreads();
+  uint8_t* rows = pc.dst + kColpackHeaderBytes + (radix ? colpack2r_range_bytes(L) : 0) +
+                  (delta ? colpack2_table_bytes(pc.nrec, buf_records) : 0);
   for (int64_t tile = blockIdx.x; tile < ntiles; tile += gridDim.x) {
     const int64_t r0 = tile * kCpTileRows;
     const int nrows = (int)min((int64_t)kCpTileRows, pc.nrec - r0);
-    const int nbytes = nrows * S;
+    const int nbytes = (nrows * row_bits + 7) >> 3;
     for (int i = t; i < (nbytes + 15) >> 4; i += kCpThreads) reinterpret_cast<uint4*>(s_tile)[i] = make_uint4(0, 0, 0, 0);
     __syncthreads();
     const uint8_t* src = pc.src + r0 * L;
@@ -282,11 +340,19 @@
       uint64_t x = load_cols(rec + 8 * g, ncol);
       if (group_has_key(g, ko, kl)) x = with_key_delta(x, g, key_delta(rec, r0 + r, L, buf_records, ko, kl), ko, kl);
       x -= s_base[g];
-      const uint64_t sh = s_shift[g];
       uint64_t word = 0;
-#pragma unroll
-      for (int c = 0; c < 8; ++c) word |= ((x >> (8 * c)) & 0xFF) << ((uint32_t)(sh >> (8 * c)) & 0xFF);
-      const int bit = r * S * 8 + s_bo[g];
+      if (radix) {
+        const uint32_t lo = (uint32_t)x, hi = (uint32_t)(x >> 32);
+        const uint32_t* m = s_mult[g];
+        const uint32_t f0 = (lo & 0xFF) + ((lo >> 8) & 0xFF) * m[1] + ((lo >> 16) & 0xFF) * m[2] + (lo >> 24) * m[3];
+        const uint32_t f1 = (hi & 0xFF) + ((hi >> 8) & 0xFF) * m[5] + ((hi >> 16) & 0xFF) * m[6] + (hi >> 24) * m[7];
+        word = (uint64_t)f0 | ((uint64_t)f1 << s_h0[g]);
+      } else {
+        const uint64_t sh = s_shift[g];
+#pragma unroll
+        for (int c = 0; c < 8; ++c) word |= ((x >> (8 * c)) & 0xFF) << ((uint32_t)(sh >> (8 * c)) & 0xFF);
+      }
+      const int bit = r * row_bits + s_bo[g];
       const int wi = bit >> 5, ws = bit & 31;
       const uint64_t lo = word << ws;
       const uint32_t w0 = (uint32_t)lo, w1 = (uint32_t)(lo >> 32), w2 = ws ? (uint32_t)(word >> (64 - ws)) : 0u;
@@ -295,7 +361,7 @@
       if (w2) atomicOr(&s_tile[wi + 2], w2);
     }
     __syncthreads();
-    uint8_t* out = rows + r0 * S;
+    uint8_t* out = rows + r0 * row_bits / 8;
     const int n16 = nbytes >> 4;
     for (int i = t; i < n16; i += kCpThreads)
       reinterpret_cast<uint4*>(out)[i] = reinterpret_cast<const uint4*>(s_tile)[i];
@@ -308,9 +374,10 @@
 size_t colpack_table_bytes(int npieces) { return (size_t)npieces * kCpTableStride * sizeof(uint32_t); }
 
 void launch_colpack(const ColpackPieceDesc* pieces, int npieces, int64_t max_nrec, int L, int64_t buf_records,
-                    uint32_t* table, ColpackResult* results, hipStream_t s, int version, int key_off, int key_len) {
+                    uint32_t* table, ColpackResult* results, hipStream_t s, int version, int key_off, int key_len,
+                    bool radix) {
   if (npieces <= 0) return;
-  if (version != (int)kColpackVersion2) version = (int)kColpackVersion, key_len = 0;
+  if (version != (int)kColpackVersion2) version = (int)kColpackVersion, key_len = 0, radix = false;
   if (key_len <= 0 || key_len > kColpackMaxKeyBytes || key_off < 0 || key_off + key_len > L || buf_records < 1 ||
       buf_records > 0xFFFFFFFFll)
     key_len = 0;
@@ -323,7 +390,7 @@
   hipLaunchKernelGGL(colpack_stats_kernel, dim3((unsigned)sb, (unsigned)npieces), dim3(kCpThreads), 0, s, pieces, L,
                      (uint32_t)buf_records, key_off, key_len, table);
   hipLaunchKernelGGL(colpack_plan_kernel, dim3((unsigned)npieces), dim3(64), 0, s, pieces, L, (uint32_t)buf_records,
-                     (uint32_t)version, key_off, key_len, table, results);
+                     (uint32_t)version, key_off, key_len, radix ? 1 : 0, table, results);
   int64_t pb = (max_nrec + kCpTileRows - 1) / kCpTileRows;
   pb = std::max<int64_t>(1, std::min<int64_t>(pb, 1024));
   if (G == 13)
diff --git a/csrc/gpu/device_engine.cc b/csrc/gpu/device_engine.cc
--- a/csrc/gpu/device_engine.cc
+++ b/csrc/gpu/device_engine.cc
@@ -729,10 +729,11 @@
   if (cfg_.store != "hbm" && cfg_.store != "host" && cfg_.store != "disk")
     throw std::runtime_error("unknown store tier " + cfg_.store);
   const int version = delivery_pack_version(cfg_.delivery_pack);
-  if (version < 0) throw std::runtime_error("ShuffleJob: delivery_pack must be auto, v1 or off");
+  if (version < 0) throw std::runtime_error("ShuffleJob: delivery_pack must be auto, v2, v1 or off");
   check_delivery_order(cfg_.delivery_order);
   pack_ = cfg_.deliver_host && version != 0;
-  lay_ = fixed_layout(cfg_.kv_buf_bytes, cfg_.d2h_piece_bytes, cfg_.pinned_slots, pack_ ? version : 0);
+  lay_ = fixed_layout(cfg_.kv_buf_bytes, cfg_.d2h_piece_bytes, cfg_.pinned_slots, pack_ ? version : 0,
+                      pack_ && delivery_pack_radix(cfg_.delivery_pack));
   R_ = cfg_.reducers;
   Q_ = cfg_.rounds;
   C_ = R_ * Q_;
@@ -812,6 +813,7 @@
   if (!pack_) return name + " pack=off";
   name += " pack=colbits v" + std::to_string(lay_.pack_version);
   if (last_delta_ >= 0) name += last_delta_ ? " delta" : " plain";
+  if (last_radix_ > 0) name += " radix";
   if (last_d2h_ratio_ >= 0) {
     char b[32];
     std::snprintf(b, sizeof(b), " d2h/in=%.3f", last_d2h_ratio_);
@@ -1601,6 +1603,10 @@
             step_delta_ += pr.delta ? 1 : 0;
             step_stride_min_ = step_stride_min_ < 0 ? (int64_t)pr.stride : std::min<int64_t>(step_stride_min_, pr.stride);
             step_stride_max_ = std::max<int64_t>(step_stride_max_, pr.stride);
+            const int64_t row_bits = pr.row_bits ? (int64_t)pr.row_bits : 8 * (int64_t)pr.stride;
+            step_radix_ += pr.row_bits ? 1 : 0;
+            step_row_bits_min_ = step_row_bits_min_ < 0 ? row_bits : std::min(step_row_bits_min_, row_bits);
+            step_row_bits_max_ = std::max(step_row_bits_max_, row_bits);
           }
         }
         cv_.notify_all();
@@ -1802,6 +1808,9 @@
     step_d2h_bytes_ = step_packed_ = step_raw_ = step_delta_ = 0;
     step_stride_min_ = -1;
     step_stride_max_ = 0;
+    step_radix_ = 0;
+    step_row_bits_min_ = -1;
+    step_row_bits_max_ = 0;
     step_unpack_ms_ = 0;
     step_t0_ms_ = t0;
     first_issue_ms_ = last_landing_ms_ = idle_since_ms_ = eof_done_ms_ = -1;
@@ -2084,7 +2093,7 @@
       auto pack_range = [&](int a, int b) {
         launch_colpack(d_pack_pieces_[q].as<ColpackPieceDesc>() + a, b - a, pack_max_nrec_[q], kTeraRecordBytes,
                        lay_.buf_records, d_pack_table_.as<uint32_t>(), d_pack_results_[slot].as<ColpackResult>() + a,
-                       s_compute_, lay_.pack_version, kTeraKeyOffset, kTeraKeyBytes);
+                       s_compute_, lay_.pack_version, kTeraKeyOffset, kTeraKeyBytes, lay_.pack_radix);
         HIP_CHECK(hipGetLastError());
         HIP_CHECK(hipMemcpyAsync(h_pack_results_[slot].as<ColpackResult>() + a,
                                  d_pack_results_[slot].as<ColpackResult>() + a, (size_t)(b - a) * sizeof(ColpackResult),
@@ -2151,6 +2160,10 @@
     st.pack_delta_pieces = step_delta_;
     st.pack_stride_min = std::max<int64_t>(step_stride_min_, 0);
     st.pack_stride_max = step_stride_max_;
+    st.pack_radix_pieces = step_radix_;
+    st.pack_row_bits_min = std::max<int64_t>(step_row_bits_min_, 0);
+    st.pack_row_bits_max = step_row_bits_max_;
+    if (deliver && pack_) last_radix_ = step_packed_ > 0 && step_radix_ == step_packed_ ? 1 : 0;
     if (deliver && pack_) last_delta_ = step_packed_ > 0 && step_delta_ == step_packed_ ? 1 : 0;
     st.unpack_ms = step_unpack_ms_;
     st.slot_wait_ms = step_slot_wait_ms_;
diff --git a/csrc/gpu/device_engine.h b/csrc/gpu/device_engine.h
--- a/csrc/gpu/device_engine.h
+++ b/csrc/gpu/device_engine.h
@@ -241,6 +241,9 @@
   int64_t pack_delta_pieces = 0;
   int64_t pack_stride_min = 0;
   int64_t pack_stride_max = 0;
+  int64_t pack_radix_pieces = 0;
+  int64_t pack_row_bits_min = 0;
+  int64_t pack_row_bits_max = 0;
   double unpack_ms = 0;
   double lead_in_ms = 0;
   double link_idle_ms = 0;
@@ -392,6 +395,7 @@
   std::vector<DeviceBuffer> d_pack_results_;
   std::vector<PinnedBuffer> h_pack_results_;
   double last_d2h_ratio_ = -1;
+  int last_radix_ = -1;
   int last_delta_ = -1;
 
   std::unique_ptr<SdmaEngine> sdma_;
@@ -430,6 +434,7 @@
   double step_d2h_ms_ = 0;
   int64_t step_d2h_bytes_ = 0, step_packed_ = 0, step_raw_ = 0, step_delta_ = 0;
   int64_t step_stride_min_ = -1, step_stride_max_ = 0;
+  int64_t step_radix_ = 0, step_row_bits_min_ = -1, step_row_bits_max_ = 0;
   double step_unpack_ms_ = 0;
   std::vector<bool> slot_flying_;
   int flying_ = 0;
diff --git a/csrc/gpu/device_reduce.cc b/csrc/gpu/device_reduce.cc
--- a/csrc/gpu/device_reduce.cc
+++ b/csrc/gpu/device_reduce.cc
@@ -280,7 +280,7 @@
       ColpackResult* dr = ws_.d_pk_res.as<ColpackResult>() + half * S;
       HIP_CHECK(hipMemcpyAsync(dd, hd, (size_t)n * sizeof(ColpackPieceDesc), hipMemcpyHostToDevice, ws_.ps));
       launch_colpack(dd, n, hd[0].nrec, (int)kTeraRecordBytes, lay_.buf_records, ws_.d_pk_table.as<uint32_t>(), dr, ws_.ps,
-                     lay_.pack_version, kTeraKeyOffset, kTeraKeyBytes);
+                     lay_.pack_version, kTeraKeyOffset, kTeraKeyBytes, lay_.pack_radix);
       HIP_CHECK(hipGetLastError());
       HIP_CHECK(hipMemcpyAsync(host_results() + half * S, dr, (size_t)n * sizeof(ColpackResult), hipMemcpyDeviceToHost, ws_.ps));
       HIP_CHECK(hipEventRecord(ws_.packed_ev[half], ws_.ps));
@@ -306,6 +306,7 @@
           h = Held{lay_.packed_copy_len(pr.bytes, len / kTeraRecordBytes), true};
           from = ws_.pring.as<uint8_t>() + (int64_t)at * lay_.region_bytes;
           st_.delta_pieces += pr.delta ? 1 : 0;
+          st_.radix_pieces += pr.row_bits ? 1 : 0;
         }
       }
       hsa_signal_t sg = ring_.sig[(size_t)(k % S)];
@@ -376,7 +377,7 @@
   const double slot = (double)round_bytes * 1.1 * 1.125;
   int64_t packed = 0;
   if (cfg && cfg->pack_version != 0) {
-    const FixedLayout lay = fixed_layout(cfg->kv_buf_bytes, cfg->piece_bytes, cfg->pinned_slots, cfg->pack_version);
+    const FixedLayout lay = fixed_layout(cfg->kv_buf_bytes, cfg->piece_bytes, cfg->pinned_slots, cfg->pack_version, cfg->pack_radix);
     const PackNeed n = pack_need(lay, (int64_t)((double)round_bytes * 1.1) / kTeraRecordBytes + 1);
     packed = n.ring + n.desc + n.res + n.table;
     packed += packed / 8;
@@ -388,7 +389,7 @@
   HIP_CHECK(hipSetDevice(cfg.device));
   const int64_t rec = std::max<int64_t>(1, cfg.round_bytes / kTeraRecordBytes);
   const int64_t mr = rec + rec / 8;
-  const FixedLayout lay = fixed_layout(cfg.kv_buf_bytes, cfg.piece_bytes, cfg.pinned_slots, cfg.pack_version);
+  const FixedLayout lay = fixed_layout(cfg.kv_buf_bytes, cfg.piece_bytes, cfg.pinned_slots, cfg.pack_version, cfg.pack_radix);
   std::vector<std::unique_ptr<WsLease>> leases;
   std::vector<std::unique_ptr<Ring>> rings;
   for (int i = 0; i < std::max(1, count); ++i) {
@@ -442,7 +443,7 @@
   WsLease lease(cfg.device, N * kTeraRecordBytes);
   FixedWs& ws = *lease.w;
   hipStream_t s = ws.s;
-  const FixedLayout lay = fixed_layout(cfg.kv_buf_bytes, cfg.piece_bytes, cfg.pinned_slots, cfg.pack_version);
+  const FixedLayout lay = fixed_layout(cfg.kv_buf_bytes, cfg.piece_bytes, cfg.pinned_slots, cfg.pack_version, cfg.pack_radix);
   if (N == 0) {
     const uint8_t eof[2] = {0xFF, 0xFF};
     const double a = now_ms();
@@ -686,7 +687,7 @@
     lease.clean = true;
     return st;
   }
-  const FixedLayout lay = fixed_layout(cfg.kv_buf_bytes, cfg.piece_bytes, cfg.pinned_slots, cfg.pack_version);
+  const FixedLayout lay = fixed_layout(cfg.kv_buf_bytes, cfg.piece_bytes, cfg.pinned_slots, cfg.pack_version, cfg.pack_radix);
   HbmLedger& led = HbmLedger::get();
   int64_t round_bytes = std::max<int64_t>(cfg.round_bytes, kTeraRecordBytes);
   struct Span {
diff --git a/csrc/gpu/device_reduce.h b/csrc/gpu/device_reduce.h
--- a/csrc/gpu/device_reduce.h
+++ b/csrc/gpu/device_reduce.h
@@ -18,6 +18,7 @@
   int64_t piece_bytes = 64ll << 20;
   int pinned_slots = 4;
   int pack_version = 0;
+  bool pack_radix = false;
   int64_t sample_every = 4096;
   std::function<bool()> stop;
   std::function<bool()> decode_turn;
@@ -41,6 +42,7 @@
   int64_t packed_pieces = 0;
   int64_t raw_pieces = 0;
   int64_t delta_pieces = 0;
+  int64_t radix_pieces = 0;
   double unpack_ms = 0;
   double pack_wait_ms = 0;
 };
diff --git a/csrc/gpu/fixed_delivery.cc b/csrc/gpu/fixed_delivery.cc
--- a/csrc/gpu/fixed_delivery.cc
+++ b/csrc/gpu/fixed_delivery.cc
@@ -20,7 +20,7 @@
 
 int delivery_pack_version(const std::string& value) {
   int v;
-  if (value == "auto")
+  if (value == "auto" || value == "v2")
     v = (int)kColpackVersion2;
   else if (value == "v1")
     v = (int)kColpackVersion;
@@ -31,6 +31,10 @@
   if (const char* e = std::getenv("UDA_DELIVERY_PACK"))
     if (std::atoi(e) == 0) v = 0;
   return v;
+}
+
+bool delivery_pack_radix(const std::string& value) {
+  return value == "auto" && delivery_pack_version(value) == (int)kColpackVersion2;
 }
 
 int64_t FixedLayout::piece_bound(int64_t nrec) const {
@@ -44,9 +48,11 @@
   return packed_bytes;
 }
 
-FixedLayout fixed_layout(int64_t kv_buf_bytes, int64_t piece_bytes, int pinned_slots, int pack_version) {
+FixedLayout fixed_layout(int64_t kv_buf_bytes, int64_t piece_bytes, int pinned_slots, int pack_version,
+                         bool pack_radix) {
   FixedLayout l;
   l.pack_version = pack_version;
+  l.pack_radix = pack_radix && pack_version == (int)kColpackVersion2;
   l.slots = std::max(2, pinned_slots);
   l.kv_buf_bytes = kv_buf_bytes;
   l.buf_records = std::max<int64_t>(1, kv_buf_bytes / kFixedRecordBytes);
diff --git a/csrc/gpu/fixed_delivery.h b/csrc/gpu/fixed_delivery.h
--- a/csrc/gpu/fixed_delivery.h
+++ b/csrc/gpu/fixed_delivery.h
@@ -11,9 +11,11 @@
 constexpr int64_t kFixedEofBytes = 2;
 
 int delivery_pack_version(const std::string& value);
+bool delivery_pack_radix(const std::string& value);
 
 struct FixedLayout {
   int pack_version = 0;
+  bool pack_radix = false;
   int slots = 2;
   int64_t kv_buf_bytes = 0;
   int64_t buf_records = 1, buf_bytes = kFixedRecordBytes;
@@ -27,7 +29,8 @@
   uint8_t* slot(uint8_t* ring, int64_t k) const { return ring + (k % slots) * slot_bytes; }
   uint8_t* staging(uint8_t* ring, int i) const { return ring + (int64_t)slots * slot_bytes + (i & 1) * staging_bytes; }
 };
-FixedLayout fixed_layout(int64_t kv_buf_bytes, int64_t piece_bytes, int pinned_slots, int pack_version);
+FixedLayout fixed_layout(int64_t kv_buf_bytes, int64_t piece_bytes, int pinned_slots, int pack_version,
+                         bool pack_radix = false);
 
 struct FixedPiece {
   const uint8_t* base = nullptr;
diff --git a/csrc/gpu/kernels.h b/csrc/gpu/kernels.h
--- a/csrc/gpu/kernels.h
+++ b/csrc/gpu/kernels.h
@@ -173,12 +173,12 @@
   uint32_t packed;
   uint32_t stride;
   uint32_t delta;
-  uint32_t reserved;
+  uint32_t row_bits;
 };
 size_t colpack_table_bytes(int npieces);
 void launch_colpack(const ColpackPieceDesc* pieces, int npieces, int64_t max_nrec, int L, int64_t buf_records,
                     uint32_t* table, ColpackResult* results, hipStream_t s, int version = 1, int key_off = 0,
-                    int key_len = 0);
+                    int key_len = 0, bool radix = false);
 
 struct DecodeDesc {
   int64_t src;
diff --git a/csrc/python/bindings.cc b/csrc/python/bindings.cc
--- a/csrc/python/bindings.cc
+++ b/csrc/python/bindings.cc
@@ -80,6 +80,9 @@
   d["pack_delta_pieces"] = s.pack_delta_pieces;
   d["pack_stride_min"] = s.pack_stride_min;
   d["pack_stride_max"] = s.pack_stride_max;
+  d["pack_radix_pieces"] = s.pack_radix_pieces;
+  d["pack_row_bits_min"] = s.pack_row_bits_min;
+  d["pack_row_bits_max"] = s.pack_row_bits_max;
   d["raw_pieces"] = s.raw_pieces;
   d["unpack_ms"] = s.unpack_ms;
   d["lead_in_ms"] = s.lead_in_ms;
@@ -410,6 +413,18 @@
     out.resize((size_t)n);
     return py::bytes(out);
   }, py::arg("records"), py::arg("record_bytes"), py::arg("buf_records"), py::arg("key_off"), py::arg("key_len"));
+  m.def("colpack2r_encode", [](py::bytes b, int L, int64_t buf_records, int key_off, int key_len) {
+    std::string s = b;
+    if (L < 1 || L > kColpackMaxRecordBytes || s.empty() || s.size() % (size_t)L)
+      throw py::value_error("colpack2r_encode: need whole records of 1..256 bytes");
+    if (key_off < 0 || key_len < 0 || key_len > kColpackMaxKeyBytes || key_off + key_len > L)
+      throw py::value_error("colpack2r_encode: key field outside the record or longer than 16 bytes");
+    const int64_t nrec = (int64_t)s.size() / L;
+    std::string out((size_t)colpack2_bound(L, nrec, buf_records), '\0');
+    const int64_t n = colpack2r_encode((const uint8_t*)s.data(), nrec, L, buf_records, key_off, key_len, (uint8_t*)&out[0]);
+    out.resize((size_t)n);
+    return py::bytes(out);
+  }, py::arg("records"), py::arg("record_bytes"), py::arg("buf_records"), py::arg("key_off"), py::arg("key_len"));
   m.def("colpack_decode", [](py::bytes b, int expect_L, int64_t expect_records, const std::string& path, int64_t row0,
                              int64_t rows) {
     std::string s = b;
@@ -423,6 +438,9 @@
     std::string out((size_t)(rows * p.L), '\0');
     if (path == "bmi2") {
       if (!colpack_unpack_bmi2(p, row0, rows, (uint8_t*)&out[0])) throw std::runtime_error("no BMI2 on this CPU");
+    } else if (path == "simd") {
+      if (!colpack_unpack_radix_simd(p, row0, rows, (uint8_t*)&out[0]))
+        throw std::runtime_error("the AVX2 radix decoder does not take this piece on this CPU");
     } else if (path == "scalar") {
       colpack_unpack_scalar(p, row0, rows, (uint8_t*)&out[0]);
     } else {
@@ -432,7 +450,7 @@
   }, py::arg("piece"), py::arg("expect_record_bytes") = 0, py::arg("expect_records") = 0, py::arg("path") = "auto",
      py::arg("row0") = 0, py::arg("rows") = -1);
   auto gpu_encode = [](const std::vector<std::string>& pieces, int L, int64_t buf_records, int device, int version,
-                       int key_off, int key_len) {
+                       int key_off, int key_len, bool radix) {
     if (L < 1 || L > kColpackMaxRecordBytes || pieces.empty()) throw py::value_error("gpu_colpack_encode: bad arguments");
     if (key_off < 0 || key_len < 0 || key_len > kColpackMaxKeyBytes || key_off + key_len > L)
       throw py::value_error("gpu_colpack_encode: key field outside the record or longer than 16 bytes");
@@ -470,7 +488,7 @@
       hipStream_t s = nullptr;
       HIP_CHECK(hipStreamCreateWithFlags(&s, hipStreamNonBlocking));
       gpu::launch_colpack(ddesc.as<gpu::ColpackPieceDesc>(), n, max_nrec, L, buf_records, dtab.as<uint32_t>(),
-                          dres.as<gpu::ColpackResult>(), s, version, key_off, key_len);
+                          dres.as<gpu::ColpackResult>(), s, version, key_off, key_len, radix);
       HIP_CHECK(hipGetLastError());
       HIP_CHECK(hipStreamSynchronize(s));
       HIP_CHECK(hipStreamDestroy(s));
@@ -488,11 +506,16 @@
     return ret;
   };
   m.def("gpu_colpack_encode", [gpu_encode](const std::vector<std::string>& pieces, int L, int64_t buf_records, int device) {
-    return gpu_encode(pieces, L, buf_records, device, 1, 0, 0);
+    return gpu_encode(pieces, L, buf_records, device, 1, 0, 0, false);
   }, py::arg("pieces"), py::arg("record_bytes"), py::arg("buf_records") = 1, py::arg("device") = 0);
   m.def("gpu_colpack2_encode", [gpu_encode](const std::vector<std::string>& pieces, int L, int64_t buf_records,
                                             int key_off, int key_len, int device) {
-    return gpu_encode(pieces, L, buf_records, device, 2, key_off, key_len);
+    return gpu_encode(pieces, L, buf_records, device, 2, key_off, key_len, false);
+  }, py::arg("pieces"), py::arg("record_bytes"), py::arg("buf_records"), py::arg("key_off"), py::arg("key_len"),
+     py::arg("device") = 0);
+  m.def("gpu_colpack2r_encode", [gpu_encode](const std::vector<std::string>& pieces, int L, int64_t buf_records,
+                                             int key_off, int key_len, int device) {
+    return gpu_encode(pieces, L, buf_records, device, 2, key_off, key_len, true);
   }, py::arg("pieces"), py::arg("record_bytes"), py::arg("buf_records"), py::arg("key_off"), py::arg("key_len"),
      py::arg("device") = 0);
   m.def("fixed_delivery_piece", [](py::bytes piece, int64_t record_bytes, int64_t buf_bytes, int64_t kv_buf, bool packed,
@@ -533,6 +556,7 @@
   }, py::arg("piece"), py::arg("record_bytes"), py::arg("buf_bytes"), py::arg("kv_buf"), py::arg("packed"), py::arg("last"),
      py::arg("deliver") = true);
   m.def("delivery_pack_version", &gpu::delivery_pack_version);
+  m.def("delivery_pack_radix", &gpu::delivery_pack_radix);
   m.def("fixed_delivery_packed_copy_len", [](int64_t kv_buf, int64_t piece_bytes, int pinned_slots, int pack_version,
                                              int64_t packed_bytes, int64_t nrec) {
     return gpu::fixed_layout(kv_buf, piece_bytes, pinned_slots, pack_version).packed_copy_len(packed_bytes, nrec);
@@ -559,7 +583,8 @@
     cfg.piece_bytes = piece_bytes;
     cfg.sample_every = 16;
     cfg.pack_version = gpu::delivery_pack_version(pack);
-    if (cfg.pack_version < 0) throw py::value_error("gpu_device_reduce_fixed: pack is auto, v1 or off");
+    cfg.pack_radix = gpu::delivery_pack_radix(pack);
+    if (cfg.pack_version < 0) throw py::value_error("gpu_device_reduce_fixed: pack is auto, v2, v1 or off");
     if (kv_buf < 1 || round_bytes < 1 || piece_bytes < 1) throw py::value_error("gpu_device_reduce_fixed: bad sizes");
     for (const auto& r : runs)
       if (r.size() % (size_t)gpu::kTeraRecordBytes) throw py::value_error("gpu_device_reduce_fixed: need whole records");
@@ -597,6 +622,7 @@
     d["packed_pieces"] = st.packed_pieces;
     d["raw_pieces"] = st.raw_pieces;
     d["delta_pieces"] = st.delta_pieces;
+    d["radix_pieces"] = st.radix_pieces;
     d["unpack_ms"] = st.unpack_ms;
     d["pack_wait_ms"] = st.pack_wait_ms;
     d["d2h_wait_ms"] = st.d2h_wait_ms;
```

New measurement: 82.46. 0.898x the previous value.
